# guoyihonggyh/MOBODY-Model-Based-Off-Dynamics-Offline-Reinforcement-Learning

Hardware: AMD Instinct MI355X
Metric: transitions/sec (minibatch rows through train(), refresh amortised at 1/5000) + grad-steps/sec (higher is better)
Workload: dtype f16x2

## Files before the change

### include/mobody_hip.h

```cpp
#ifndef MOBODY_HIP_H
#define MOBODY_HIP_H
#include <stddef.h>
#include <stdint.h>

#ifdef __cplusplus
extern "C" {
#endif

#define MOBODY_ABI_VERSION 6
#define MOBODY_E_ARG (-1)
#define MOBODY_E_LAUNCH (-2)
#define MOBODY_E_UNSUPPORTED (-3)

#define MOBODY_HIDDEN 256
#define MOBODY_ENSEMBLE 7
#define MOBODY_LATENT 16

enum { MOBODY_TERM_NEVER = 0, MOBODY_TERM_HALFCHEETAH = 1, MOBODY_TERM_HOPPER = 2, MOBODY_TERM_ANT = 3,
       MOBODY_TERM_WALKER2D = 4, MOBODY_TERM_HUMANOID = 5, MOBODY_TERM_PEN = 6 };

typedef struct MobodyLayer {
  int32_t in_dim, out_dim;
  int32_t Kp, Np;
  int64_t w_off, b_off;
// ... 31 lines not shown
#define MOBODY_HEALTH_F16_RANGE 1
#define MOBODY_HEALTH_NONFINITE 2
#define MOBODY_F16_W_LIMIT 255.875f
int mobody_health_bind(int32_t* words_dev);
int mobody_health_clear(void* stream);

int mobody_rng_normal(uint32_t seed, uint32_t stream_id, uint32_t call, int64_t n, float* out, void* stream);
int mobody_rng_index(uint32_t seed, uint32_t stream_id, uint32_t call, int64_t n, uint32_t bound, int32_t* out,
                     void* stream);

int mobody_dyn_forward(const float* dyn_blob, const float* dyn_planes, int precision, int S, int A, const float* obs,
                       const float* act, int64_t B, int use_trg, float* mean, void* stream);
int64_t mobody_dyn_planes_floats(void);
int mobody_dyn_planes(const float* dyn_blob, int S, int A, float* planes, int precision, void* stream);

int64_t mobody_dyn_step_workspace(int S, int A, int64_t B);

int mobody_dyn_step(const float* dyn_blob, const float* dyn_planes, int precision, int S, int A, int task,
                    const float* obs, const float* act, int64_t B,
                    const float* noise, const int32_t* elite_idx, const uint8_t* alive, const int32_t* elites,
                    int n_elites, uint32_t seed,
                    uint32_t call, const int64_t* call_dev, float penalty_coef, int use_penalty, int use_trg, float* next_obs,
                    float* reward,
                    uint8_t* terminal, float* penalty, float* raw_reward, float* mean_out, float* workspace,
                    void* stream);

int mobody_mopo_step(const float* dyn_blob, const float* dyn_planes, const float* mopo_blob, const float* mopo_blob_T,
                     int precision, int S, int A, int task, const float* obs, const float* act, int64_t B,
                     const float* noise, const int32_t* elite_idx, const uint8_t* alive, const int32_t* elites,
                     int n_elites, uint32_t seed, uint32_t call, float penalty_coef, int use_penalty, float* next_obs,
                     float* reward, uint8_t* terminal, float* penalty, float* raw_reward, float* mean_out,
                     float* workspace, void* stream);

enum { MOBODY_UNC_PAIRWISE = 0,
       MOBODY_UNC_ALEATORIC = 1,
       MOBODY_UNC_ENS_STD = 2 };

typedef struct MobodyEnsStep {
  int32_t struct_bytes, uncertainty_mode;
  const float *dyn_blob, *dyn_planes, *mopo_blob, *mopo_blob_T;
  int32_t precision, S, A, task;
  const float *obs, *act;
  int64_t B;
  const float* noise; const int32_t* elite_idx; const uint8_t* alive;
  const int32_t* elites;
  int32_t n_elites; uint32_t seed, call; int32_t use_penalty;
  const int64_t* call_dev;
  float penalty_coef; int32_t use_trg;
  float *next_obs, *reward; uint8_t* terminal; float *penalty, *raw_reward, *mean_out, *workspace;
} MobodyEnsStep;
int mobody_ens_step(const MobodyEnsStep* a, void* stream);

typedef struct MobodyBufferView {
  const float* state; const float* action; const float* next_state; const float* reward; const float* not_done;
  int64_t pitch;
} MobodyBufferView;
int64_t mobody_ring_pitch(int S, int A);

int64_t mobody_rollout_workspace(int S, int A, int64_t B);
int mobody_rollout(const float* dyn_blob, const float* dyn_planes, const float* actor_blob, const float* actor_blob_T,
                   int precision, int S, int A, int task, float max_action,
                   const float* init_obs, int64_t B, int H, const int32_t* elites, int n_elites, uint32_t seed, uint32_t call0,
                   float penalty_coef, int use_penalty, int use_trg, float env_filter, int filter_bad_rollout,
                   const MobodyBufferView* ring, int64_t cap, int64_t* ptr_size, float* workspace, void* stream);

typedef struct MobodyEnsRollout {
  int32_t struct_bytes, uncertainty_mode;
  const float *dyn_blob, *dyn_planes, *mopo_blob, *mopo_blob_T, *actor_blob, *actor_blob_T;
  int32_t precision, S, A, task;
  const float* init_obs;
  int64_t B;
  int32_t H, n_elites;
  const int32_t* elites;
  uint32_t seed, call0;
  const int64_t* call_dev;
  float max_action, penalty_coef, env_filter; int32_t use_penalty, use_trg, filter_bad_rollout;
  const MobodyBufferView* ring;
  int64_t cap;
  int64_t* ptr_size;
  float* workspace;
} MobodyEnsRollout;
int64_t mobody_ens_rollout_workspace(const MobodyEnsRollout* a);
int mobody_ens_rollout(const MobodyEnsRollout* a, void* stream);

int mobody_termination(int task, const float* next_obs, int64_t B, int S, uint8_t* done, void* stream);

int mobody_rollout_mask(const uint8_t* alive_in, const uint8_t* terminal, const float* penalty, float env_filter,
                        int use_filter, int64_t B, uint8_t* keep, uint8_t* alive_out, void* stream);

int mobody_sample_indices(uint32_t seed, uint32_t stream_id, const int64_t* counter, int64_t call_offset, int64_t n,
                          const int64_t* size, int32_t* out, void* stream);

int mobody_counter_add(int64_t* counter, int n, int64_t inc, void* stream);

int mobody_mlp3_forward(const float* blob, const float* blob_T, int precision, int in_dim, int out_dim, int members,
                        const float* src0, int n0, const float* src1, int n1, int64_t rows, int out_mode,
                        float max_action, float* out, float* save_x, float* save_h1, float* save_h2, void* stream);

int mobody_gather_batch(const MobodyBufferView* bufs, const int32_t* const* idx, const int64_t* counts, int nbuf,
                        int S, int A, float* state, float* action, float* next_state, float* reward, float* not_done,
                        void* stream);

int mobody_gather_batch_rng(const MobodyBufferView* bufs, const int64_t* counts, int nbuf, int S, int A,
                            const uint32_t* seeds, const int64_t* call_offsets, const int64_t* counter,
                            const int64_t* const* sizes, float* state, float* action, float* next_state,
                            float* reward, float* not_done, int64_t* const* bump, int nbump, void* stream);

int mobody_ring_append(const MobodyBufferView* ring, int64_t cap, int64_t* ptr_size, int S, int A, const float* obs,
                       const float* act, const float* next_obs, const float* reward, const uint8_t* terminal,
                       const uint8_t* keep, int64_t M, int32_t* scan_ws, void* stream);

typedef struct MobodyTrainDims {
  int32_t S, A;
  int64_t N;
  int64_t Nt;
  int64_t N_global;
  int64_t Nt_global;
} MobodyTrainDims;

typedef struct MobodyHyper {
  float gamma, tau, max_action, weight, bc_coef;
  int32_t q_weighted, scale_q;
  int32_t precision;
} MobodyHyper;

int64_t mobody_train_workspace(const MobodyTrainDims* d);

int mobody_critic_step(const MobodyTrainDims* d, const MobodyHyper* h, const float* actor_blob, const float* actor_blob_T,
                       const float* q_blob, const float* q_blob_T, const float* qtarg_blob, const float* qtarg_blob_T,
                       const float* state, const float* action, const float* next_state, const float* reward,
                       const float* not_done, const float* q_next, float* grad_q, float* loss_out, float* workspace,
                       int policy_forward, void* stream);

int mobody_critic_update(const MobodyTrainDims* d, const MobodyHyper* h, const float* actor_blob, const float* actor_blob_T,
                         float* q_blob, float* q_blob_T, float* qtarg_blob, float* qtarg_blob_T, const float* state,
                         const float* action, const float* next_state, const float* reward, const float* not_done,
                         const float* q_next, float* m, float* v, int64_t t, const int64_t* t_dev, float lr,
                         float* loss_out, float* workspace, int policy_forward, int64_t* bump, void* stream);

int mobody_actor_forward(const MobodyTrainDims* d, const MobodyHyper* h, const float* actor_blob, const float* actor_blob_T,
                         const float* q_blob, const float* q_blob_T, const float* state, const float* action, float* stats,
                         float* workspace, int policy_ready, void* stream);

int mobody_actor_backward(const MobodyTrainDims* d, const MobodyHyper* h, const float* actor_blob,
                          const float* actor_blob_T, const float* q_blob, const float* q_blob_T, const float* state,
                          const float* action, const float* stats, const float* v_true, float* grad_actor,
                          float* loss_out, float* workspace, void* stream);

int mobody_critic_update_phase(const MobodyTrainDims* d, const MobodyHyper* h, const float* actor_blob, const float* actor_blob_T,
                               float* q_blob, float* q_blob_T, float* qtarg_blob, float* qtarg_blob_T, const float* state,
                               const float* action, const float* next_state, const float* reward, const float* not_done,
                               const float* q_next, float* m, float* v, int64_t t, const int64_t* t_dev, float lr, float* loss_out,
                               float* workspace, int policy_forward, int64_t* bump, int phase, void* stream);

int mobody_actor_update(const MobodyTrainDims* d, const MobodyHyper* h, float* actor_blob, float* actor_blob_T,
                        const float* q_blob, const float* q_blob_T, const float* state, const float* action,
                        const float* stats, const float* v_true, float* m, float* v, int64_t t, const int64_t* t_dev,
                        float lr, float* loss_out, float* workspace, void* stream);

int mobody_value_loss_grad(const float* qt, const float* v, int64_t N, int64_t N_global, float* dz3, float* loss_out,
                           float* lossp_ws, void* stream);

int mobody_adam_polyak(int in_dim, int out_dim, int members, float* blob, float* blob_T, const float* grad, float* m,
                       float* v, float* target, float* target_T, int64_t t, float lr, float tau, float grad_scale,
                       int precision, void* stream);

int mobody_adam_polyak_dev(int in_dim, int out_dim, int members, float* blob, float* blob_T, const float* grad,
                           float* m, float* v, float* target, float* target_T, const int64_t* t_dev, float lr, float tau,
                           float grad_scale, int precision, void* stream);

int mobody_par_penalty(const float* next_state_true, const float* next_state_model, float* reward, float coef,
                       int64_t n, int S, void* stream);

int64_t mobody_mlp3_backward_workspace(int in_dim, int out_dim, int members, int64_t rows);
int mobody_mlp3_backward(const float* blob_T, int in_dim, int out_dim, int members, const float* dz3, const float* x,
                         const float* h1, const float* h2, int64_t rows, float* grad, float* workspace, void* stream);

int mobody_dara_inputs(const float* s, const float* a, const float* s2, int64_t N, int S, int A, float std,
                       const float* noise_sas, const float* noise_sa, uint32_t seed, uint32_t call, float* x_sas,
                       float* x_sa, void* stream);

int mobody_dara_loss_grad(const float* z_sas, const float* z_sa, const int32_t* labels, int64_t N, int64_t n_src,
                          float* dz_sas, float* dz_sa, float* loss_out, float* lossp_ws, void* stream);

int mobody_dara_penalty(const float* z_sas, const float* z_sa, int64_t n, float coef, float* reward, float* delta_out,
                        void* stream);

typedef struct MobodyPretrainLayout {
  int32_t S, A, za_in, _pad;
  MobodyMlpLayout enc, tr, rw;
  int64_t off_enc, off_tr, off_rw, off_za_src, off_za_trg;
  int64_t za_w1, za_b1, za_w2, za_b2, za_member_floats;
  int64_t total_floats;
  int64_t t_off_enc, t_off_tr, t_off_rw, t_total_floats;
} MobodyPretrainLayout;
int mobody_pretrain_layout(int S, int A, MobodyPretrainLayout* out);
int mobody_pretrain_transpose(int S, int A, const float* blob, float* blob_T, int precision, void* stream);
int64_t mobody_pretrain_workspace(int S, int A, int64_t b);

int mobody_pretrain_gather(const float* state, const float* action, const float* next_state, const float* reward,
                           const int32_t* idx, int64_t n_idx, int64_t start, const int64_t* start_dev, int64_t b, int S,
                           int A, float* xenc, float* act, float* rew, void* stream);

int mobody_pretrain_grads(int S, int A, int64_t b, int64_t b_global, int use_trg, float encoder_loss_coef,
                          const float* blob, const float* blob_T, const float* xenc, const float* act, const float* rew,
                          const float* noise6, const float* noise7, uint32_t seed, uint32_t call, float* grad,
                          float* loss_out, float* workspace, int precision, float transition_coef, float reward_coef,
                          void* stream);

int mobody_pretrain_update(int S, int A, int64_t b, int use_trg, float encoder_loss_coef, float* blob, float* blob_T,
                           const float* xenc, const float* act, const float* rew, const float* noise6, const float* noise7,
                           uint32_t seed, uint32_t call, const int64_t* call_dev, float* m, float* v, int64_t t_main,
                           int64_t t_za, const int64_t* t_dev, float lr, float* loss_out, float* loss_acc, float* workspace,
                           int precision, void* stream);

int mobody_pretrain_adam(int S, int A, int use_trg, float* blob, float* blob_T, const float* grad, float* m, float* v,
                         int64_t t_main, int64_t t_za, float lr, float grad_scale, int precision, int net_mask, int64_t t_rw,
                         void* stream);

int mobody_pretrain_za_adam(int S, int A, int use_trg, float* blob, const float* grad, float* m, float* v, int64_t t_za,
                            float lr, float grad_scale, void* stream);

int64_t mobody_dyn_validate_workspace(int S, int A, int64_t B);
int mobody_dyn_validate(const float* dyn_blob, int S, int A, const float* obs, const float* act, const float* next_obs,
                        const float* rew, int64_t B, int use_trg, float* out, float* workspace, void* stream);

typedef struct MobodyPretrainMopoLayout {
  int32_t S, A, _pad0, _pad1;
  MobodyMlpLayout dyn, rw;
  int64_t off_dyn, off_rw, total_floats;
  int64_t t_off_dyn, t_off_rw, t_total_floats;
} MobodyPretrainMopoLayout;
int mobody_pretrain_mopo_layout(int S, int A, MobodyPretrainMopoLayout* out);
int mobody_pretrain_mopo_transpose(int S, int A, const float* blob, float* blob_T, int precision, void* stream);
int64_t mobody_pretrain_mopo_workspace(int S, int A, int64_t b);
int mobody_pretrain_mopo_grads(int S, int A, int64_t b, int64_t b_global, int use_trg, float encoder_loss_coef,
                               const float* blob, const float* blob_T, const float* xenc, const float* act, const float* rew,
                               const float* noise, uint32_t seed, uint32_t call, float* grad, float* loss_out,
                               float* workspace, int precision, void* stream);
int mobody_pretrain_mopo_update(int S, int A, int64_t b, int use_trg, float encoder_loss_coef, float* blob, float* blob_T,
                                const float* xenc, const float* act, const float* rew, const float* noise, uint32_t seed,
                                uint32_t call, const int64_t* call_dev, float* m, float* v, int64_t t, const int64_t* t_dev,
                                float lr, float* loss_out, float* loss_acc, float* workspace, int precision, void* stream);
int mobody_pretrain_mopo_adam(int S, int A, float* blob, float* blob_T, const float* grad, float* m, float* v, int64_t t,
                              float lr, float grad_scale, int precision, void* stream);
int mobody_dyn_validate_mopo(const float* dyn_blob, const float* mopo_blob, int S, int A, const float* obs, const float* act,
                             const float* next_obs, const float* rew, int64_t B, float* out, float* workspace, void* stream);

int mobody_mlp_transpose(int in_dim, int out_dim, int members, const float* blob, float* blob_T, int precision,
                         void* stream);

#ifdef __cplusplus
}
#endif
#endif
```

### mobody-model-based-off-dynamics-offline-reinforcement-learning_amd/_lib.py

```python
import ctypes as C
import os

_HERE = os.path.dirname(os.path.abspath(__file__))
LIB_PATH = os.path.join(_HERE, "csrc", "libmobody_hip.so")

i32, i64, u32, f32 = C.c_int32, C.c_int64, C.c_uint32, C.c_float
vp = C.c_void_p


class MobodyLayer(C.Structure):
    _fields_ = [("in_dim", i32), ("out_dim", i32), ("Kp", i32), ("Np", i32), ("w_off", i64), ("b_off", i64)]


DL_NAMES = ["zs1", "zs2", "zs3", "za_src1", "za_src2", "za_trg1", "za_trg2", "transition1", "transition2",
            "transition3", "reward_model1", "reward_model2", "reward_model3"]


class MobodyDynLayout(C.Structure):
    _fields_ = [("S", i32), ("A", i32), ("E", i32), ("_pad", i32), ("layer", MobodyLayer * len(DL_NAMES)),
                ("total_floats", i64)]


class MobodyMlpLayout(C.Structure):
    _fields_ = [("in_dim", i32), ("out_dim", i32), ("members", i32), ("Kp1", i32), ("Np3", i32), ("Np1t", i32),
                ("w1", i64), ("b1", i64), ("w2", i64), ("b2", i64), ("w3", i64), ("b3", i64),
                ("member_floats", i64), ("total_floats", i64), ("w3t", i64), ("w2t", i64), ("w1t", i64),
                ("t_member_floats", i64), ("t_total_floats", i64), ("w2p", i64), ("w2tp", i64)]


class MobodyPretrainLayout(C.Structure):
    _fields_ = [("S", i32), ("A", i32), ("za_in", i32), ("_pad", i32), ("enc", MobodyMlpLayout), ("tr", MobodyMlpLayout),
                ("rw", MobodyMlpLayout), ("off_enc", i64), ("off_tr", i64), ("off_rw", i64), ("off_za_src", i64),
                ("off_za_trg", i64), ("za_w1", i64), ("za_b1", i64), ("za_w2", i64), ("za_b2", i64),
                ("za_member_floats", i64), ("total_floats", i64), ("t_off_enc", i64), ("t_off_tr", i64),
                ("t_off_rw", i64), ("t_total_floats", i64)]


class MobodyPretrainMopoLayout(C.Structure):
    _fields_ = [("S", i32), ("A", i32), ("_pad0", i32), ("_pad1", i32), ("dyn", MobodyMlpLayout), ("rw", MobodyMlpLayout),
                ("off_dyn", i64), ("off_rw", i64), ("total_floats", i64), ("t_off_dyn", i64), ("t_off_rw", i64),
                ("t_total_floats", i64)]


class MobodyBufferView(C.Structure):
    _fields_ = [("state", vp), ("action", vp), ("next_state", vp), ("reward", vp), ("not_done", vp), ("pitch", i64)]


class MobodyTrainDims(C.Structure):
    _fields_ = [("S", i32), ("A", i32), ("N", i64), ("Nt", i64), ("N_global", i64), ("Nt_global", i64)]


class MobodyHyper(C.Structure):
    _fields_ = [("gamma", f32), ("tau", f32), ("max_action", f32), ("weight", f32), ("bc_coef", f32),
                ("q_weighted", i32), ("scale_q", i32), ("precision", i32)]


class MobodyEnsStep(C.Structure):
    _fields_ = [("struct_bytes", i32), ("uncertainty_mode", i32), ("dyn_blob", vp), ("dyn_planes", vp), ("mopo_blob", vp),
                ("mopo_blob_T", vp), ("precision", i32), ("S", i32), ("A", i32), ("task", i32), ("obs", vp), ("act", vp),
                ("B", i64), ("noise", vp), ("elite_idx", vp), ("alive", vp), ("elites", C.POINTER(i32)), ("n_elites", i32),
                ("seed", u32), ("call", u32), ("use_penalty", i32), ("call_dev", vp), ("penalty_coef", f32), ("use_trg", i32),
                ("next_obs", vp), ("reward", vp), ("terminal", vp), ("penalty", vp), ("raw_reward", vp), ("mean_out", vp),
                ("workspace", vp)]


class MobodyEnsRollout(C.Structure):
    _fields_ = [("struct_bytes", i32), ("uncertainty_mode", i32), ("dyn_blob", vp), ("dyn_planes", vp), ("mopo_blob", vp),
                ("mopo_blob_T", vp), ("actor_blob", vp), ("actor_blob_T", vp), ("precision", i32), ("S", i32), ("A", i32),
                ("task", i32), ("init_obs", vp), ("B", i64), ("H", i32), ("n_elites", i32), ("elites", C.POINTER(i32)),
                ("seed", u32), ("call0", u32), ("call_dev", vp), ("max_action", f32), ("penalty_coef", f32),
                ("env_filter", f32), ("use_penalty", i32), ("use_trg", i32), ("filter_bad_rollout", i32),
                ("ring", C.POINTER(MobodyBufferView)), ("cap", i64), ("ptr_size", vp), ("workspace", vp)]


PRECISIONS = {"f32": 0, "bf16": 1, "bf16x2": 2, "bf16x3": 3, "f16x2": 4}


UNCERTAINTY_MODES = {"pairwise-diff": 0, "aleatoric": 1, "ensemble_std": 2}

TERM_IDS = {"never": 0, "halfcheetah": 1, "hopper": 2, "ant": 3, "walker2d": 4, "humanoid": 5, "pen": 6}

HEALTH_WORDS, HEALTH_F16_RANGE, HEALTH_NONFINITE = 8, 1, 2

PROTOTYPES = {
    "mobody_last_error": (C.c_char_p, []),
    "mobody_abi_version": (C.c_int, []),
    "mobody_dyn_layout": (C.c_int, [C.c_int, C.c_int, C.POINTER(MobodyDynLayout)]),
    "mobody_mlp_layout": (C.c_int, [C.c_int, C.c_int, C.c_int, C.POINTER(MobodyMlpLayout)]),
    "mobody_prof_begin": (C.c_int, [C.c_int]),
    "mobody_prof_end": (C.c_int, [C.POINTER(C.c_double), C.POINTER(i64), C.c_int]),
    "mobody_health_bind": (C.c_int, [vp]),
    "mobody_health_clear": (C.c_int, [vp]),
    "mobody_rng_normal": (C.c_int, [u32, u32, u32, i64, vp, vp]),
    "mobody_rng_index": (C.c_int, [u32, u32, u32, i64, u32, vp, vp]),
    "mobody_dyn_forward": (C.c_int, [vp, vp, C.c_int, C.c_int, C.c_int, vp, vp, i64, C.c_int, vp, vp]),
    "mobody_dyn_planes_floats": (i64, []),
    "mobody_dyn_planes": (C.c_int, [vp, C.c_int, C.c_int, vp, C.c_int, vp]),
    "mobody_dyn_step_workspace": (i64, [C.c_int, C.c_int, i64]),
    "mobody_dyn_step": (C.c_int, [vp, vp, C.c_int, C.c_int, C.c_int, C.c_int, vp, vp, i64, vp, vp, vp, C.POINTER(i32), C.c_int,
                                  u32, u32, vp, f32, C.c_int, C.c_int, vp, vp, vp, vp, vp, vp, vp, vp]),
    "mobody_mopo_step": (C.c_int, [vp, vp, vp, vp, C.c_int, C.c_int, C.c_int, C.c_int, vp, vp, i64, vp, vp, vp, C.POINTER(i32), C.c_int,
                                   u32, u32, f32, C.c_int, vp, vp, vp, vp, vp, vp, vp, vp]),
    "mobody_ens_step": (C.c_int, [C.POINTER(MobodyEnsStep), vp]),
    "mobody_ens_rollout_workspace": (i64, [C.POINTER(MobodyEnsRollout)]),
    "mobody_ens_rollout": (C.c_int, [C.POINTER(MobodyEnsRollout), vp]),
    "mobody_rollout_workspace": (i64, [C.c_int, C.c_int, i64]),
    "mobody_rollout": (C.c_int, [vp, vp, vp, vp, C.c_int, C.c_int, C.c_int, C.c_int, f32, vp, i64, C.c_int, C.POINTER(i32), C.c_int, u32, u32, f32,
                                 C.c_int, C.c_int, f32, C.c_int, C.POINTER(MobodyBufferView), i64, vp, vp, vp]),
    "mobody_termination": (C.c_int, [C.c_int, vp, i64, C.c_int, vp, vp]),
    "mobody_rollout_mask": (C.c_int, [vp, vp, vp, f32, C.c_int, i64, vp, vp, vp]),
    "mobody_sample_indices": (C.c_int, [u32, u32, vp, i64, i64, vp, vp, vp]),
    "mobody_counter_add": (C.c_int, [vp, C.c_int, i64, vp]),
    "mobody_mlp3_forward": (C.c_int, [vp, vp, C.c_int, C.c_int, C.c_int, C.c_int, vp, C.c_int, vp, C.c_int, i64, C.c_int, f32, vp,
                                      vp, vp, vp, vp]),
    "mobody_gather_batch": (C.c_int, [C.POINTER(MobodyBufferView), C.POINTER(vp), C.POINTER(i64), C.c_int, C.c_int,
                                      C.c_int, vp, vp, vp, vp, vp, vp]),
    "mobody_gather_batch_rng": (C.c_int, [C.POINTER(MobodyBufferView), C.POINTER(i64), C.c_int, C.c_int, C.c_int,
                                          C.POINTER(u32), C.POINTER(i64), vp, C.POINTER(vp), vp, vp, vp, vp, vp, C.POINTER(vp), C.c_int,
                                          vp]),
    "mobody_ring_append": (C.c_int, [C.POINTER(MobodyBufferView), i64, vp, C.c_int, C.c_int, vp, vp, vp, vp, vp, vp, i64, vp,
                                     vp]),
    "mobody_ring_pitch": (i64, [C.c_int, C.c_int]),
    "mobody_train_workspace": (i64, [C.POINTER(MobodyTrainDims)]),
    "mobody_critic_step": (C.c_int, [C.POINTER(MobodyTrainDims), C.POINTER(MobodyHyper), vp, vp, vp, vp, vp, vp, vp, vp, vp,
                                     vp, vp, vp, vp, vp, vp, C.c_int, vp]),
    "mobody_critic_update": (C.c_int, [C.POINTER(MobodyTrainDims), C.POINTER(MobodyHyper), vp, vp, vp, vp, vp, vp, vp, vp, vp,
                                       vp, vp, vp, vp, vp, i64, vp, f32, vp, vp, C.c_int, vp, vp]),
    "mobody_critic_update_phase": (C.c_int, [C.POINTER(MobodyTrainDims), C.POINTER(MobodyHyper), vp, vp, vp, vp, vp, vp, vp, vp, vp,
                                             vp, vp, vp, vp, vp, i64, vp, f32, vp, vp, C.c_int, vp, C.c_int, vp]),
    "mobody_actor_update": (C.c_int, [C.POINTER(MobodyTrainDims), C.POINTER(MobodyHyper), vp, vp, vp, vp, vp, vp, vp,
                                      vp, vp, vp, i64, vp, f32, vp, vp, vp]),
    "mobody_value_loss_grad": (C.c_int, [vp, vp, i64, i64, vp, vp, vp, vp]),
    "mobody_actor_forward": (C.c_int, [C.POINTER(MobodyTrainDims), C.POINTER(MobodyHyper), vp, vp, vp, vp, vp, vp, vp, vp,
                                       C.c_int, vp]),
    "mobody_actor_backward": (C.c_int, [C.POINTER(MobodyTrainDims), C.POINTER(MobodyHyper), vp, vp, vp, vp, vp, vp,
                                        vp, vp, vp, vp, vp, vp]),
    "mobody_adam_polyak": (C.c_int, [C.c_int, C.c_int, C.c_int, vp, vp, vp, vp, vp, vp, vp, i64, f32, f32, f32, C.c_int, vp]),
    "mobody_adam_polyak_dev": (C.c_int, [C.c_int, C.c_int, C.c_int, vp, vp, vp, vp, vp, vp, vp, vp, f32, f32, f32, C.c_int, vp]),
    "mobody_par_penalty": (C.c_int, [vp, vp, vp, f32, i64, C.c_int, vp]),
    "mobody_mlp3_backward_workspace": (i64, [C.c_int, C.c_int, C.c_int, i64]),
    "mobody_mlp3_backward": (C.c_int, [vp, C.c_int, C.c_int, C.c_int, vp, vp, vp, vp, i64, vp, vp, vp]),
    "mobody_dara_inputs": (C.c_int, [vp, vp, vp, i64, C.c_int, C.c_int, f32, vp, vp, u32, u32, vp, vp, vp]),
    "mobody_dara_loss_grad": (C.c_int, [vp, vp, vp, i64, i64, vp, vp, vp, vp, vp]),
    "mobody_dara_penalty": (C.c_int, [vp, vp, i64, f32, vp, vp, vp]),
    "mobody_mlp_transpose": (C.c_int, [C.c_int, C.c_int, C.c_int, vp, vp, C.c_int, vp]),
    "mobody_pretrain_layout": (C.c_int, [C.c_int, C.c_int, C.POINTER(MobodyPretrainLayout)]),
    "mobody_pretrain_transpose": (C.c_int, [C.c_int, C.c_int, vp, vp, C.c_int, vp]),
    "mobody_pretrain_workspace": (i64, [C.c_int, C.c_int, i64]),
    "mobody_pretrain_gather": (C.c_int, [vp, vp, vp, vp, vp, i64, i64, vp, i64, C.c_int, C.c_int, vp, vp, vp, vp]),
    "mobody_pretrain_update": (C.c_int, [C.c_int, C.c_int, i64, C.c_int, f32, vp, vp, vp, vp, vp, vp, vp, u32, u32, vp, vp,
                                         vp, i64, i64, vp, f32, vp, vp, vp, C.c_int, vp]),
    "mobody_pretrain_grads": (C.c_int, [C.c_int, C.c_int, i64, i64, C.c_int, f32, vp, vp, vp, vp, vp, vp, vp, u32, u32,
                                        vp, vp, vp, C.c_int, f32, f32, vp]),
    "mobody_pretrain_adam": (C.c_int, [C.c_int, C.c_int, C.c_int, vp, vp, vp, vp, vp, i64, i64, f32, f32, C.c_int, C.c_int, i64, vp]),
    "mobody_pretrain_za_adam": (C.c_int, [C.c_int, C.c_int, C.c_int, vp, vp, vp, vp, i64, f32, f32, vp]),
    "mobody_pretrain_mopo_layout": (C.c_int, [C.c_int, C.c_int, C.POINTER(MobodyPretrainMopoLayout)]),
    "mobody_pretrain_mopo_transpose": (C.c_int, [C.c_int, C.c_int, vp, vp, C.c_int, vp]),
    "mobody_pretrain_mopo_workspace": (i64, [C.c_int, C.c_int, i64]),
    "mobody_pretrain_mopo_grads": (C.c_int, [C.c_int, C.c_int, i64, i64, C.c_int, f32, vp, vp, vp, vp, vp, vp, u32, u32, vp, vp,
                                             vp, C.c_int, vp]),
    "mobody_pretrain_mopo_update": (C.c_int, [C.c_int, C.c_int, i64, C.c_int, f32, vp, vp, vp, vp, vp, vp, u32, u32, vp, vp, vp,
                                              i64, vp, f32, vp, vp, vp, C.c_int, vp]),
    "mobody_pretrain_mopo_adam": (C.c_int, [C.c_int, C.c_int, vp, vp, vp, vp, vp, i64, f32, f32, C.c_int, vp]),
    "mobody_dyn_validate_mopo": (C.c_int, [vp, vp, C.c_int, C.c_int, vp, vp, vp, vp, i64, vp, vp, vp]),
    "mobody_dyn_validate_workspace": (i64, [C.c_int, C.c_int, i64]),
    "mobody_dyn_validate": (C.c_int, [vp, C.c_int, C.c_int, vp, vp, vp, vp, i64, C.c_int, vp, vp, vp]),
}

_lib = None


def load():
    global _lib
    if _lib is not None:
        return _lib
    import torch
    if not os.path.exists(LIB_PATH):
        raise ImportError(
            f"{LIB_PATH} not found: build it with `python {os.path.join(_HERE, 'csrc', 'build.py')}` "
            "(or __graft_entry__.build()). There is no CPU fallback for the MOBODY hot path.")
    lib = C.CDLL(LIB_PATH)
    for name, (res, args) in PROTOTYPES.items():
        fn = getattr(lib, name)
        fn.restype, fn.argtypes = res, args
    if lib.mobody_abi_version() != 6:
        raise ImportError("libmobody_hip.so ABI version mismatch")
    _lib = lib
    return lib


class MobodyError(RuntimeError):
    pass


def check(rc, what=""):
    if rc != 0:
        msg = load().mobody_last_error().decode(errors="replace")
        raise MobodyError(f"{what} failed ({rc}): {msg}")


def ptr(t):
    if t is None:
        return None
    assert t.is_contiguous(), "C ABI needs contiguous tensors"
    return t.data_ptr()


_dev_index = None


def cur_stream():
    global _dev_index
    import torch
    if _dev_index is None:
        _dev_index = torch.cuda.current_device()
    return torch._C._cuda_getCurrentRawStream(_dev_index)


def dyn_layout(S, A):
    L = MobodyDynLayout()
    check(load().mobody_dyn_layout(S, A, C.byref(L)), "mobody_dyn_layout")
    return L


def mlp_layout(in_dim, out_dim, members):
    L = MobodyMlpLayout()
    check(load().mobody_mlp_layout(in_dim, out_dim, members, C.byref(L)), "mobody_mlp_layout")
    return L


def pretrain_layout(S, A):
    L = MobodyPretrainLayout()
    check(load().mobody_pretrain_layout(S, A, C.byref(L)), "mobody_pretrain_layout")
    return L


def pretrain_mopo_layout(S, A):
    L = MobodyPretrainMopoLayout()
    check(load().mobody_pretrain_mopo_layout(S, A, C.byref(L)), "mobody_pretrain_mopo_layout")
    return L
```

### mobody-model-based-off-dynamics-offline-reinforcement-learning_amd/algo/offline_offline/mobody.py

```python
import numpy as np
import torch

from ... import _lib, dp, ops, packing
from .. import utils

REFRESH_EVERY = 5000
REFRESH_SRC, REFRESH_TAR = 50000, 2000
REFRESH_FROM_SRC_TAR = 100
GRAPH_DYN_SEED = 0x51ED


class _PackedNet(object):

    def __init__(self, in_dim, out_dim, members, prefixes, device, out_mode=0, max_action=1.0, init=True, precision=0):
        self.in_dim, self.out_dim, self.members, self.prefixes = in_dim, out_dim, members, prefixes
        self.device, self.out_mode, self.max_action = device, out_mode, float(max_action)
        self.precision = int(precision)
        self.layout = _lib.mlp_layout(in_dim, out_dim, members)
        if init:
            sd = {}
            for p in prefixes:
                for li, (i, o) in zip((0, 2, 4), ((in_dim, 256), (256, 256), (256, out_dim))):
                    bound = 1.0 / np.sqrt(i)
                    sd[f"{p}network.{li}.weight"] = torch.empty(o, i).uniform_(-bound, bound)
# ... 288 lines not shown
        rew_mean = res["rewards"].mean()
        if self.config["filter_bad_rollout"]:
            keep = (res["penalty"] <= self.config["env_filter"]).squeeze(1)
            res = {k: v[keep] for k, v in res.items()}
        return res, {"num_transitions": n_tr, "reward_mean": rew_mean}

    def _rollout_into_fake(self, init_obss, rollout_length, use_trg=True):
        if rollout_length == 0:
            return 0
        dyn, m, fb = self.dynamics, self.dynamics.model, self.fake_replay_buffer
        obs = init_obss.contiguous()
        B = obs.shape[0]
        m.inference()
        self._roll_ws = ops.rollout(m.packed(), self.policy.blob, self.S, self.A, dyn._task_id, self.policy.max_action, obs,
                                    rollout_length, list(m.elites_host()),
                                    (dyn.seed + dp.rank_salt()) & 0xFFFFFFFF, dyn._calls + 1, float(dyn._penalty_coef or 0.0),
                                    use_trg, True, self.config["env_filter"], self.config["filter_bad_rollout"],
                                    fb._fields(), fb.max_size, fb.ptr_size, getattr(self, "_roll_ws", None),
                                    dyn_planes=m.planes() if dyn.precision else None, actor_blob_T=self.policy.blob_T,
                                    precision=dyn.precision, mopo=m.packed_mopo() if getattr(m, "mopo", False) else None,
                                    uncertainty_mode=dyn._unc_id)
        dyn._calls += rollout_length
        fb._pull()
        return B * rollout_length

    def _refresh(self, src_rb, tar_rb, batch_size):
        cfg = self.config
        world = self._world() if int(cfg.get("shard_refresh", 1)) else 1
        n_src, n_tar = -(-REFRESH_SRC // world), -(-REFRESH_TAR // world)
        s_idx = src_rb.draw_indices(n_src)
        t_idx = tar_rb.draw_indices(n_tar)
        src = ops.gather_batch([src_rb._fields()], [s_idx], self.S, self.A)
        tar = ops.gather_batch([tar_rb._fields()], [t_idx], self.S, self.A)
        if self.rng == "device":
            self._rollout_into_fake(src[0], cfg["src_rollout_length"])
            self._rollout_into_fake(tar[0], cfg["trg_rollout_length"])
        else:
            tr, _ = self.rollout(src[0], cfg["src_rollout_length"])
            self.fake_replay_buffer.add_batch(tr)
            tr, _ = self.rollout(tar[0], cfg["trg_rollout_length"])
            self.fake_replay_buffer.add_batch(tr)
        if cfg["use_src_sa_to_get_target_next_state"]:
            r = self.dynamics.step_device(src[0], src[1])
            keep = (r["penalty"] < cfg["env_filter"]).to(torch.uint8).squeeze(1)
            self.fake_replay_buffer.add_batch(dict(obss=src[0], next_obss=r["next_obs"], actions=src[1],
                                                   rewards=r["reward"], terminals=r["terminal"]), keep=keep)
        if cfg["rollout_from_src"]:
            if self.penalty_type != "dara":
                self.update_classifier(src_rb, tar_rb, batch_size)
            s_idx = src_rb.draw_indices(n_src)
            t_idx = tar_rb.draw_indices(-(-REFRESH_FROM_SRC_TAR // world))
            init = ops.gather_batch([src_rb._fields(), tar_rb._fields()], [s_idx, t_idx], self.S, self.A)[0]
            tr, _ = self.rollout(init, cfg["rollout_from_src_length"], use_trg=False)
            if tr is not None and tr["obss"].shape[0] > 0:
                self._dara_delta(tr["obss"].contiguous(), tr["actions"].contiguous(), tr["next_obss"].contiguous(),
                                 tr["rewards"], cfg["penalty_coef"])
                self.fake_replay_buffer.add_batch(tr)

    def _health_check(self):
        words = ops.health_bound(self.device)
        if words is None or self._fault is not None:
            return
        mask, step = ops.health_read(words)
        if mask == 0:
            return
        cls = self.classifier
        nets = (("q_funcs", self.q_funcs, self.q_optimizer), ("target_q_funcs", self.target_q_funcs, self.q_optimizer),
                ("policy", self.policy, self.policy_optimizer), ("v_func", self.v_func, self.v_optimizer),
                ("classifier.sa_classifier", cls.sa_classifier, cls.opt_sa), ("classifier.sas_classifier", cls.sas_classifier, cls.opt_sas))
        found = []
        for name, n, opt in nets:
            w2 = ops._mlp_w2(n.blob, n.layout, n.members)
            m = float(w2.abs().max())
            if (n.precision == 4 and not (m < ops.F16_W_LIMIT)) or not bool(torch.isfinite(n.blob).all()):
                found.append((name, m, opt))
        frozen = self._health_rewind(step, found[0][2] if found else None)
        self._graph = None
        bits = "|".join(ops.health_bits(mask))
        where = ", ".join(f"{name} (max |W2| = {m:g})" for name, m, _ in found) or "no policy network (another object on this device)"
        msg = (f"device health word {bits}" + (f" at Adam step {step}" if step else "") + f": {where}; "
               f"{frozen} optimizer step(s) were frozen, the parameters are those of the last healthy update (an optimizer launch "
               f"that ran next to the faulting one on another stream, if there was one, may hold that step in part). "
               f"f16x2 planes hold |w| < {ops.F16_W_LIMIT}: use mfma='bf16x3' (or f16_guard='fallback')")
        if self.f16_guard == "fallback" and mask == _lib.HEALTH_F16_RANGE and found:
            import warnings
            warnings.warn("falling back to mfma='bf16x3': " + msg)
            self.mfma, self.precision = "bf16x3", ops.prec_id("bf16x3")
            self.config["mfma"] = "bf16x3"
            for n in (self.q_funcs, self.target_q_funcs, self.policy):
                n.precision = self.precision
                ops.mlp_transpose(n.blob, n.in_dim, n.out_dim, n.members, out=n.blob_T, precision=self.precision)
                n.version += 1
            self._ws, self._ws_key = None, None
            ops.health_clear()
            return
        self._fault = msg
        raise FloatingPointError(msg)

    def _health_rewind(self, step, opt):
        order = [self.v_optimizer, self.q_optimizer, self.policy_optimizer]
        if opt not in order or step <= 0 or opt.t < step:
            return 0
        n = opt.t - step
        k = order.index(opt)
        for j, o in enumerate(order):
            if o.t > 0:
                o.t = max(0, o.t - n - (1 if j > k else 0))
        return n

    def _graph_ok(self, writer):
        want = self.use_graph == 1 or (self.use_graph == 2 and self._batch[0].shape[0] < 4096)
        dyn = self.dynamics
        par_ok = self.penalty_type != "par" or (dyn is not None and getattr(dyn, "noise_fn", None) is None
                                                and dyn.rng == "device")
        adv_ok = not self.config["advantage"] or (self._world() == 1 and self.fused_update and self._v_ws is not None)
        logs = writer is not None and (self.total_it % 5000 == 0 or (self.penalty_type == "par" and self.total_it % 100 == 0))
        return (want and self.rng == "device" and par_ok and adv_ok and (self.total_it - 1) % REFRESH_EVERY != 0 and not logs)

    @staticmethod
    def _world():
        d = torch.distributed
        return d.get_world_size() if d.is_available() and d.is_initialized() else 1

    def _graph_segments(self, src, tar, batch_size, world, segmented):
        cfg, S, A = self.config, self.S, self.A
        ns, nt = int(cfg["src_ratio"] * batch_size), int(cfg["trg_ratio"] * batch_size)
        nf = int(cfg["fake_batch_scale"] * batch_size) if cfg["fake_batch_scale"] != 0 else 0
        N, Nt = ns + nt + nf, ns + nt
        Ng, Ntg = N * world, Nt * world
        c, b = self._ctr, self._batch
        bufs, cnts, seeds = [src, tar], [ns, nt], [self._seed_for(101), self._seed_for(102)]
        if nf > 0:
            bufs.append(self.fake_replay_buffer); cnts.append(nf); seeds.append(self._seed_for(103))

        par = self.penalty_type == "par"

        def par_relabel(call):
            r = self.dynamics.step_device(b[0][:ns], b[1][:ns], call=call, call_dev=c[0:1], seed_offset=GRAPH_DYN_SEED)
            ops.par_penalty(b[2][:ns], r["next_obs"], b[3][:ns], cfg["penalty_coef"])

        def critic():
            ops.counter_add(c[0:3])
            ops.gather_batch_rng([rb._fields() for rb in bufs], cnts, seeds, [0] * len(bufs), c[0:1],
                                 [rb.ptr_size[1:2] for rb in bufs], S, A, b)
            if par:
                par_relabel(0)
            self.critic_grad(b, N, Nt, Ng, Ntg)

        def critic_apply_actor_stats():
            self.q_optimizer.step_dev(c[1:2], target=self.target_q_funcs, tau=self.tau)
            self.actor_stats(b, N, Nt, Ng, Ntg)

        def fused_step():
            ops.gather_batch_rng([rb._fields() for rb in bufs], cnts, seeds, [1] * len(bufs), c[0:1],
                                 [rb.ptr_size[1:2] for rb in bufs], S, A, b, bump=(c[1:2], c[2:3], c[3:4]))
            if par and not cfg["advantage"] and int(cfg.get("par_overlap", 1)):
                main = torch.cuda.current_stream()
                if getattr(self, "_side_stream", None) is None:
                    self._side_stream = torch.cuda.Stream(device=self.device)
                side = self._side_stream
                side.wait_stream(main)
                with torch.cuda.stream(side):
                    par_relabel(1)
                self.critic_update(b, N, Nt, t_dev=c[1:2], bump=c[0:1], phase=1)
                main.wait_stream(side)
                self.critic_update(b, N, Nt, t_dev=c[1:2], bump=c[0:1], phase=2)
                self.actor_stats(b, N, Nt, N, Nt)
                self.actor_update(b, N, Nt, t_dev=c[2:3])
                return
            if par:
                par_relabel(1)
            if cfg["advantage"]:
                self.value_grad(b, N, Nt, N, Nt)
                self.v_optimizer.step_dev(c[3:4])
            self.critic_update(b, N, Nt, t_dev=c[1:2], bump=c[0:1])
            self.actor_stats(b, N, Nt, N, Nt)
            self.actor_update(b, N, Nt, t_dev=c[2:3])

        def actor():
            self.actor_grad(b, N, Nt, Ng, Ntg)

        def actor_apply():
            self.policy_optimizer.step_dev(c[2:3])

        if not segmented:
            if self.fused_update:
                return [fused_step]
            return [lambda: (critic(), critic_apply_actor_stats(), actor(), actor_apply())]
        if self.dp_graph == "captured":
            d = torch.distributed

            def whole_step():
                critic(); d.all_reduce(self.q_optimizer.grad)
                critic_apply_actor_stats(); d.all_reduce(self._stats)
                actor(); d.all_reduce(self.policy_optimizer.grad)
                actor_apply()
            return [whole_step]
        return [critic, critic_apply_actor_stats, actor, actor_apply]

    def _graph_step(self, src, tar, batch_size):
        world = self._world()
        segmented = world > 1 or (self._force_segments and torch.distributed.is_initialized())
        if segmented and self.dp_graph == "captured" and torch.distributed.get_backend() != "nccl":
            self.dp_graph = "segments"
        fb = self.fake_replay_buffer
        nets = (self.q_funcs, self.target_q_funcs, self.policy, self.v_func)
        opts = (self.q_optimizer, self.policy_optimizer, self.v_optimizer)
        dyn_key = None
        if self.penalty_type == "par":
            m = self.dynamics.model
            dyn_key = (m.packed().data_ptr(), m.planes().data_ptr() if self.dynamics.precision else 0, self.dynamics.precision,
                       m.elites_host(), float(self.dynamics._penalty_coef or 0.0), self.dynamics._unc_id,
                       tuple(t.data_ptr() for t in m.packed_mopo()) if getattr(m, "mopo", False) else None)
        key = (batch_size, id(src), id(tar), src.state.data_ptr(), tar.state.data_ptr(), world, segmented,
               id(fb), fb.state.data_ptr(), fb.ptr_size.data_ptr(), tuple(t.data_ptr() for t in self._batch),
               tuple((n.blob.data_ptr(), n.blob_T.data_ptr()) for n in nets), self.precision,
               tuple((o.m.data_ptr(), o.v.data_ptr(), o.grad.data_ptr()) for o in opts),
               None if self._ws is None else self._ws.data_ptr(), self.dp_graph, dyn_key,
               None if self._v_ws is None else self._v_ws.data_ptr())
        if self._graph is None or self._graph_key != key:
            torch.cuda.synchronize()
            self._ctr[1] = self.q_optimizer.t
            self._ctr[2] = self.policy_optimizer.t
            self._ctr[3] = self.v_optimizer.t
            if self.penalty_type == "par":
                self.dynamics.step_device(self._batch[0][:int(self.config["src_ratio"] * batch_size)],
                                          self._batch[1][:int(self.config["src_ratio"] * batch_size)], call=0)
            graphs = []
            try:
                for seg in self._graph_segments(src, tar, batch_size, world, segmented):
                    g = torch.cuda.CUDAGraph()
                    with torch.cuda.graph(g, capture_error_mode="thread_local"):
                        seg()
                    graphs.append(g)
            except Exception as exc:
                import warnings
                torch.cuda.synchronize()
                if segmented and self.dp_graph == "captured":
                    warnings.warn(f"capturing the all-reduces failed ({exc!r}); falling back to segment graphs")
                    self.dp_graph, self._graph = "segments", None
                    return self._graph_step(src, tar, batch_size)
                warnings.warn(f"HIP-graph capture of the train() step failed ({exc!r}); continuing eagerly")
                self.use_graph, self._graph = 0, None
                return False
            self._graph, self._graph_key = graphs, key
        if len(self._graph) == 1:
            self._graph[0].replay()
        else:
            d = torch.distributed
            ga, gb, gc, gd = self._graph
            ga.replay()
            d.all_reduce(self.q_optimizer.grad)
            gb.replay()
            d.all_reduce(self._stats)
            gc.replay()
            d.all_reduce(self.policy_optimizer.grad)
            gd.replay()
        self.q_optimizer.t += 1
        self.policy_optimizer.t += 1
        if self.config["advantage"]:
            self.v_optimizer.t += 1
        return True

    def train(self, src_replay_buffer, tar_replay_buffer, batch_size=128, writer=None, wandbrun=None):
        cfg = self.config
        self.total_it += 1
        self.src_replay_buffer, self.tar_replay_buffer = src_replay_buffer, tar_replay_buffer
        if not self._synced:
            self.sync_replicas()
        S, A = self.S, self.A
        ns, nt = int(cfg["src_ratio"] * batch_size), int(cfg["trg_ratio"] * batch_size)
        nf = int(cfg["fake_batch_scale"] * batch_size) if cfg["fake_batch_scale"] != 0 else 0
        N, Nt = ns + nt + nf, ns + nt
        if (self.total_it - 1) % REFRESH_EVERY == 0 or (writer is not None and self.total_it % 5000 == 0):
            self._health_check()
        if (self._batch is not None and self._batch_key == (N,) and self._graph_ok(writer)
                and self._graph_step(src_replay_buffer, tar_replay_buffer, batch_size)):
            return
        if self._graph is not None:
            self._graph = None
        if self.penalty_type == "dara" and self.total_it == 1:
            self._dara_warmup(src_replay_buffer, tar_replay_buffer, batch_size, writer)
        if self._batch_key != (N,):
            dev = self.device
            self._batch = (torch.empty(N, S, device=dev), torch.empty(N, A, device=dev), torch.empty(N, S, device=dev),
                           torch.empty(N, 1, device=dev), torch.empty(N, 1, device=dev))
            self._batch_key = (N,)
        b = self._batch
        self._gather([src_replay_buffer, tar_replay_buffer], [ns, nt], tuple(t[:Nt] for t in b))
        if self.penalty_type == "par":
            r = self.dynamics.step_device(b[0][:ns], b[1][:ns])
            if writer is not None and self.total_it % 100 == 0:
                writer.add_scalar("train/reward_penalty_par", torch.mean((b[2][:ns] - r["next_obs"]) ** 2), global_step=self.total_it)
            ops.par_penalty(b[2][:ns], r["next_obs"], b[3][:ns], cfg["penalty_coef"])
        if (self.total_it - 1) % REFRESH_EVERY == 0:
            self._refresh(src_replay_buffer, tar_replay_buffer, batch_size)
        if nf > 0:
            self._gather([self.fake_replay_buffer], [nf], tuple(t[Nt:] for t in b))
        log5k = writer is not None and self.total_it % 5000 == 0
        if log5k and cfg["advantage"]:
            qt = ops.mlp3_forward(self.target_q_funcs.blob, S + A, 1, 2, b[0], b[1]).view(2, N)
            v0 = ops.mlp3_forward(self.v_func.blob, S, 1, 1, b[0]).view(N)
            writer.add_scalar("train/adv", (torch.minimum(qt[0], qt[1]) - v0).mean(), self.total_it)
            writer.add_scalar("train/value", v0.mean(), self.total_it)
        self._update(b, N, Nt)
        if log5k:
            if cfg["q_weighted"] and Nt > 0:
                qb = ops.mlp3_forward(self.q_funcs.blob, S + A, 1, 2, b[0][:Nt], b[1][:Nt], blob_T=self.q_funcs.blob_T,
                                      precision=self.precision).view(2, Nt)
                qb = torch.minimum(qb[0], qb[1])
                if cfg["advantage"]:
                    adv = qb - ops.mlp3_forward(self.v_func.blob, S, 1, 1, b[0][:Nt]).view(Nt)
                else:
                    adv = qb / qb.abs().mean()
                writer.add_scalar("train/exp_adv", torch.exp(3.0 * adv).clamp(max=100.0).mean(), self.total_it)
            q_loss, pi_loss, bc_loss = [float(x) for x in self._loss[:3].tolist()]
            writer.add_scalar("train/q_loss", q_loss, self.total_it)
            writer.add_scalar("train/policy_loss", pi_loss, self.total_it)
            writer.add_scalar("train/bc_loss", bc_loss, self.total_it)
            prec = self.precision
            q12 = ops.mlp3_forward(self.q_funcs.blob, self.S + self.A, 1, 2, b[0], b[1], blob_T=self.q_funcs.blob_T, precision=prec)
            pi = ops.mlp3_forward(self.policy.blob, self.S, self.A, 1, b[0], out_mode=1, max_action=cfg["max_action"],
                                  blob_T=self.policy.blob_T, precision=prec)[0]
            qpi = ops.mlp3_forward(self.q_funcs.blob, self.S + self.A, 1, 2, b[0], pi, blob_T=self.q_funcs.blob_T, precision=prec)
            writer.add_scalar("train/q1", q12[0].mean(), self.total_it)
            writer.add_scalar("train/q_behavior", torch.minimum(q12[0], q12[1]).mean(), self.total_it)
            writer.add_scalar("train/q_policy", torch.minimum(qpi[0], qpi[1]).mean(), self.total_it)
            if wandbrun is not None:
                wandbrun.log({"train/policy_loss": pi_loss, "train/q_loss": q_loss}, step=self.total_it)

    def _gather(self, bufs, counts, out):
        if self.rng == "device":
            for rb in bufs:
                if rb.size <= 0:
                    raise ValueError("low >= high")
                rb._draws += 1
            salt = dp.rank_salt()
            ops.gather_batch_rng([rb._fields() for rb in bufs], counts, [(rb.seed + salt) & 0xFFFFFFFF for rb in bufs],
                                 [rb._draws for rb in bufs], None, [rb.ptr_size[1:2] for rb in bufs], self.S, self.A, out)
        else:
            idx = [rb.draw_indices(n) for rb, n in zip(bufs, counts)]
            ops.gather_batch([rb._fields() for rb in bufs], idx, self.S, self.A, out=out)

    def _update(self, b, N, Nt):
        d = torch.distributed
        dist = d if d.is_available() and d.is_initialized() else None
        if self.fused_update and dp.world_size(dist) == 1:
            if self.config["advantage"]:
                self.value_grad(b, N, Nt, N, Nt)
                self.value_apply()
            self.critic_update(b, N, Nt)
            self.actor_stats(b, N, Nt, N, Nt)
            self.actor_update(b, N, Nt)
        else:
            dp.dp_update(self, b, N, Nt, dist)

    def comm_device(self):
        return self.device

    def _dims(self, N, Nt, Ng, Ntg):
        if self._ws_key != (N, Nt):
            self._ws = ops.train_workspace(ops.train_dims(self.S, self.A, N, Nt, N, Nt), self.device)
            self._ws_key = (N, Nt)
        return ops.train_dims(self.S, self.A, N, Nt, Ng, Ntg), ops.hyper(self.config)

    def has_value_phase(self):
        return bool(self.config["advantage"])

    def value_grad(self, b, N, Nt, Ng, Ntg):
        S, A = self.S, self.A
        qt = ops.mlp3_forward(self.target_q_funcs.blob, S + A, 1, 2, b[0], b[1])
        v, x, h1, h2 = ops.mlp3_forward(self.v_func.blob, S, 1, 1, b[0], save=True)
        dz3, loss = ops.value_loss_grad(qt.view(2, N), v.view(N), Ng)
        self._v_ws = ops.mlp3_backward(self.v_func.blob_T, S, 1, 1, dz3, x, h1, h2, self.v_optimizer.grad, self._v_ws)
        self._loss[3:4].copy_(loss)

    def value_grad_buffer(self):
        return self.v_optimizer.grad

    def value_apply(self):
        self.v_optimizer.step()

    def critic_grad(self, b, N, Nt, Ng, Ntg):
        dims, hyp = self._dims(N, Nt, Ng, Ntg)
        q_next = None
        if self.config["advantage"]:
            q_next = ops.mlp3_forward(self.v_func.blob, self.S, 1, 1, b[2]).view(N)
        ops.critic_step(dims, hyp, self.policy.blob, self.q_funcs.blob, self.q_funcs.blob_T, self.target_q_funcs.blob,
                        b, self.q_optimizer.grad, self._loss[0:1], self._ws, q_next=q_next,
                        policy_forward=self._policy_rides_along(), actor_blob_T=self.policy.blob_T,
                        qtarg_blob_T=self.target_q_funcs.blob_T)

    def _policy_rides_along(self):
        return not self.config["advantage"]

    def critic_update(self, b, N, Nt, t_dev=None, bump=None, phase=0):
        dims, hyp = self._dims(N, Nt, N, Nt)
        q_next = None
        if self.config["advantage"]:
            assert phase == 0, "the phased critic update is not used with the V-function target"
            q_next = ops.mlp3_forward(self.v_func.blob, self.S, 1, 1, b[2]).view(N)
        o = self.q_optimizer
        if t_dev is None and phase != 2:
            o.t += 1
        ops.critic_update(dims, hyp, self.policy.blob, self.q_funcs.blob, self.q_funcs.blob_T, self.target_q_funcs.blob, b,
                          o.m, o.v, o.t, o.lr, self._loss[0:1], self._ws, q_next=q_next, t_dev=t_dev,
                          policy_forward=self._policy_rides_along(), actor_blob_T=self.policy.blob_T,
                          qtarg_blob_T=self.target_q_funcs.blob_T, bump=bump, phase=phase)

    def actor_update(self, b, N, Nt, t_dev=None):
        dims, hyp = self._dims(N, Nt, N, Nt)
        v_true = None
        if self.config["advantage"] and Nt > 0:
            v_true = ops.mlp3_forward(self.v_func.blob, self.S, 1, 1, b[0][:Nt]).view(Nt)
        o = self.policy_optimizer
        if t_dev is None:
            o.t += 1
        ops.actor_update(dims, hyp, self.policy.blob, self.policy.blob_T, self.q_funcs.blob, self.q_funcs.blob_T, b[0], b[1],
                         self._stats, o.m, o.v, o.t, o.lr, self._loss[1:3], self._ws, v_true=v_true, t_dev=t_dev)

    def critic_grad_buffer(self):
        return self.q_optimizer.grad

    def critic_apply(self):
        self.q_optimizer.step(target=self.target_q_funcs, tau=self.tau)

    def actor_stats(self, b, N, Nt, Ng, Ntg):
        dims, hyp = self._dims(N, Nt, Ng, Ntg)
        ops.actor_forward(dims, hyp, self.policy.blob, self.q_funcs.blob, b[0], b[1], self._stats, self._ws,
                          policy_ready=self._policy_rides_along(), actor_blob_T=self.policy.blob_T, q_blob_T=self.q_funcs.blob_T)

    def stats_buffer(self):
        return self._stats

    def actor_grad(self, b, N, Nt, Ng, Ntg):
        dims, hyp = self._dims(N, Nt, Ng, Ntg)
        v_true = None
        if self.config["advantage"] and Nt > 0:
            v_true = ops.mlp3_forward(self.v_func.blob, self.S, 1, 1, b[0][:Nt]).view(Nt)
        ops.actor_backward(dims, hyp, self.policy.blob, self.policy.blob_T, self.q_funcs.blob, self.q_funcs.blob_T,
                           b[0], b[1], self._stats, self.policy_optimizer.grad, self._loss[1:3], self._ws, v_true=v_true)

    def actor_grad_buffer(self):
        return self.policy_optimizer.grad

    def actor_apply(self):
        self.policy_optimizer.step()

    def losses(self):
        return tuple(float(x) for x in self._loss[:3].tolist())

    def save(self, filename):
        self._health_check()
        torch.save(self.q_funcs.state_dict(), filename + "_critic")
        torch.save(self.q_optimizer.state_dict(), filename + "_critic_optimizer")
        torch.save(self.policy.state_dict(), filename + "_actor")
        torch.save(self.policy_optimizer.state_dict(), filename + "_actor_optimizer")

    def load(self, filename):
        self._graph = None
        self._synced = False
        ld = lambda s: torch.load(filename + s, map_location="cpu", weights_only=True)
        self.q_funcs.load_state_dict(ld("_critic"))
        self.q_optimizer.load_state_dict(ld("_critic_optimizer"))
        self.policy.load_state_dict(ld("_actor"))
        self.policy_optimizer.load_state_dict(ld("_actor_optimizer"))
```

### mobody-model-based-off-dynamics-offline-reinforcement-learning_amd/csrc/layers.h

```cpp
#pragma once
#include <stdint.h>
#include <stdlib.h>

#include <type_traits>

#include "../../include/mobody_hip.h"
#include "tile.h"

namespace mobody {

template <int ACT, int MT, class Extra, class Between>
__device__ __forceinline__ void wide_layer(float* Xs, const float* __restrict__ W, const float* __restrict__ b, int Kp,
                                           WideRing& ring, Extra&& extra, Between&& between, uint32_t* mask = nullptr,
                                           bool full = false, int mask_groups = 1 << 30) {
  const float bias0 = b[64 * wave_col() + (lane_id() & 31)], bias1 = b[64 * wave_col() + 32 + (lane_id() & 31)];
  f32x16 acc[MT][2];
  wide_zero<MT>(acc);
  wide_gemm<MT>(Xs, W, Kp, acc, ring);
  if (Kp == HID) TR(3);
  between();
  lds_barrier();
  if (full) {
    wide_foreach<MT>(acc, [&](int row, int col, float v) {
      const float y = activate<ACT>(v + ((col & 32) ? bias1 : bias0));
      Xs[row * LDX + col] = y;
      extra(std::false_type{}, row, col, y);
    });
  } else {
    wide_foreach<MT>(acc, [&](int row, int col, float v) {
      const float y = activate<ACT>(v + ((col & 32) ? bias1 : bias0));
      Xs[row * LDX + col] = y;
      extra(std::true_type{}, row, col, y);
    });
  }
  if (mask != nullptr) {
    const int i = lane_id() & 31, hh = lane_id() >> 5;
#pragma unroll
    for (int mt = 0; mt < MT; ++mt)
#pragma unroll
      for (int nt = 0; nt < 2; ++nt) {
        const float bias = nt ? bias1 : bias0;
        uint32_t word = 0;
#pragma unroll
        for (int r = 0; r < 16; ++r)
          word |= (uint32_t)(activate<ACT>(acc[mt][nt][r] + bias) > 0.f) << ((r & 3) + 8 * (r >> 2) + 4 * hh);
        word |= (uint32_t)__shfl_xor((int)word, 32);
        if (hh == 0 && mt < mask_groups) mask[mt * HID + 64 * wave_col() + 32 * nt + i] = word;
      }
  }
  lds_barrier();
}

template <int ACT, int MT, class Extra>
__device__ __forceinline__ void wide_layer(float* Xs, const float* __restrict__ W, const float* __restrict__ b, int Kp,
                                           Extra&& extra) {
  WideRing ring;
  wide_prefetch(W, Kp, ring);
  wide_layer<ACT, MT>(Xs, W, b, Kp, ring, extra, [] {});
}

template <int MT, class Extra, class Between>
__device__ __forceinline__ void wide_layer_swish_d(float* Xs, const float* __restrict__ W, const float* __restrict__ b,
                                                   int Kp, WideRing& ring, Extra&& extra, Between&& between, bool full) {
  const float bias0 = b[64 * wave_col() + (lane_id() & 31)], bias1 = b[64 * wave_col() + 32 + (lane_id() & 31)];
  f32x16 acc[MT][2];
  wide_zero<MT>(acc);
  wide_gemm<MT>(Xs, W, Kp, acc, ring);
  between();
  lds_barrier();
  auto body = [&](auto guarded) {
    wide_foreach<MT>(acc, [&](int row, int col, float v) {
      const float z = v + ((col & 32) ? bias1 : bias0);
      const float sig = fast_rcp(1.f + __expf(-z));
      const float y = z * sig;
      Xs[row * LDX + col] = y;
      extra(guarded, row, col, y, sig * (1.f + z * (1.f - sig)));
    });
  };
  if (full) body(std::false_type{});
  else body(std::true_type{});
  lds_barrier();
}

struct NoExtra {
  template <class Guard>
  __device__ __forceinline__ void operator()(Guard, int, int, float) const {}
};

struct Mlp3FwdArgs {
  const float* src[3];
  int ld[3], n[3];
  long long src_ms[3];
  long long x_ms;
  const float *w1, *b1, *w2, *b2, *w3, *b3;
  long long sw1, sb1, sw2, sb2, sw3, sb3;
  int Kp1, Np3, nout;
  long long rows;
  float* out;
  long long out_mstride;
  int out_ld;
  float* save_x;
  float* save_h1;
  float* save_h2;
  uint32_t* mask1;
  uint32_t* mask2;
  const unsigned short* w2_planes;
  long long planes_ms;
  float* save_d1;
  float* save_d2;
  unsigned short* save_h1p;
  long long h1p_ms;
  long long h1p_plane;
  int* save_e1;
  int out_mode;
  const float* resid;
  int resid_ld;
  float max_action;
};

constexpr long long DYN_PLANE_MEMBER = 3LL * HID * HID;
__host__ __device__ inline long long dyn_planes_off(int layer, int member) { return ((long long)layer * NENS + member) * DYN_PLANE_MEMBER; }

inline Mlp3FwdArgs fwd_net(const float* blob, const MobodyMlpLayout& L, long long rows) {
  Mlp3FwdArgs a{};
  a.w1 = blob + L.w1; a.b1 = blob + L.b1; a.w2 = blob + L.w2; a.b2 = blob + L.b2; a.w3 = blob + L.w3; a.b3 = blob + L.b3;
  a.sw1 = a.sb1 = a.sw2 = a.sb2 = a.sw3 = a.sb3 = L.member_floats;
  a.Kp1 = L.Kp1; a.Np3 = L.Np3; a.nout = L.out_dim; a.rows = rows;
  return a;
}
inline void fwd_set_planes(Mlp3FwdArgs& a, const float* blob_T, const MobodyMlpLayout& L) {
  a.w2_planes = reinterpret_cast<const unsigned short*>(blob_T + L.w2p);
  a.planes_ms = 2 * L.t_member_floats;
}
inline Mlp3FwdArgs fwd_reward_head(const float* dyn_blob, const MobodyDynLayout& L, const float* dyn_planes, long long rows) {
  Mlp3FwdArgs a{};
  const MobodyLayer &l1 = L.layer[MOBODY_DL_RW1], &l2 = L.layer[MOBODY_DL_RW2], &l3 = L.layer[MOBODY_DL_RW3];
  a.w1 = dyn_blob + l1.w_off; a.b1 = dyn_blob + l1.b_off; a.sw1 = (long long)l1.Kp * l1.Np; a.sb1 = l1.Np;
  a.w2 = dyn_blob + l2.w_off; a.b2 = dyn_blob + l2.b_off; a.sw2 = (long long)l2.Kp * l2.Np; a.sb2 = l2.Np;
  a.w3 = dyn_blob + l3.w_off; a.b3 = dyn_blob + l3.b_off; a.sw3 = (long long)l3.Kp * l3.Np; a.sb3 = l3.Np;
  a.Kp1 = l1.Kp; a.Np3 = l3.Np; a.nout = 1; a.rows = rows;
  if (dyn_planes != nullptr) {
    a.w2_planes = reinterpret_cast<const unsigned short*>(dyn_planes) + dyn_planes_off(2, 0);
    a.planes_ms = DYN_PLANE_MEMBER;
  }
  return a;
}
inline void fwd_set_src(Mlp3FwdArgs& a, int k, const float* src, int ld, int n, long long ms = 0) {
  a.src[k] = src; a.ld[k] = ld; a.n[k] = n; a.src_ms[k] = ms;
}
inline void fwd_set_out(Mlp3FwdArgs& a, float* out, int out_mode, float max_action, const float* resid = nullptr, int resid_ld = 0) {
  a.out = out; a.out_mstride = a.rows * a.nout; a.out_ld = a.nout;
  a.out_mode = out_mode; a.max_action = max_action; a.resid = resid; a.resid_ld = resid_ld;
}
inline void fwd_set_saves(Mlp3FwdArgs& a, float* x, long long x_ms, float* h1, int* e1, float* h2, uint32_t* m1 = nullptr,
                          uint32_t* m2 = nullptr, float* d1 = nullptr, float* d2 = nullptr) {
  if (e1 != nullptr && h1 != nullptr) {
    const long long r32 = (a.rows + 31) & ~31LL;
    a.save_h1p = reinterpret_cast<unsigned short*>(h1); a.h1p_plane = r32 * HID; a.h1p_ms = 2 * r32 * HID; a.save_e1 = e1;
    h1 = nullptr;
  }
  a.save_x = x; a.x_ms = x_ms; a.save_h1 = h1; a.save_h2 = h2; a.mask1 = m1; a.mask2 = m2; a.save_d1 = d1; a.save_d2 = d2;
}

template <class F>
inline int dispatch_out_width(int Np3, F&& f) {
  return Np3 == 16 ? f(std::integral_constant<int, 1>{}) : Np3 == 32 ? f(std::integral_constant<int, 2>{})
                                                                     : f(std::integral_constant<int, 0>{});
}

int launch_mlp3_forward(const Mlp3FwdArgs& a, int members_a, const Mlp3FwdArgs& b, int members_b, int act, int prec, hipStream_t st);
inline int launch_mlp3_forward(const Mlp3FwdArgs& a, int members, int act, int prec, hipStream_t st) {
  return launch_mlp3_forward(a, members, Mlp3FwdArgs{}, 0, act, prec, st);
}

constexpr int MLP_TILE_ROWS = 32;
constexpr int MLP_MT = MLP_TILE_ROWS / 32;

__device__ __forceinline__ int fwd_load_sources(const Mlp3FwdArgs& a, int m, float* Xs, long long row0, int rows_here) {
  int c0 = 0;
#pragma unroll
  for (int k = 0; k < 3; ++k) {
    if (a.n[k] > 0) {
      tile_load(Xs, c0, a.src[k] + m * a.src_ms[k] + row0 * a.ld[k], a.ld[k], a.n[k], 0, rows_here, MLP_TILE_ROWS);
      c0 += a.n[k];
    }
  }
  return c0;
}

__device__ __forceinline__ void fwd_save_x(const Mlp3FwdArgs& a, int m, const float* Xs, long long row0, int rows_here) {
  if (a.save_x != nullptr && (m == 0 || a.x_ms != 0)) {
    const int c = threadIdx.x & 31, r0 = threadIdx.x >> 5;
    float* sx = a.save_x + m * a.x_ms;
    for (int col = c; col < a.Kp1; col += 32)
      for (int r = r0; r < rows_here; r += NTHREADS >> 5) sx[(row0 + r) * a.Kp1 + col] = Xs[r * LDX + col];
  }
}

struct FwdTileOut { float *h1, *h2; uint32_t *mask1, *mask2; float* out; };
__device__ __forceinline__ FwdTileOut fwd_tile_out(const Mlp3FwdArgs& a, int m, long long row0) {
  FwdTileOut t;
  t.h1 = a.save_h1 ? a.save_h1 + ((long long)m * a.rows + row0) * HID : nullptr;
  t.h2 = a.save_h2 ? a.save_h2 + ((long long)m * a.rows + row0) * HID : nullptr;
  const long long mtile = ((long long)m * ((a.rows + 31) / 32) + row0 / 32) * HID;
  t.mask1 = a.mask1 ? a.mask1 + mtile : nullptr;
  t.mask2 = a.mask2 ? a.mask2 + mtile : nullptr;
  t.out = a.out + m * a.out_mstride + row0 * a.out_ld;
  return t;
}

__device__ __forceinline__ void fwd_emit(const Mlp3FwdArgs& a, float* out, long long row0, int rows_here, int row, int col,
                                         float v, float bias) {
  if (row < rows_here && col < a.nout) {
    float y = v + bias;
    if (a.out_mode == 1) y = a.max_action * tanhf(y);
    if (a.resid != nullptr) y += a.resid[(row0 + row) * a.resid_ld + col];
    out[row * a.out_ld + col] = y;
  }
}

}
```

### mobody-model-based-off-dynamics-offline-reinforcement-learning_amd/csrc/mlp_fwd.hip

```cpp
#include <stdlib.h>

#include "common.h"
#include "layers.h"

namespace mobody {

constexpr int TB = MLP_TILE_ROWS;

template <int ACT, int NT>
__device__ __forceinline__ void mlp3_fwd_tail(const Mlp3FwdArgs& a, int m, float* Xs, WideRing& ring, float* h2,
                                              uint32_t* mask2, float* out, long long row0, int rows_here) {
  const float* w3 = a.w3 + m * a.sw3;
  const float* b3 = a.b3 + m * a.sb3;
  const bool full = rows_here == TB;
  auto save_h2 = [=](auto guarded, int row, int col, float y) {
    if (h2 != nullptr && (!decltype(guarded)::value || row < rows_here)) h2[row * HID + col] = y;
  };
  auto emit = [&](int row, int col, float v, float bias) { fwd_emit(a, out, row0, rows_here, row, col, v, bias); };
  if constexpr (NT > 0) {
    NarrowRegs<NT> br;
    const int mycol = threadIdx.x % (16 * NT);
    float bias;
    wide_layer<ACT, MLP_MT>(Xs, a.w2 + m * a.sw2, a.b2 + m * a.sb2, HID, ring, save_h2, [&] {
      narrow_prefetch<NT>(w3, 16 * NT, br);
      bias = b3[mycol < a.nout ? mycol : 0];
    }, mask2, full, (rows_here + 31) / 32);
    TR(4);
    narrow_run<TB / 16, NT>(Xs, br, [&](int row, int col, float v) { emit(row, col, v, bias); });
  } else {
    wide_layer<ACT, MLP_MT>(Xs, a.w2 + m * a.sw2, a.b2 + m * a.sb2, HID, ring, save_h2, [] {}, mask2, full, (rows_here + 31) / 32);
    TR(4);
    narrow_layer(Xs, w3, HID, a.Np3, [&](int row, int col, float v) { emit(row, col, v, b3[col < a.nout ? col : 0]); }, TB);
  }
}

template <int ACT, int NT>
__device__ __forceinline__ void mlp3_fwd_tile(const Mlp3FwdArgs& a, int m, float* Xs) {
  const long long row0 = (long long)blockIdx.x * TB;
  const int rows_here = (int)min((long long)TB, a.rows - row0);
  const float* w1 = a.w1 + m * a.sw1;
  const float* w2 = a.w2 + m * a.sw2;
  TR(0);
  WideRing ring;
  wide_prefetch(w1, a.Kp1, ring);
  tile_zero_cols(Xs, fwd_load_sources(a, m, Xs, row0, rows_here), a.Kp1, TB);
  lds_barrier();
  TR(1);
  fwd_save_x(a, m, Xs, row0, rows_here);
  const FwdTileOut t = fwd_tile_out(a, m, row0);
  float* h1 = t.h1;
  wide_layer<ACT, MLP_MT>(Xs, w1, a.b1 + m * a.sb1, a.Kp1, ring,
                      [=](auto guarded, int row, int col, float y) {
                        if (h1 != nullptr && (!decltype(guarded)::value || row < rows_here)) h1[row * HID + col] = y;
                      },
                      [&] { wide_prefetch(w2, HID, ring); }, t.mask1, rows_here == TB, (rows_here + 31) / 32);
  TR(2);
  mlp3_fwd_tail<ACT, NT>(a, m, Xs, ring, t.h2, t.mask2, t.out, row0, rows_here);
  TR(5);
}

template <int ACT, int NT>
__global__ __launch_bounds__(NTHREADS, 2) void k_mlp3_fwd(Mlp3FwdArgs a) {
  extern __shared__ __attribute__((aligned(16))) float Xs[];
  mlp3_fwd_tile<ACT, NT>(a, blockIdx.y, Xs);
}

template <int ACT, int NT>
__global__ __launch_bounds__(NTHREADS, 2) void k_mlp3_fwd2(Mlp3FwdArgs a, Mlp3FwdArgs b, int members_a) {
  extern __shared__ __attribute__((aligned(16))) float Xs[];
  const bool second = (int)blockIdx.y >= members_a;
  const Mlp3FwdArgs s = second ? b : a;
  if ((long long)blockIdx.x * TB >= s.rows) return;
  mlp3_fwd_tile<ACT, NT>(s, second ? (int)blockIdx.y - members_a : (int)blockIdx.y, Xs);
}

template <int ACT, int NT>
static int launch_fwd_t(const Mlp3FwdArgs& a, int members, hipStream_t stream) {
  size_t lds = (size_t)TB * LDX * sizeof(float);
  static bool once = false;
  if (!once) {
    int rc = allow_big_lds(k_mlp3_fwd<ACT, NT>, 160 * 1024);
    if (rc) return rc;
    once = true;
  }
  dim3 grid((unsigned)cdiv(a.rows, TB), (unsigned)members);
  ProfScope prof(PROF_MLP_FWD, stream);
  hipLaunchKernelGGL((k_mlp3_fwd<ACT, NT>), grid, dim3(NTHREADS), lds, stream, a);
  MB_LAUNCH_OK("k_mlp3_fwd");
  return 0;
}

template <int NT>
static int launch_fwd2_t(const Mlp3FwdArgs& a, int members_a, const Mlp3FwdArgs& b, int members_b, hipStream_t stream) {
  size_t lds = (size_t)TB * LDX * sizeof(float);
  static bool once = false;
  if (!once) {
    int rc = allow_big_lds(k_mlp3_fwd2<ACT_RELU, NT>, 160 * 1024);
    if (rc) return rc;
    once = true;
  }
  const long long rows = a.rows > b.rows ? a.rows : b.rows;
  dim3 grid((unsigned)cdiv(rows, TB), (unsigned)(members_a + members_b));
  ProfScope prof(PROF_MLP_FWD, stream);
  hipLaunchKernelGGL((k_mlp3_fwd2<ACT_RELU, NT>), grid, dim3(NTHREADS), lds, stream, a, b, members_a);
  MB_LAUNCH_OK("k_mlp3_fwd2");
  return 0;
}

static int launch_fwd_pair(const Mlp3FwdArgs& a, int members_a, const Mlp3FwdArgs& b, int members_b, hipStream_t stream) {
  return dispatch_out_width(a.Np3, [&](auto nt) { return launch_fwd2_t<decltype(nt)::value>(a, members_a, b, members_b, stream); });
}

template <int ACT>
static int launch_fwd_act(const Mlp3FwdArgs& a, int members, hipStream_t stream) {
  return dispatch_out_width(a.Np3, [&](auto nt) { return launch_fwd_t<ACT, decltype(nt)::value>(a, members, stream); });
}

static int launch_mlp3_fwd(const Mlp3FwdArgs& a, int members, int act, hipStream_t stream) {
  return act == ACT_SWISH ? launch_fwd_act<ACT_SWISH>(a, members, stream) : launch_fwd_act<ACT_RELU>(a, members, stream);
}

int launch_mlp3_fwd_bf(const Mlp3FwdArgs& a, int members_a, const Mlp3FwdArgs& b, int members_b, int act, int prec, hipStream_t st);
int launch_fwd_train(const Mlp3FwdArgs& a, int members, hipStream_t st);

static bool nets_share_launch(const Mlp3FwdArgs& a, const Mlp3FwdArgs& b, int act, int prec) {
  if (act != ACT_RELU) return false;
  return a.Np3 == b.Np3 || (prec == PREC_F16X2 && ((a.Np3 == 16 && b.Np3 == 32) || (a.Np3 == 32 && b.Np3 == 16)));
}

int launch_mlp3_forward(const Mlp3FwdArgs& a, int members_a, const Mlp3FwdArgs& b, int members_b, int act, int prec, hipStream_t st) {
  auto one = [&](const Mlp3FwdArgs& x, int members) {
    if (prec != PREC_F32) return launch_mlp3_fwd_bf(x, members, Mlp3FwdArgs{}, 0, act, prec, st);
    return x.save_d1 != nullptr ? launch_fwd_train(x, members, st) : launch_mlp3_fwd(x, members, act, st);
  };
  const bool has_a = members_a > 0 && a.rows > 0, has_b = members_b > 0 && b.rows > 0;
  if (!has_a || !has_b) return has_a ? one(a, members_a) : has_b ? one(b, members_b) : 0;
  if (!nets_share_launch(a, b, act, prec)) {
    int rc = one(a, members_a);
    return rc ? rc : one(b, members_b);
  }
  return prec == PREC_F32 ? launch_fwd_pair(a, members_a, b, members_b, st) : launch_mlp3_fwd_bf(a, members_a, b, members_b, act, prec, st);
}

}

using namespace mobody;

extern "C" int mobody_mlp3_forward(const float* blob, const float* blob_T, int precision, int in_dim, int out_dim,
                                   int members, const float* src0, int n0, const float* src1, int n1, int64_t rows,
                                   int out_mode, float max_action, float* out, float* save_x, float* save_h1,
                                   float* save_h2, void* stream) {
  MobodyMlpLayout L;
  int rc = mobody_mlp_layout(in_dim, out_dim, members, &L);
  if (rc) return rc;
  MB_REQUIRE(rows >= 0, "mobody_mlp3_forward: rows < 0");
  if (rows == 0) return 0;
  MB_REQUIRE(blob && src0 && out, "mobody_mlp3_forward: null pointer");
  MB_REQUIRE(n0 + n1 == in_dim && n0 > 0 && n1 >= 0 && (n1 == 0 || src1), "mobody_mlp3_forward: n0+n1=%d != in_dim=%d", n0 + n1, in_dim);
  rc = check_precision("mobody_mlp3_forward", precision, blob_T != nullptr);
  if (rc) return rc;
  Mlp3FwdArgs a = fwd_net(blob, L, rows);
  fwd_set_src(a, 0, src0, n0, n0);
  fwd_set_src(a, 1, src1, n1, n1);
  fwd_set_out(a, out, out_mode, max_action);
  fwd_set_saves(a, save_x, 0, save_h1, nullptr, save_h2);
  if (precision != PREC_F32) fwd_set_planes(a, blob_T, L);
  return launch_mlp3_forward(a, members, ACT_RELU, precision, as_stream(stream));
}
```

### mobody-model-based-off-dynamics-offline-reinforcement-learning_amd/csrc/mlp_fwd_bf.hip

```cpp
#include <stdlib.h>

#include "common.h"
#include "layers_bf.h"

namespace mobody {

constexpr int TB = MLP_TILE_ROWS, MT = MLP_MT;
constexpr int FWD_L1_RING = 3;
constexpr int FWD_F16_WAVES = 4;

template <int ACT, int PM, int NT, bool DS = false>
__device__ __forceinline__ void mlp3_fwd_bf_tile(const Mlp3FwdArgs& a, int m, float* Xs) {
  char* Ps = reinterpret_cast<char*>(Xs);
  float* scr = reinterpret_cast<float*>(Ps + split_scr_offset<PM, TB>());
  const long long row0 = (long long)blockIdx.x * TB;
  const int rows_here = (int)min((long long)TB, a.rows - row0);
  const bool full = rows_here == TB;
  const float* w1 = a.w1 + m * a.sw1;
  const s16x8* w2b = reinterpret_cast<const s16x8*>(a.w2_planes + m * a.planes_ms);
  const float* w3 = a.w3 + m * a.sw3;
  const float* b3 = a.b3 + m * a.sb3;
  TR(0);
  WideRingT<FWD_L1_RING> ring;
  wide_prefetch(w1, a.Kp1, ring);
  int c0;
  if (a.n[0] <= 32 && a.n[1] <= 32 && a.n[2] == 0) {
    tile_load2<TB>(Xs, a.src[0] + m * a.src_ms[0] + row0 * a.ld[0], a.ld[0], a.n[0],
                   a.n[1] > 0 ? a.src[1] + m * a.src_ms[1] + row0 * a.ld[1] : nullptr, a.ld[1], a.n[1], rows_here);
    c0 = a.n[0] + a.n[1];
  } else {
    c0 = fwd_load_sources(a, m, Xs, row0, rows_here);
  }
  tile_zero_cols(Xs, c0, a.Kp1, TB);
  lds_barrier();
  TR(1);
  fwd_save_x(a, m, Xs, row0, rows_here);
  const FwdTileOut t = fwd_tile_out(a, m, row0);
  float* d1 = DS ? a.save_d1 + ((long long)m * a.rows + row0) * HID : nullptr;
  float* d2 = DS ? a.save_d2 + ((long long)m * a.rows + row0) * HID : nullptr;
  const int mg = (rows_here + 31) / 32;
  BfRing<PM> bring;
  PlaneSave gs{nullptr, 0, nullptr};
  if (a.save_h1p != nullptr) {
    gs.base = reinterpret_cast<short*>(a.save_h1p) + m * a.h1p_ms + (row0 / 8) * (HID * 8);
    gs.plane_stride = a.h1p_plane;
    gs.e_out = a.save_e1 + (long long)m * cdiv(a.rows, 32) + row0 / 32;
  }
  const int e1 = wide_layer_to_planes<ACT, MT, PM, TB, DS>(Xs, Ps, scr, w1, a.b1 + m * a.sb1, a.Kp1, ring,
                                                           [&] { bf_prefetch<PM>(w2b, bring); }, t.mask1, full, mg, rows_here, t.h1, gs, d1);
  TR(2);
  auto emit = [&](int row, int col, float v, float bias) { fwd_emit(a, t.out, row0, rows_here, row, col, v, bias); };
  if constexpr (NT > 0) {
    NarrowRegs<NT> br;
    const int mycol = threadIdx.x % (16 * NT);
    float bias;
    bf_layer<ACT, MT, PM, TB, DS>(Xs, Ps, e1, w2b, a.b2 + m * a.sb2, bring, [&] {
      narrow_prefetch<NT>(w3, 16 * NT, br);
      bias = b3[mycol < a.nout ? mycol : 0];
    }, t.mask2, mg, rows_here, t.h2, d2);
    TR(4);
    narrow_run<TB / 16, NT>(Xs, br, [&](int row, int col, float v) { emit(row, col, v, bias); });
  } else {
    bf_layer<ACT, MT, PM, TB, DS>(Xs, Ps, e1, w2b, a.b2 + m * a.sb2, bring, [] {}, t.mask2, mg, rows_here, t.h2, d2);
    narrow_layer(Xs, w3, HID, a.Np3, [&](int row, int col, float v) { emit(row, col, v, b3[col < a.nout ? col : 0]); }, TB);
  }
  TR(5);
}

template <int ACT, int PM, int NT, bool DS = false, int NT2 = NT>
__global__ __launch_bounds__(NTHREADS, (PM == 4 && !DS) ? FWD_F16_WAVES : 2) void k_mlp3_fwd_bf(Mlp3FwdArgs a, Mlp3FwdArgs b, int members_a) {
  extern __shared__ __attribute__((aligned(16))) float Xs[];
  const bool second = (int)blockIdx.y >= members_a;
  const Mlp3FwdArgs s = second ? b : a;
  if ((long long)blockIdx.x * TB >= s.rows) return;
  if constexpr (NT2 == NT) {
    mlp3_fwd_bf_tile<ACT, PM, NT, DS>(s, second ? (int)blockIdx.y - members_a : (int)blockIdx.y, Xs);
  } else {
    if (second) mlp3_fwd_bf_tile<ACT, PM, NT2, DS>(s, (int)blockIdx.y - members_a, Xs);
    else mlp3_fwd_bf_tile<ACT, PM, NT, DS>(s, (int)blockIdx.y, Xs);
  }
}

template <int ACT, int PM, int NT, bool DS = false, int NT2 = NT>
static int launch_bf_t(const Mlp3FwdArgs& a, int members_a, const Mlp3FwdArgs& b, int members_b, hipStream_t st) {
  constexpr size_t lds = split_lds_bytes<PM, TB>();
  static bool once = false;
  if (!once) {
    int rc = allow_big_lds(k_mlp3_fwd_bf<ACT, PM, NT, DS, NT2>, 160 * 1024);
    if (rc) return rc;
    once = true;
  }
  const long long rows = a.rows > b.rows ? a.rows : b.rows;
  ProfScope prof(PROF_MLP_FWD, st);
  hipLaunchKernelGGL((k_mlp3_fwd_bf<ACT, PM, NT, DS, NT2>), dim3((unsigned)cdiv(rows, TB), (unsigned)(members_a + members_b)),
                     dim3(NTHREADS), lds, st, a, b, members_a);
  MB_LAUNCH_OK("k_mlp3_fwd_bf");
  return 0;
}

template <int ACT, int PM>
static int launch_bf_nt(const Mlp3FwdArgs& a, int ma, const Mlp3FwdArgs& b, int mb, hipStream_t st) {
  if constexpr (PM == 4 && ACT == ACT_RELU) {
    if (mb > 0 && a.Np3 != b.Np3)
      return a.Np3 == 16 ? launch_bf_t<ACT, PM, 1, false, 2>(a, ma, b, mb, st) : launch_bf_t<ACT, PM, 2, false, 1>(a, ma, b, mb, st);
  }
  return dispatch_out_width(a.Np3, [&](auto nt) { return launch_bf_t<ACT, PM, decltype(nt)::value>(a, ma, b, mb, st); });
}

int launch_mlp3_fwd_bf(const Mlp3FwdArgs& a, int members_a, const Mlp3FwdArgs& b, int members_b, int act, int prec, hipStream_t st) {
  if (a.save_d1 != nullptr || a.save_d2 != nullptr) {
    if (act != ACT_SWISH || prec != PREC_F16X2 || members_b != 0 || !a.save_d1 || !a.save_d2)
      return fail(MOBODY_E_ARG, "launch_mlp3_fwd_bf: derivative saves need one Swish net in the f16x2 mode");
    return dispatch_out_width(a.Np3, [&](auto nt) { return launch_bf_t<ACT_SWISH, 4, decltype(nt)::value, true>(a, members_a, b, 0, st); });
  }
#define BF_CASE(ACT, PM) launch_bf_nt<ACT, PM>(a, members_a, b, members_b, st)
  if (act == ACT_SWISH) return prec == PREC_BF16 ? BF_CASE(ACT_SWISH, 1) : prec == PREC_BF16X2 ? BF_CASE(ACT_SWISH, 2) : prec == PREC_BF16X3 ? BF_CASE(ACT_SWISH, 3) : BF_CASE(ACT_SWISH, 4);
  return prec == PREC_BF16 ? BF_CASE(ACT_RELU, 1) : prec == PREC_BF16X2 ? BF_CASE(ACT_RELU, 2) : prec == PREC_BF16X3 ? BF_CASE(ACT_RELU, 3) : BF_CASE(ACT_RELU, 4);
#undef BF_CASE
}

}
```

### mobody-model-based-off-dynamics-offline-reinforcement-learning_amd/csrc/replay.hip

```cpp
#include <stdlib.h>

#include "common.h"
#include "rng.h"

namespace mobody {

constexpr int ROWS_WG = 16;

__host__ __device__ inline bool view_packed(const MobodyBufferView& b, int S, int A) {
  return b.pitch > 0 && b.pitch % 16 == 0 && b.pitch >= 2LL * S + A + 2 && (reinterpret_cast<uintptr_t>(b.state) & 15) == 0 &&
         b.action == b.state + S && b.next_state == b.action + A && b.reward == b.next_state + S && b.not_done == b.reward + 1;
}

struct GatherArgs {
  MobodyBufferView bufs[3];
  int packed[3];
  const int32_t* idx[3];
  long long start[4];
  int nbuf, S, A, WS;
  float *state, *action, *next_state, *reward, *not_done;
  uint32_t seed[3];
  long long call_offset[3];
  const long long* counter;
  const long long* size[3];
  long long* bump[4];
  int nbump;
};

__host__ __device__ inline uint32_t div_magic(int n) { return (uint32_t)((0x100000000ULL + (uint32_t)n - 1) / (uint32_t)n); }
__device__ __forceinline__ int fast_div(int e, uint32_t magic, int n) { return n == 1 ? e : (int)__umulhi((uint32_t)e, magic); }

__device__ __forceinline__ void stage_to_batch(const float* stage, int WS, int off, int n, int rows, float* out) {
  const uint32_t magic = div_magic(n);
  for (int e = threadIdx.x; e < rows * n; e += 256) {
    const int r = fast_div(e, magic, n), c = e - r * n;
    out[e] = stage[r * WS + off + c];
  }
}

__device__ __forceinline__ long long gather_src(const GatherArgs& a, long long r, int& k) {
  k = 0;
  if (a.nbuf > 1 && r >= a.start[1]) k = 1;
  if (a.nbuf > 2 && r >= a.start[2]) k = 2;
  if (a.idx[k] != nullptr) return a.idx[k][r - a.start[k]];
  const uint32_t call = (uint32_t)((a.counter ? a.counter[0] : 0) + a.call_offset[k]);
  const long long sz = a.size[k][0];
  return rng_index_at(a.seed[k], STREAM_SAMPLE, call, (uint64_t)(r - a.start[k]), (uint32_t)(sz > 0 ? sz : 1));
}

template <int P, int NQ>
__global__ __launch_bounds__(256) void k_gather_rows(GatherArgs a) {
  extern __shared__ __attribute__((aligned(16))) float stage[];
  constexpr int ROWS = ROWS_WG * P;
  const int lane = threadIdx.x & 15, g = threadIdx.x >> 4;
  if (blockIdx.x == 0 && threadIdx.x == 0)
    for (int k = 0; k < a.nbump; ++k) a.bump[k][0] += 1;
  const long long row0 = (long long)blockIdx.x * ROWS;
  const long long N = a.start[a.nbuf];
  const int S = a.S, A = a.A, WS = a.WS, nq = WS >> 2;
  const float* mine = nullptr;
  if (lane < P) {
    const long long r = min(row0 + ROWS_WG * lane + g, N - 1);
    int k;
    const long long src = gather_src(a, r, k);
    mine = a.bufs[k].state + src * a.bufs[k].pitch;
  }
  typedef float v4f __attribute__((ext_vector_type(4)));
  typedef const __attribute__((address_space(1))) v4f* gptr_t;
  v4f v[P][NQ];
#pragma unroll
  for (int p = 0; p < P; ++p) {
    const unsigned long long up = (unsigned long long)mine;
    const unsigned lo = (unsigned)__shfl((int)(unsigned)up, (threadIdx.x & 48) + p, 64), hi = (unsigned)__shfl((int)(unsigned)(up >> 32), (threadIdx.x & 48) + p, 64);
    gptr_t rp = (gptr_t)(((unsigned long long)hi << 32) | lo);
#pragma unroll
    for (int j = 0; j < NQ; ++j) v[p][j] = rp[min(lane + 16 * j, nq - 1)];
  }
#pragma unroll
  for (int p = 0; p < P; ++p)
#pragma unroll
    for (int j = 0; j < NQ; ++j)
      if (lane + 16 * j < nq) reinterpret_cast<v4f*>(stage + (ROWS_WG * p + g) * WS)[lane + 16 * j] = v[p][j];
  __syncthreads();
  const int rows = (int)min((long long)ROWS, N - row0);
  stage_to_batch(stage, WS, 0, S, rows, a.state + row0 * S);
  stage_to_batch(stage, WS, S, A, rows, a.action + row0 * A);
  stage_to_batch(stage, WS, S + A, S, rows, a.next_state + row0 * S);
  stage_to_batch(stage, WS, 2 * S + A, 1, rows, a.reward + row0);
  stage_to_batch(stage, WS, 2 * S + A + 1, 1, rows, a.not_done + row0);
}

__global__ __launch_bounds__(256) void k_gather(GatherArgs a) {
  extern __shared__ __attribute__((aligned(16))) float stage[];
  const int lane = threadIdx.x & 15, g = threadIdx.x >> 4;
  if (blockIdx.x == 0 && threadIdx.x == 0)
    for (int k = 0; k < a.nbump; ++k) a.bump[k][0] += 1;
  const long long row0 = (long long)blockIdx.x * ROWS_WG;
  const long long row = row0 + g;
  const long long N = a.start[a.nbuf];
  const bool ok = row < N;
  const long long r = ok ? row : 0;
  int k = 0;
  long long src = 0;
  if (lane == 0) src = gather_src(a, r, k);
  src = __shfl(src, threadIdx.x & 48, 64);
  k = __shfl(k, threadIdx.x & 48, 64);
  const int S = a.S, A = a.A, WS = a.WS;
  float* mine = stage + g * WS;
  if (ok) {
    const MobodyBufferView& b = a.bufs[k];
    if (a.packed[k]) {
      const float4* rp = reinterpret_cast<const float4*>(b.state + src * b.pitch);
      for (int q = lane; 4 * q < WS; q += 16) reinterpret_cast<float4*>(mine)[q] = rp[q];
    } else {
      const long long ps = b.pitch ? b.pitch : S, pa = b.pitch ? b.pitch : A, p1 = b.pitch ? b.pitch : 1;
      for (int c = lane; c < S; c += 16) {
        mine[c] = b.state[src * ps + c];
        mine[S + A + c] = b.next_state[src * ps + c];
      }
      for (int c = lane; c < A; c += 16) mine[S + c] = b.action[src * pa + c];
      if (lane == 0) mine[2 * S + A] = b.reward[src * p1];
      if (lane == 1) mine[2 * S + A + 1] = b.not_done[src * p1];
    }
  }
  __syncthreads();
  const int rows = (int)min((long long)ROWS_WG, N - row0);
  stage_to_batch(stage, WS, 0, S, rows, a.state + row0 * S);
  stage_to_batch(stage, WS, S, A, rows, a.action + row0 * A);
  stage_to_batch(stage, WS, S + A, S, rows, a.next_state + row0 * S);
  stage_to_batch(stage, WS, 2 * S + A, 1, rows, a.reward + row0);
  stage_to_batch(stage, WS, 2 * S + A + 1, 1, rows, a.not_done + row0);
}

template <int P, int NQ>
static void launch_gather_rows(const GatherArgs& a, long long N, hipStream_t st) {
  const size_t lds = (size_t)ROWS_WG * P * a.WS * sizeof(float);
  hipLaunchKernelGGL((k_gather_rows<P, NQ>), dim3((unsigned)cdiv(N, ROWS_WG * P)), dim3(256), lds, st, a);
}

static int launch_gather(const GatherArgs& a, long long N, hipStream_t st) {
  const size_t lds = (size_t)ROWS_WG * a.WS * sizeof(float);
  if (lds > 64 * 1024) return fail(MOBODY_E_ARG, "gather: rows of %d floats do not fit the LDS stage", a.WS);
  bool all_packed = true;
  for (int k = 0; k < a.nbuf; ++k) all_packed = all_packed && (a.packed[k] || a.start[k + 1] == a.start[k]);
  const int nq = (a.WS / 4 + 15) / 16;
  if (all_packed && nq <= 4) {
    if (nq == 1) launch_gather_rows<4, 1>(a, N, st);
    else if (nq == 2) launch_gather_rows<2, 2>(a, N, st);
    else if (nq == 3) launch_gather_rows<1, 3>(a, N, st);
    else launch_gather_rows<1, 4>(a, N, st);
    MB_LAUNCH_OK("k_gather_rows");
    return 0;
  }
  hipLaunchKernelGGL(k_gather, dim3((unsigned)cdiv(N, ROWS_WG)), dim3(256), lds, st, a);
  MB_LAUNCH_OK("k_gather");
  return 0;
}

constexpr int SCAN_PER_THREAD = 16;
constexpr int SCAN_BLOCK = 1024 * SCAN_PER_THREAD;

struct ScanArgs {
  const uint8_t* keep;
  long long M, cap;
  int32_t *pos, *tops, *meta;
  long long* ptr_size;
  int nblocks;
};

__device__ __forceinline__ int32_t block_scan_1024(int32_t v, int32_t* wtot) {
  const int lane = threadIdx.x & 63, w = threadIdx.x >> 6;
#pragma unroll
  for (int o = 1; o < 64; o <<= 1) {
    const int32_t u = __shfl_up(v, o, 64);
    if (lane >= o) v += u;
  }
  __syncthreads();
  if (lane == 63) wtot[w] = v;
  __syncthreads();
  int32_t before = 0;
#pragma unroll
  for (int k = 0; k < 15; ++k) before += (k < w) ? wtot[k] : 0;
  return v + before;
}

__global__ __launch_bounds__(1024) void k_scan_blocks(ScanArgs a) {
  __shared__ int32_t wtot[16];
  __shared__ int last;
  constexpr int T = SCAN_PER_THREAD;
  const long long i0 = (long long)blockIdx.x * SCAN_BLOCK + T * threadIdx.x;
  int32_t f[T];
  if (a.keep != nullptr && i0 + T <= a.M && ((reinterpret_cast<uintptr_t>(a.keep) & 15) == 0)) {
    const uint4 w = *reinterpret_cast<const uint4*>(a.keep + i0);
    const uint32_t ws[4] = {w.x, w.y, w.z, w.w};
#pragma unroll
    for (int j = 0; j < T; ++j) f[j] = ((ws[j >> 2] >> (8 * (j & 3))) & 0xffu) != 0;
  } else {
#pragma unroll
    for (int j = 0; j < T; ++j) f[j] = (i0 + j < a.M) ? (a.keep ? (a.keep[i0 + j] != 0) : 1) : 0;
  }
  int32_t mine4 = 0;
#pragma unroll
  for (int j = 0; j < T; ++j) mine4 += f[j];
  const int32_t inc = block_scan_1024(mine4, wtot);
  int32_t run = inc - mine4;
  if (i0 + T <= a.M) {
#pragma unroll
    for (int q = 0; q < T / 4; ++q) {
      int4 o;
      o.x = run; run += f[4 * q]; o.y = run; run += f[4 * q + 1]; o.z = run; run += f[4 * q + 2]; o.w = run; run += f[4 * q + 3];
      reinterpret_cast<int4*>(a.pos + i0)[q] = o;
    }
  } else {
#pragma unroll
    for (int j = 0; j < T; ++j) {
      if (i0 + j < a.M) a.pos[i0 + j] = run;
      run += f[j];
    }
  }
  if (threadIdx.x == 1023) {
    a.tops[blockIdx.x] = inc;
    __threadfence();
    last = atomicAdd(&a.meta[0], 1) == a.nblocks - 1;
  }
  __syncthreads();
  if (!last) return;
  __threadfence();
  const int32_t mine = (int)threadIdx.x < a.nblocks ? a.tops[threadIdx.x] : 0;
  const int32_t pre = block_scan_1024(mine, wtot);
  if ((int)threadIdx.x < a.nblocks) a.tops[threadIdx.x] = pre - mine;
  if (threadIdx.x == 1023) {
    const long long K = pre;
    const long long ptr = a.ptr_size[0], size = a.ptr_size[1];
    a.meta[1] = (int32_t)K;
    a.meta[2] = (int32_t)(ptr & 0xFFFFFFFFLL); a.meta[3] = (int32_t)(ptr >> 32);
    const long long end = (ptr + K < a.cap) ? ptr + K : a.cap;
    const long long used = end - ptr;
    long long nptr = end % a.cap;
    const long long nsize = size + used < a.cap ? size + used : a.cap;
    if (nptr == 0) nptr = K - used;
    a.ptr_size[0] = nptr;
    a.ptr_size[1] = nsize;
    a.meta[0] = 0;
  }
}

struct RingArgs {
  MobodyBufferView ring;
  int packed;
  long long cap;
  int S, A, WS;
  const float *obs, *act, *next_obs, *reward;
  const uint8_t *terminal, *keep;
  long long M;
  const int32_t *pos, *tops, *meta;
};

__device__ __forceinline__ long long ring_dst(long long j, long long ptr, long long K, long long cap) {
  const long long end = (ptr + K < cap) ? ptr + K : cap;
  const long long used = end - ptr;
  return j < used ? ptr + j : j - used;
}

__device__ __forceinline__ void batch_to_stage(float* stage, int WS, int off, int n, int rows, const float* in) {
  const uint32_t magic = div_magic(n);
  for (int e = threadIdx.x; e < rows * n; e += 256) {
    const int r = fast_div(e, magic, n), c = e - r * n;
    stage[r * WS + off + c] = in[e];
  }
}

constexpr int STAGE_U = 5;
struct StageRegs { float v[STAGE_U]; };
__device__ __forceinline__ void stage_ld(StageRegs& r, int n, int rows, const float* in) {
  const int total = rows * n;
#pragma unroll
  for (int u = 0; u < STAGE_U; ++u) r.v[u] = in[min((int)threadIdx.x + 256 * u, total - 1)];
}
__device__ __forceinline__ void stage_st(const StageRegs& r, float* stage, int WS, int off, int n, int rows, const float* in) {
  const uint32_t magic = div_magic(n);
  const int total = rows * n;
#pragma unroll
  for (int u = 0; u < STAGE_U; ++u) {
    const int e = threadIdx.x + 256 * u;
    if (e < total) { const int rr = fast_div(e, magic, n); stage[rr * WS + off + (e - rr * n)] = r.v[u]; }
  }
  for (int e = threadIdx.x + 256 * STAGE_U; e < total; e += 256) {
    const int rr = fast_div(e, magic, n);
    stage[rr * WS + off + (e - rr * n)] = in[e];
  }
}

template <int P>
__global__ __launch_bounds__(256) void k_ring_scatter(RingArgs a) {
  extern __shared__ __attribute__((aligned(16))) float stage[];
  const int lane = threadIdx.x & 15, g = threadIdx.x >> 4;
  const long long row0 = (long long)blockIdx.x * (ROWS_WG * P);
  const int S = a.S, A = a.A, WS = a.WS, W = 2 * S + A + 2;
  const int rows = (int)min((long long)ROWS_WG * P, a.M - row0);
  const long long base = a.tops[row0 / SCAN_BLOCK];
  const long long K = a.meta[1];
  const long long ptr = ((long long)(uint32_t)a.meta[2]) | ((long long)a.meta[3] << 32);
  int32_t pos[P];
  bool kept[P];
#pragma unroll
  for (int p = 0; p < P; ++p) {
    const long long i = row0 + ROWS_WG * p + g, ic = min(i, a.M - 1);
    pos[p] = a.pos[ic];
    kept[p] = i < a.M && (a.keep == nullptr || a.keep[ic] != 0);
  }
  StageRegs rs, ra, rn;
  stage_ld(rs, S, rows, a.obs + row0 * S);
  stage_ld(ra, A, rows, a.act + row0 * A);
  stage_ld(rn, S, rows, a.next_obs + row0 * S);
  const int tr = min((int)threadIdx.x, rows - 1);
  const float rew = a.reward[row0 + tr];
  const float ndone = 1.f - (float)(a.terminal[row0 + tr] != 0);
  stage_st(rs, stage, WS, 0, S, rows, a.obs + row0 * S);
  stage_st(ra, stage, WS, S, A, rows, a.act + row0 * A);
  stage_st(rn, stage, WS, S + A, S, rows, a.next_obs + row0 * S);
  if ((int)threadIdx.x < rows) { stage[threadIdx.x * WS + 2 * S + A] = rew; stage[threadIdx.x * WS + 2 * S + A + 1] = ndone; }
  for (int e = threadIdx.x; e < rows * (WS - W); e += 256) {
    const int r = e / (WS - W), c = e - r * (WS - W);
    stage[r * WS + W + c] = 0.f;
  }
  __syncthreads();
  const MobodyBufferView& b = a.ring;
#pragma unroll
  for (int p = 0; p < P; ++p) {
    if (!kept[p]) continue;
    const long long d = ring_dst(base + pos[p], ptr, K, a.cap);
    const float* mine = stage + (ROWS_WG * p + g) * WS;
    if (a.packed) {
      float4* rp = reinterpret_cast<float4*>(const_cast<float*>(b.state) + d * b.pitch);
      for (int q = lane; 4 * q < WS; q += 16) rp[q] = reinterpret_cast<const float4*>(mine)[q];
    } else {
      const long long ps = b.pitch ? b.pitch : S, pa = b.pitch ? b.pitch : A, p1 = b.pitch ? b.pitch : 1;
      float* bs = const_cast<float*>(b.state); float* bn = const_cast<float*>(b.next_state); float* ba = const_cast<float*>(b.action);
      for (int c = lane; c < S; c += 16) {
        bs[d * ps + c] = mine[c];
        bn[d * ps + c] = mine[S + A + c];
      }
      for (int c = lane; c < A; c += 16) ba[d * pa + c] = mine[S + c];
      if (lane == 0) const_cast<float*>(b.reward)[d * p1] = mine[2 * S + A];
      if (lane == 1) const_cast<float*>(b.not_done)[d * p1] = mine[2 * S + A + 1];
    }
  }
}

int launch_ring_append(const MobodyBufferView& ring, long long cap, long long* ptr_size, int S, int A, const float* obs,
                       const float* act, const float* next_obs, const float* reward, const uint8_t* terminal,
                       const uint8_t* keep, long long M, int32_t* scan_ws, hipStream_t st) {
  const int nblocks = (int)cdiv(M, SCAN_BLOCK);
  int32_t* meta = scan_ws;
  int32_t* tops = scan_ws + 8;
  int32_t* pos = scan_ws + 1040;
  ScanArgs sa{keep, M, cap, pos, tops, meta, ptr_size, nblocks};
  hipLaunchKernelGGL(k_scan_blocks, dim3(nblocks), dim3(1024), 0, st, sa);
  MB_LAUNCH_OK("k_scan_blocks");
  const int packed = view_packed(ring, S, A);
  const int WS = packed ? (int)ring.pitch : (2 * S + A + 2 + 3) & ~3;
  const int P = M >= 32768 && WS <= 64 ? 4 : 1;
  const size_t lds = (size_t)ROWS_WG * P * WS * sizeof(float);
  if (lds > 64 * 1024) return fail(MOBODY_E_ARG, "ring append: rows of %d floats do not fit the LDS stage", WS);
  RingArgs a{ring, packed, cap, S, A, WS, obs, act, next_obs, reward, terminal, keep, M, pos, tops, meta};
  if (P == 4) hipLaunchKernelGGL(k_ring_scatter<4>, dim3((unsigned)cdiv(M, ROWS_WG * 4)), dim3(256), lds, st, a);
  else hipLaunchKernelGGL(k_ring_scatter<1>, dim3((unsigned)cdiv(M, ROWS_WG)), dim3(256), lds, st, a);
  MB_LAUNCH_OK("k_ring_scatter");
  return 0;
}

static int check_view(const char* who, const MobodyBufferView& b, int S, int A) {
  MB_REQUIRE(b.state && b.action && b.next_state && b.reward && b.not_done, "%s: null pointer in a buffer view", who);
  MB_REQUIRE(b.pitch == 0 || b.pitch >= S, "%s: pitch %lld smaller than a state row", who, (long long)b.pitch);
  return 0;
}

}
using namespace mobody;

extern "C" int64_t mobody_ring_pitch(int S, int A) { return S >= 1 && A >= 1 ? ((2LL * S + A + 2 + 15) / 16) * 16 : -1; }

static int gather_common(const char* who, GatherArgs& a, const MobodyBufferView* bufs, const int64_t* counts, int nbuf, int S, int A,
                         float* state, float* action, float* next_state, float* reward, float* not_done, long long& N) {
  MB_REQUIRE(S >= 1 && A >= 1, "%s: bad dims", who);
  N = 0;
  for (int k = 0; k < nbuf; ++k) {
    MB_REQUIRE(counts[k] >= 0, "%s: negative count", who);
    if (counts[k] > 0) { int rc = check_view(who, bufs[k], S, A); if (rc) return rc; }
    a.bufs[k] = bufs[k]; a.packed[k] = view_packed(bufs[k], S, A); a.start[k] = N; N += counts[k];
  }
  a.start[nbuf] = N; a.nbuf = nbuf; a.S = S; a.A = A; a.WS = (2 * S + A + 2 + 3) & ~3;
  if (N == 0) return 0;
  MB_REQUIRE(state && action && next_state && reward && not_done, "%s: null output", who);
  a.state = state; a.action = action; a.next_state = next_state; a.reward = reward; a.not_done = not_done;
  return 0;
}

extern "C" int mobody_gather_batch(const MobodyBufferView* bufs, const int32_t* const* idx, const int64_t* counts,
                                   int nbuf, int S, int A, float* state, float* action, float* next_state,
                                   float* reward, float* not_done, void* stream) {
  MB_REQUIRE(bufs && idx && counts && nbuf >= 1 && nbuf <= 3, "mobody_gather_batch: need 1..3 source buffers");
  GatherArgs a{};
  long long N;
  int rc = gather_common("mobody_gather_batch", a, bufs, counts, nbuf, S, A, state, action, next_state, reward, not_done, N);
  if (rc || N == 0) return rc;
  for (int k = 0; k < nbuf; ++k) {
    MB_REQUIRE(counts[k] == 0 || idx[k], "mobody_gather_batch: null index array of source %d", k);
    a.idx[k] = idx[k];
  }
  return launch_gather(a, N, as_stream(stream));
}

extern "C" int mobody_ring_append(const MobodyBufferView* ring, int64_t cap, int64_t* ptr_size, int S, int A, const float* obs,
                                  const float* act, const float* next_obs, const float* reward,
                                  const uint8_t* terminal, const uint8_t* keep, int64_t M, int32_t* scan_ws,
                                  void* stream) {
  MB_REQUIRE(M >= 0 && cap >= 1, "mobody_ring_append: bad sizes");
  if (M == 0) return 0;
  MB_REQUIRE(M <= cap, "mobody_ring_append: batch of %lld rows overflows the ring of %lld twice (add_batch would raise)", (long long)M, (long long)cap);
  MB_REQUIRE(M <= (int64_t)SCAN_BLOCK * 1024, "mobody_ring_append: at most %d rows per call", SCAN_BLOCK * 1024);
  MB_REQUIRE(ring && ptr_size && obs && act && next_obs && reward && terminal && scan_ws, "mobody_ring_append: null pointer");
  MB_REQUIRE(S >= 1 && A >= 1, "mobody_ring_append: bad dims");
  int rc = check_view("mobody_ring_append", *ring, S, A);
  if (rc) return rc;
  return launch_ring_append(*ring, cap, (long long*)ptr_size, S, A, obs, act, next_obs, reward, terminal, keep, M, scan_ws,
                            as_stream(stream));
}

extern "C" int mobody_gather_batch_rng(const MobodyBufferView* bufs, const int64_t* counts, int nbuf, int S, int A,
                                       const uint32_t* seeds, const int64_t* call_offsets, const int64_t* counter,
                                       const int64_t* const* sizes, float* state, float* action, float* next_state,
                                       float* reward, float* not_done, int64_t* const* bump, int nbump, void* stream) {
  MB_REQUIRE(bufs && counts && seeds && call_offsets && sizes && nbuf >= 1 && nbuf <= 3, "mobody_gather_batch_rng: need 1..3 source buffers");
  MB_REQUIRE(nbump >= 0 && nbump <= 4 && (nbump == 0 || bump), "mobody_gather_batch_rng: at most 4 words to advance");
  GatherArgs a{};
  long long N;
  int rc = gather_common("mobody_gather_batch_rng", a, bufs, counts, nbuf, S, A, state, action, next_state, reward, not_done, N);
  if (rc || N == 0) return rc;
  for (int k = 0; k < nbuf; ++k) {
    MB_REQUIRE(counts[k] == 0 || sizes[k], "mobody_gather_batch_rng: null size word of source %d", k);
    a.idx[k] = nullptr; a.seed[k] = seeds[k]; a.call_offset[k] = call_offsets[k]; a.size[k] = (const long long*)sizes[k];
  }
  a.counter = (const long long*)counter;
  for (int k = 0; k < nbump; ++k) {
    MB_REQUIRE(bump[k] && bump[k] != counter, "mobody_gather_batch_rng: bump word %d is null or the call counter itself", k);
    a.bump[k] = (long long*)bump[k];
  }
  a.nbump = nbump;
  return launch_gather(a, N, as_stream(stream));
}
```

### mobody-model-based-off-dynamics-offline-reinforcement-learning_amd/csrc/train.hip

```cpp
#include <math.h>

#include "common.h"
#include "layers.h"
#include "train.h"

namespace mobody {

struct TrainWs {
  uint32_t *mq1, *mq2, *ma1, *ma2;
  int *eh1q, *eh1a, *edz2;
  float *pin;
  float *pi, *qt, *q, *qb, *xq, *h1q, *h2q, *xa, *h1a, *h2a, *dz3q, *dz2, *dz1, *dz3a, *dxa, *bcw, *dbp, *slabs, *lossp;
  long long total;
  int nsplit_q, nsplit_a, ntiles;
  MobodyMlpLayout Lq, La;
};

static int carve(const MobodyTrainDims& d, float* base, TrainWs& w) {
  int rc = mobody_mlp_layout(d.S + d.A, 1, 2, &w.Lq);
  if (rc) return rc;
  rc = mobody_mlp_layout(d.S, d.A, 1, &w.La);
  if (rc) return rc;
  const long long N = d.N, Nt = d.Nt;
  const long long N32 = (N + 31) & ~31LL;
// ... 48 lines not shown
  const int w = threadIdx.x >> 6, nw = blockDim.x >> 6;
  __syncthreads();
  if ((threadIdx.x & 63) == 0) sm[w] = v;
  __syncthreads();
  float s = 0.f;
  for (int k = 0; k < nw; ++k) s += sm[k];
  return s;
}

__global__ __launch_bounds__(1024) void k_actor_stats(const float* qp, const float* qb, long long N, long long Nt,
                                                      float* stats) {
  __shared__ float sm[16];
  constexpr int U = 4;
  float s0 = 0.f, s1 = 0.f;
  for (long long base = threadIdx.x; base < N; base += U * 1024) {
    float a[U], b[U];
#pragma unroll
    for (int u = 0; u < U; ++u) { const long long r = base + u * 1024; const long long rc = r < N ? r : 0; a[u] = qp[rc]; b[u] = qp[N + rc]; }
#pragma unroll
    for (int u = 0; u < U; ++u) if (base + u * 1024 < N) s0 += fabsf(fminf(a[u], b[u]));
  }
  for (long long base = threadIdx.x; base < Nt; base += U * 1024) {
    float a[U], b[U];
#pragma unroll
    for (int u = 0; u < U; ++u) { const long long r = base + u * 1024; const long long rc = r < Nt ? r : 0; a[u] = qb[rc]; b[u] = qb[Nt + rc]; }
#pragma unroll
    for (int u = 0; u < U; ++u) if (base + u * 1024 < Nt) s1 += fabsf(fminf(a[u], b[u]));
  }
  s0 = block_sum(s0, sm);
  s1 = block_sum(s1, sm);
  if (threadIdx.x == 0) { stats[0] = s0; stats[1] = s1; }
}

__global__ __launch_bounds__(256) void k_v_loss(const float* qt, const float* v, long long N, float invNg, int Np3,
                                                float* dz3, float* lossp) {
  __shared__ float sm[4];
  const long long row = (long long)blockIdx.x * blockDim.x + threadIdx.x;
  float l = 0.f;
  if (row < N) {
    const float adv = fminf(qt[row], qt[N + row]) - v[row];
    const float w = fabsf(0.7f - (adv < 0.f ? 1.f : 0.f));
    l = w * adv * adv;
    float* o = dz3 + row * Np3;
    o[0] = -2.f * w * adv * invNg;
    for (int c = 1; c < Np3; ++c) o[c] = 0.f;
  }
  l = block_sum(l, sm);
  if (threadIdx.x == 0) lossp[blockIdx.x] = l;
}
__global__ __launch_bounds__(256) void k_sum_scale(const float* parts, int n, float scale, float* out) {
  __shared__ float sm[4];
  float s = 0.f;
  for (int k = threadIdx.x; k < n; k += blockDim.x) s += parts[k];
  s = block_sum(s, sm);
  if (threadIdx.x == 0) out[0] = s * scale;
}

__global__ __launch_bounds__(256) void k_adam(AdamTarget a, const float* g, long long n, MobodyMlpLayout L) {
  __shared__ float adam_sm[2];
  adam_block_consts(a, adam_sm);
  const long long j = (long long)blockIdx.x * blockDim.x + threadIdx.x;
  if (j >= n || (health_mask(a) != 0 && health_foreign(a))) return;
  adam_element(a, L, j, g[j], adam_sm);
}

int launch_adam(const AdamTarget& a, const float* g, const MobodyMlpLayout& L, hipStream_t st) {
  hipLaunchKernelGGL(k_adam, dim3((unsigned)cdiv(L.total_floats, 256)), dim3(256), 0, st, a, g, (long long)L.total_floats, L);
  MB_LAUNCH_OK("k_adam");
  return 0;
}

__global__ __launch_bounds__(256) void k_mlp_transpose(MobodyMlpLayout L, const float* blob, float* bt, int precision, int* health) {
  const long long j = (long long)blockIdx.x * blockDim.x + threadIdx.x;
  if (j >= L.t_total_floats) return;
  const int m = (int)(j / L.t_member_floats);
  const long long o = j - (long long)m * L.t_member_floats;
  const float* src = blob + (long long)m * L.member_floats;
  if (o >= L.w2p) {
    if (o >= L.w2p + HID * HID) return;
    const int e = (int)(o - L.w2p), k = e / HID, n = e % HID;
    const float w = src[L.w2 + wide_idx(k, n)];
    write_w2_planes(bt + (long long)m * L.t_member_floats, L, k, n, w, precision);
    if (precision == 4) {
      short* tm = reinterpret_cast<short*>(bt + (long long)m * L.t_member_floats);
      tm[2 * L.w2p + bf_plane_idx(2, k, n)] = 0; tm[2 * L.w2tp + bf_plane_idx(2, n, k)] = 0;
      health_check_f16(health, w);
    }
    return;
  }
  float val;
  if (o < L.w1t) {
    const bool is3 = o < L.w2t;
    const long long oo = is3 ? o : o - L.w2t;
    const long long g = oo >> 2;
    const int kk = (int)(g / HID) * 4 + (int)(oo & 3), c = (int)(g % HID);
    val = is3 ? src[L.w3 + (long long)c * L.Np3 + kk] : src[L.w2 + wide_idx(c, kk)];
  } else {
    const long long oo = o - L.w1t;
    const int n = (int)(oo / L.Np1t), k = (int)(oo % L.Np1t);
    val = k < L.Kp1 ? src[L.w1 + wide_idx(k, n)] : 0.f;
  }
  bt[j] = val;
}

static Mlp3FwdArgs fwd_args(const float* blob, const MobodyMlpLayout& L, const float* s0, int n0, const float* s1, int n1,
                            long long rows, float* out, int out_mode, float max_action, float* sx, float* sh1,
                            float* sh2, uint32_t* m1 = nullptr, uint32_t* m2 = nullptr, const float* blob_T = nullptr,
                            int* e1 = nullptr) {
  Mlp3FwdArgs a = fwd_net(blob, L, rows);
  if (blob_T != nullptr) fwd_set_planes(a, blob_T, L);
  fwd_set_src(a, 0, s0, n0, n0);
  fwd_set_src(a, 1, s1, n1, s1 ? n1 : 0);
  fwd_set_out(a, out, out_mode, max_action);
  fwd_set_saves(a, sx, 0, sh1, e1, sh2, m1, m2);
  return a;
}

static int weight_grads(const MobodyMlpLayout& L, const float* x, const float* h1, const float* h2, const float* dz3,
                        const float* dz2, const float* dz1, long long rows, const TrainWs& w, float* grad,
                        const LossFinal& loss, const AdamTarget& adam, hipStream_t st, int prec = 0, const int* e_h1 = nullptr) {
  return mlp3_weight_grads(L, x, 0, h1, h2, dz3, dz2, dz1, rows, L.members == 1 ? w.nsplit_a : w.nsplit_q, w.slabs, w.dbp,
                           w.ntiles, grad, loss, adam, st, prec, prec == PREC_F16X2 ? e_h1 : nullptr, prec == PREC_F16X2 ? w.edz2 : nullptr);
}

static Mlp3BwdArgs bwd_args(const MobodyMlpLayout& L, const float* blob_T, const float* dz3, const float* h1,
                            const float* h2, long long rows, float* dz2, float* dz1, float* dbp,
                            const uint32_t* m1 = nullptr, const uint32_t* m2 = nullptr, int prec = PREC_F32, int* e2 = nullptr) {
  Mlp3BwdArgs b = bwd_net(L, blob_T, rows);
  bwd_set_planes(b, L, prec);
  bwd_set_acts(b, h1, h2, m1, m2, 0);
  bwd_set_grads(b, dz3, dz2, dz1, dbp, prec == PREC_F16X2 ? e2 : nullptr);
  return b;
}

}

using namespace mobody;

extern "C" int64_t mobody_train_workspace(const MobodyTrainDims* d) {
  if (check_dims(d, "mobody_train_workspace")) return -1;
  TrainWs w;
  if (carve(*d, nullptr, w)) return -1;
  return w.total;
}

static AdamTarget adam_target(float* blob, float* blob_T, float* m, float* v, float* target, int64_t t, const int64_t* t_dev,
                              float lr, float tau, float grad_scale, int precision);

static int critic_impl(const MobodyTrainDims* d, const MobodyHyper* h, const float* actor_blob, const float* actor_blob_T,
                       const float* q_blob, const float* q_blob_T, const float* qtarg_blob, const float* qtarg_blob_T,
                       const float* state, const float* action,
                       const float* next_state, const float* reward, const float* not_done, const float* q_next,
                       float* grad_q, const AdamTarget& adam, float* loss_out, float* workspace, int policy_forward,
                       void* stream, int phase = 0) {
  int rc = check_dims(d, "mobody_critic_step");
  if (rc) return rc;
  MB_REQUIRE(h && q_blob && q_blob_T && state && action && reward && not_done && (grad_q || adam.on) && loss_out && workspace,
             "mobody_critic_step: null pointer");
  MB_REQUIRE(q_next || (actor_blob && qtarg_blob && next_state), "mobody_critic_step: need q_next or actor/target/next_state");
  rc = check_precision("mobody_critic_step", h->precision, q_next != nullptr || (actor_blob_T && qtarg_blob_T));
  if (rc) return rc;
  const int prec = h->precision;
  const float *aT = prec != PREC_F32 ? actor_blob_T : nullptr, *qT = prec != PREC_F32 ? q_blob_T : nullptr, *tT = prec != PREC_F32 ? qtarg_blob_T : nullptr;
  TrainWs w;
  rc = carve(*d, workspace, w);
  if (rc) return rc;
  hipStream_t st = as_stream(stream);
  const long long N = d->N;
  const int S = d->S, A = d->A;
  const Mlp3FwdArgs fq = fwd_args(q_blob, w.Lq, state, S, action, A, N, w.q, 0, 1.f, w.xq, w.h1q, w.h2q, w.mq1, w.mq2, qT,
                                  prec == PREC_F16X2 ? w.eh1q : nullptr);
  if (phase == 2) {
  } else if (q_next == nullptr) {
    rc = launch_mlp3_forward(fq, 2, fwd_args(actor_blob, w.La, next_state, S, nullptr, 0, N, w.pin, 1, h->max_action, nullptr, nullptr, nullptr, nullptr, nullptr, aT), 1, ACT_RELU, prec, st);
    const Mlp3FwdArgs ft = fwd_args(qtarg_blob, w.Lq, next_state, S, w.pin, A, N, w.qt, 0, 1.f, nullptr, nullptr, nullptr, nullptr, nullptr, tT);
    if (!rc && policy_forward)
      rc = launch_mlp3_forward(ft, 2, fwd_args(actor_blob, w.La, state, S, nullptr, 0, N, w.pi, 1, h->max_action, w.xa, w.h1a, w.h2a, w.ma1, w.ma2, aT,
                                               prec == PREC_F16X2 ? w.eh1a : nullptr), 1, ACT_RELU, prec, st);
    else if (!rc)
      rc = launch_mlp3_forward(ft, 2, ACT_RELU, prec, st);
  } else {
    rc = launch_mlp3_forward(fq, 2, ACT_RELU, prec, st);
  }
  if (rc || phase == 1) return rc;
  const float invNg = 1.f / (float)d->N_global;
  Mlp3BwdArgs bq = bwd_args(w.Lq, q_blob_T, w.dz3q, w.h1q, w.h2q, N, w.dz2, w.dz1, w.dbp, w.mq1, w.mq2, prec, w.edz2);
  bq.seed.mode = 1; bq.seed.q = w.q; bq.seed.qt = w.qt; bq.seed.qnext = q_next; bq.seed.r = reward; bq.seed.nd = not_done;
  bq.seed.gamma = h->gamma; bq.seed.inv_ng = invNg; bq.seed.dz3_out = w.dz3q; bq.seed.lossp = w.lossp;
  rc = launch_mlp3_bwd(bq, 2, false, st);
  if (rc) return rc;
  LossFinal lf{};
  lf.kind = 1; lf.nparts = 2 * w.ntiles; lf.scale = invNg; lf.parts = w.lossp; lf.out = loss_out;
  return weight_grads(w.Lq, w.xq, w.h1q, w.h2q, w.dz3q, w.dz2, w.dz1, N, w, grad_q, lf, adam, st, prec, w.eh1q);
}

extern "C" int mobody_critic_step(const MobodyTrainDims* d, const MobodyHyper* h, const float* actor_blob,
                                  const float* actor_blob_T, const float* q_blob, const float* q_blob_T,
                                  const float* qtarg_blob, const float* qtarg_blob_T, const float* state,
                                  const float* action, const float* next_state, const float* reward, const float* not_done,
                                  const float* q_next, float* grad_q, float* loss_out, float* workspace, int policy_forward,
                                  void* stream) {
  MB_REQUIRE(grad_q, "mobody_critic_step: grad_q is null");
  return critic_impl(d, h, actor_blob, actor_blob_T, q_blob, q_blob_T, qtarg_blob, qtarg_blob_T, state, action, next_state, reward,
                     not_done, q_next, grad_q, AdamTarget{}, loss_out, workspace, policy_forward, stream);
}

extern "C" int mobody_critic_update(const MobodyTrainDims* d, const MobodyHyper* h, const float* actor_blob,
                                    const float* actor_blob_T, float* q_blob, float* q_blob_T, float* qtarg_blob,
                                    float* qtarg_blob_T, const float* state, const float* action, const float* next_state,
                                    const float* reward, const float* not_done, const float* q_next, float* m, float* v,
                                    int64_t t, const int64_t* t_dev, float lr, float* loss_out, float* workspace,
                                    int policy_forward, int64_t* bump, void* stream) {
  MB_REQUIRE(h && q_blob && q_blob_T && qtarg_blob && m && v, "mobody_critic_update: null pointer");
  MB_REQUIRE(t_dev != nullptr || t >= 1, "mobody_critic_update: step t must be >= 1");
  MB_REQUIRE(bump == nullptr || bump != t_dev, "mobody_critic_update: bump must not be the step word the launch reads");
  AdamTarget at = adam_target(q_blob, q_blob_T, m, v, qtarg_blob, t, t_dev, lr, h->tau, 1.f, h->precision);
  at.target_T = qtarg_blob_T;
  at.bump = (long long*)bump;
  return critic_impl(d, h, actor_blob, actor_blob_T, q_blob, q_blob_T, qtarg_blob, qtarg_blob_T, state, action, next_state, reward,
                     not_done, q_next, nullptr, at, loss_out, workspace, policy_forward, stream);
}

extern "C" int mobody_critic_update_phase(const MobodyTrainDims* d, const MobodyHyper* h, const float* actor_blob,
                                          const float* actor_blob_T, float* q_blob, float* q_blob_T, float* qtarg_blob,
                                          float* qtarg_blob_T, const float* state, const float* action, const float* next_state,
                                          const float* reward, const float* not_done, const float* q_next, float* m, float* v,
                                          int64_t t, const int64_t* t_dev, float lr, float* loss_out, float* workspace,
                                          int policy_forward, int64_t* bump, int phase, void* stream) {
  MB_REQUIRE(h && q_blob && q_blob_T && qtarg_blob && m && v, "mobody_critic_update_phase: null pointer");
  MB_REQUIRE(phase == 1 || phase == 2, "mobody_critic_update_phase: phase is 1 (forwards) or 2 (backward + update)");
  MB_REQUIRE(t_dev != nullptr || t >= 1, "mobody_critic_update_phase: step t must be >= 1");
  MB_REQUIRE(bump == nullptr || bump != t_dev, "mobody_critic_update_phase: bump must not be the step word the launch reads");
  AdamTarget at = adam_target(q_blob, q_blob_T, m, v, qtarg_blob, t, t_dev, lr, h->tau, 1.f, h->precision);
  at.target_T = qtarg_blob_T;
  at.bump = (long long*)bump;
  return critic_impl(d, h, actor_blob, actor_blob_T, q_blob, q_blob_T, qtarg_blob, qtarg_blob_T, state, action, next_state, reward,
                     not_done, q_next, nullptr, at, loss_out, workspace, policy_forward, stream, phase);
}

extern "C" int mobody_actor_forward(const MobodyTrainDims* d, const MobodyHyper* h, const float* actor_blob,
                                    const float* actor_blob_T, const float* q_blob, const float* q_blob_T,
                                    const float* state, const float* action, float* stats, float* workspace, int policy_ready,
                                    void* stream) {
  int rc = check_dims(d, "mobody_actor_forward");
  if (rc) return rc;
  MB_REQUIRE(h && actor_blob && q_blob && state && action && stats && workspace, "mobody_actor_forward: null pointer");
  rc = check_precision("mobody_actor_forward", h->precision, actor_blob_T && q_blob_T);
  if (rc) return rc;
  const int prec = h->precision;
  const float *aT = prec != PREC_F32 ? actor_blob_T : nullptr, *qT = prec != PREC_F32 ? q_blob_T : nullptr;
  TrainWs w;
  rc = carve(*d, workspace, w);
  if (rc) return rc;
  hipStream_t st = as_stream(stream);
  const long long N = d->N, Nt = d->Nt;
  const int S = d->S, A = d->A;
  const Mlp3FwdArgs fb = fwd_args(q_blob, w.Lq, state, S, action, A, Nt, w.qb, 0, 1.f, nullptr, nullptr, nullptr, nullptr, nullptr, qT);
  const Mlp3FwdArgs fp = fwd_args(q_blob, w.Lq, state, S, w.pi, A, N, w.q, 0, 1.f, nullptr, nullptr, nullptr, w.mq1, w.mq2, qT);
  if (policy_ready) {
    rc = launch_mlp3_forward(fb, 2, fp, 2, ACT_RELU, prec, st);
  } else {
    rc = launch_mlp3_forward(fb, 2, fwd_args(actor_blob, w.La, state, S, nullptr, 0, N, w.pi, 1, h->max_action, w.xa, w.h1a, w.h2a, w.ma1, w.ma2, aT,
                                             prec == PREC_F16X2 ? w.eh1a : nullptr), 1, ACT_RELU, prec, st);
    if (!rc) rc = launch_mlp3_forward(fp, 2, ACT_RELU, prec, st);
  }
  if (rc) return rc;
  hipLaunchKernelGGL(k_actor_stats, dim3(1), dim3(1024), 0, st, w.q, w.qb, N, Nt, stats);
  MB_LAUNCH_OK("k_actor_stats");
  return 0;
}

static int actor_backward_impl(const MobodyTrainDims* d, const MobodyHyper* h, const float* actor_blob,
                               const float* actor_blob_T, const float* q_blob, const float* q_blob_T, const float* state,
                               const float* action, const float* stats, const float* v_true, float* grad_actor,
                               const AdamTarget& adam, float* loss_out, float* workspace, void* stream) {
  int rc = check_dims(d, "mobody_actor_backward");
  if (rc) return rc;
  MB_REQUIRE(h && actor_blob && actor_blob_T && q_blob && q_blob_T && state && action && stats && (grad_actor || adam.on) &&
                 loss_out && workspace, "mobody_actor_backward: null pointer");
  rc = check_precision("mobody_actor_backward", h->precision, true);
  if (rc) return rc;
  TrainWs w;
  rc = carve(*d, workspace, w);
  if (rc) return rc;
  hipStream_t st = as_stream(stream);
  const long long N = d->N;
  ActorRowArgs ra{};
  ra.qp = w.q; ra.qb = w.qb; ra.stats = stats; ra.pi = w.pi; ra.act = action; ra.dxa = w.dxa; ra.v_true = v_true;
  ra.bcw = w.bcw; ra.N = N; ra.Nt = d->Nt; ra.Ng = d->N_global; ra.Ntg = d->Nt_global > 0 ? d->Nt_global : 1;
  ra.A = d->A; ra.h = *h;
  Mlp3BwdArgs bq = bwd_args(w.Lq, q_blob_T, nullptr, nullptr, nullptr, N, nullptr, nullptr, w.dbp, w.mq1, w.mq2, h->precision);
  bq.seed.mode = 2; bq.seed.ar = ra;
  bq.dx = w.dxa; bq.dx_c0 = d->S; bq.dx_n = d->A;
  rc = launch_mlp3_bwd(bq, 2, true, st);
  if (rc) return rc;
  Mlp3BwdArgs ba = bwd_args(w.La, actor_blob_T, w.dz3a, w.h1a, w.h2a, N, w.dz2, w.dz1, w.dbp, w.ma1, w.ma2, h->precision, w.edz2);
  ba.seed.mode = 3; ba.seed.ar = ra; ba.seed.dz3_out = w.dz3a; ba.seed.lossp = w.lossp;
  rc = launch_mlp3_bwd(ba, 1, false, st);
  if (rc) return rc;
  LossFinal lf{};
  lf.kind = 2; lf.nparts = w.ntiles; lf.scale_q = h->scale_q; lf.weight = h->weight; lf.bc_coef = h->bc_coef;
  lf.ng = (float)ra.Ng; lf.ntg_a = (float)ra.Ntg * (float)ra.A; lf.parts = w.lossp; lf.stats = stats; lf.out = loss_out;
  return weight_grads(w.La, w.xa, w.h1a, w.h2a, w.dz3a, w.dz2, w.dz1, N, w, grad_actor, lf, adam, st, h->precision, w.eh1a);
}

extern "C" int mobody_actor_backward(const MobodyTrainDims* d, const MobodyHyper* h, const float* actor_blob,
                                     const float* actor_blob_T, const float* q_blob, const float* q_blob_T,
                                     const float* state, const float* action, const float* stats, const float* v_true,
                                     float* grad_actor, float* loss_out, float* workspace, void* stream) {
  MB_REQUIRE(grad_actor, "mobody_actor_backward: grad_actor is null");
  return actor_backward_impl(d, h, actor_blob, actor_blob_T, q_blob, q_blob_T, state, action, stats, v_true, grad_actor,
                             AdamTarget{}, loss_out, workspace, stream);
}

extern "C" int mobody_actor_update(const MobodyTrainDims* d, const MobodyHyper* h, float* actor_blob, float* actor_blob_T,
                                   const float* q_blob, const float* q_blob_T, const float* state, const float* action,
                                   const float* stats, const float* v_true, float* m, float* v, int64_t t,
                                   const int64_t* t_dev, float lr, float* loss_out, float* workspace, void* stream) {
  MB_REQUIRE(actor_blob && actor_blob_T && m && v, "mobody_actor_update: null pointer");
  MB_REQUIRE(t_dev != nullptr || t >= 1, "mobody_actor_update: step t must be >= 1");
  return actor_backward_impl(d, h, actor_blob, actor_blob_T, q_blob, q_blob_T, state, action, stats, v_true, nullptr,
                             adam_target(actor_blob, actor_blob_T, m, v, nullptr, t, t_dev, lr, -1.f, 1.f, h ? h->precision : 0), loss_out,
                             workspace, stream);
}

extern "C" int mobody_mlp_transpose(int in_dim, int out_dim, int members, const float* blob, float* blob_T, int precision,
                                    void* stream) {
  MobodyMlpLayout L;
  int rc = mobody_mlp_layout(in_dim, out_dim, members, &L);
  if (rc) return rc;
  MB_REQUIRE(blob && blob_T, "mobody_mlp_transpose: null pointer");
  rc = check_precision("mobody_mlp_transpose", precision, true);
  if (rc) return rc;
  hipLaunchKernelGGL(k_mlp_transpose, dim3((unsigned)cdiv(L.t_total_floats, 256)), dim3(256), 0, as_stream(stream), L, blob, blob_T,
                     precision, health_words());
  MB_LAUNCH_OK("k_mlp_transpose");
  return 0;
}

static AdamTarget adam_target(float* blob, float* blob_T, float* m, float* v, float* target, int64_t t, const int64_t* t_dev,
                              float lr, float tau, float grad_scale, int precision) {
  const double tt = t_dev ? 1.0 : (double)t;
  const double bc1 = 1.0 - pow(0.9, tt), bc2 = 1.0 - pow(0.999, tt);
  AdamTarget a{};
  a.p = blob; a.m = m; a.v = v; a.blob_T = blob_T;
  a.target = (target != nullptr && tau >= 0.f) ? target : nullptr;
  a.c.step_size = (float)((double)lr / bc1); a.c.bc2_sqrt = (float)sqrt(bc2);
  a.c.tau = tau; a.c.one_minus_tau = (float)(1.0 - (double)tau); a.c.gscale = grad_scale;
  a.t_dev = (const long long*)t_dev; a.lr = lr; a.on = 1; a.precision = precision;
  a.health = health_words(); a.health_tag = a.health ? health_next_tag() : 0; a.t_host = (int)t;
  return a;
}

static int adam_impl(int in_dim, int out_dim, int members, float* blob, float* blob_T, const float* grad, float* m,
                     float* v, float* target, float* target_T, int64_t t, const int64_t* t_dev, float lr, float tau,
                     float grad_scale, int precision, void* stream) {
  MobodyMlpLayout L;
  int rc = mobody_mlp_layout(in_dim, out_dim, members, &L);
  if (rc) return rc;
  MB_REQUIRE(blob && grad && m && v, "mobody_adam_polyak: null pointer");
  MB_REQUIRE(t_dev != nullptr || t >= 1, "mobody_adam_polyak: step t must be >= 1");
  rc = check_precision("mobody_adam_polyak", precision, true);
  if (rc) return rc;
  AdamTarget a = adam_target(blob, blob_T, m, v, target, t, t_dev, lr, tau, grad_scale, precision);
  a.target_T = a.target ? target_T : nullptr;
  hipStream_t st = as_stream(stream);
  hipLaunchKernelGGL(k_adam, dim3((unsigned)cdiv(L.total_floats, 256)), dim3(256), 0, st, a, grad, (long long)L.total_floats, L);
  MB_LAUNCH_OK("k_adam");
  return 0;
}

extern "C" int mobody_adam_polyak(int in_dim, int out_dim, int members, float* blob, float* blob_T, const float* grad,
                                  float* m, float* v, float* target, float* target_T, int64_t t, float lr, float tau,
// ... 48 lines not shown
```

### mobody-model-based-off-dynamics-offline-reinforcement-learning_amd/engine.py

```python
import torch

from . import ops, packing


def default_config(S, A, **over):
    cfg = dict(gamma=0.99, tau=0.005, update_interval=2, state_dim=S, action_dim=A, penalty_type="none",
               hidden_sizes=256, max_action=1.0, critic_lr=3e-4, actor_lr=3e-4, gaussian_noise_std=1.0,
               penalize_fake=0, src_ratio=1, trg_ratio=1, src_rollout_length=1, trg_rollout_length=1,
               use_src_sa_to_get_target_next_state=1, env_filter=10.0, rollout_from_src=0, fake_batch_scale=0.5,
               advantage=0, scale_Q=1, weight=2.5, bc_coef=1.0, q_weighted=1, filter_bad_rollout=1,
               penalty_coef=0.1, mopo=0, latent_reward=0, encoder_loss_coef=1, domain_loss_coef=0.0,
               cycle_loss_coef=0.3)
    cfg.update(over)
    return cfg


class Engine:

    def __init__(self, S, A, pa, pq, dev):
        self.ops, self.packing, self.S, self.A, self.dev = ops, packing, S, A, dev
        self.actor = packing.pack_mlp([{k[len("network."):]: v for k, v in pa.items()}], S, A, dev)
        self.q = packing.pack_mlp(pq, S + A, 1, dev, prefixes=["network1.", "network2."])
        self.qt = self.q.clone()
        self.prec = ops.prec_id(ops.default_mfma())
        self.actor_T = ops.mlp_transpose(self.actor, S, A, 1, precision=self.prec)
        self.q_T = ops.mlp_transpose(self.q, S + A, 1, 2, precision=self.prec)
        self.qt_T = self.q_T.clone()
        z = torch.zeros_like
        self.ma, self.va, self.mq, self.vq = z(self.actor), z(self.actor), z(self.q), z(self.q)
        self.ga, self.gq = z(self.actor), z(self.q)
        self.t = 0
        self.loss = torch.zeros(4, device=dev)
        self.stats = torch.zeros(2, device=dev)

    def step(self, batch, n_true, cfg, apply=True, dims=None):
        ops = self.ops
        S, A = self.S, self.A
        b = [torch.as_tensor(x, dtype=torch.float32).to(self.dev).contiguous() for x in batch]
        N = b[0].shape[0]
        dims = dims or ops.train_dims(S, A, N, n_true)
        hyp = ops.hyper(cfg)
        if (hyp.precision == 4) != (self.prec == 4):
            ops.mlp_transpose(self.actor, S, A, 1, out=self.actor_T, precision=hyp.precision)
            ops.mlp_transpose(self.q, S + A, 1, 2, out=self.q_T, precision=hyp.precision)
            ops.mlp_transpose(self.qt, S + A, 1, 2, out=self.qt_T, precision=hyp.precision)
        self.prec = hyp.precision
        ws = ops.train_workspace(dims, self.dev)
        ops.critic_step(dims, hyp, self.actor, self.q, self.q_T, self.qt, b, self.gq, self.loss[0:1], ws,
                        actor_blob_T=self.actor_T, qtarg_blob_T=self.qt_T)
        if apply:
            self.t += 1
            ops.adam_polyak(S + A, 1, 2, self.q, self.q_T, self.gq, self.mq, self.vq, self.qt, self.t, cfg["critic_lr"], cfg["tau"],
                            target_T=self.qt_T, precision=self.prec)
        ops.actor_forward(dims, hyp, self.actor, self.q, b[0], b[1], self.stats, ws, actor_blob_T=self.actor_T, q_blob_T=self.q_T)
        ops.actor_backward(dims, hyp, self.actor, self.actor_T, self.q, self.q_T, b[0], b[1], self.stats, self.ga,
                           self.loss[1:3], ws)
        if apply:
            ops.adam_polyak(S, A, 1, self.actor, self.actor_T, self.ga, self.ma, self.va, None, self.t, cfg["actor_lr"],
                            precision=self.prec)
        torch.cuda.synchronize()
        return dict(q_loss=float(self.loss[0]), pi_loss=float(self.loss[1]), bc_loss=float(self.loss[2]))

    def unpack(self, blob, which):
        if which == "actor":
            return {"network." + k: v for k, v in self.packing.unpack_mlp(blob, self.S, self.A, 1)[0].items()}
        ms = self.packing.unpack_mlp(blob, self.S + self.A, 1, 2)
        return {f"network{j + 1}." + k: v for j in range(2) for k, v in ms[j].items()}
```

### mobody-model-based-off-dynamics-offline-reinforcement-learning_amd/ops.py

```python
import ctypes as C

import torch

from . import _lib
from ._lib import check, cur_stream, load, ptr


def _f32(t, device=None):
    t = torch.as_tensor(t, dtype=torch.float32)
    if device is not None:
        t = t.to(device)
    return t.contiguous()


def rng_normal(seed, stream_id, call, n, device):
    out = torch.empty(n, dtype=torch.float32, device=device)
    check(load().mobody_rng_normal(seed, stream_id, call, n, ptr(out), cur_stream()), "mobody_rng_normal")
    return out


def rng_index(seed, stream_id, call, n, bound, device):
    out = torch.empty(n, dtype=torch.int32, device=device)
    check(load().mobody_rng_index(seed, stream_id, call, n, bound, ptr(out), cur_stream()), "mobody_rng_index")
    return out
# ... 60 lines not shown


def health_bound(device=None):
    idx = torch.cuda.current_device() if device is None or torch.device(device).index is None else torch.device(device).index
    return _health_blocks.get(idx)


def health_clear():
    check(load().mobody_health_clear(cur_stream()), "mobody_health_clear")


def health_read(words=None):
    w = words if words is not None else _health_blocks.get(torch.cuda.current_device())
    if w is None:
        return 0, 0
    h = w[:2].tolist()
    return int(h[0]), int(h[1])


def health_bits(mask):
    return [n for n, b in (("F16_RANGE", _lib.HEALTH_F16_RANGE), ("NONFINITE", _lib.HEALTH_NONFINITE)) if mask & b]


def _mlp_w2(blob, L, members):
    return blob[:members * L.member_floats].view(members, L.member_floats)[:, L.w2:L.w2 + 65536]


def dyn_planes(blob, S, A, out=None, precision=3):
    if prec_id(precision) == 4:
        L = _lib.dyn_layout(S, A)
        lays = [L.layer[_lib.DL_NAMES.index(n)] for n in ("zs2", "transition2", "reward_model2")]
        _check_f16_weights([blob[y.w_off:y.w_off + L.E * y.Kp * y.Np] for y in lays], "dyn_planes")
    pl = out if out is not None else torch.empty(load().mobody_dyn_planes_floats(), dtype=torch.float32, device=blob.device)
    check(load().mobody_dyn_planes(ptr(blob), S, A, ptr(pl), prec_id(precision), cur_stream()), "mobody_dyn_planes")
    return pl


def dyn_forward(blob, S, A, obs, act, use_trg=True, planes=None, precision=0):
    obs, act = _f32(obs), _f32(act)
    B = obs.shape[0]
    mean = torch.empty(7, B, S, dtype=torch.float32, device=obs.device)
    check(load().mobody_dyn_forward(ptr(blob), ptr(planes), prec_id(precision), S, A, ptr(obs), ptr(act), B, int(use_trg),
                                    ptr(mean), cur_stream()), "mobody_dyn_forward")
    return mean


def dyn_step(blob, S, A, task_id, obs, act, noise=None, elite_idx=None, alive=None, elites=(0, 1, 2, 3, 4), seed=0,
             call=0, penalty_coef=0.0, use_penalty=True, use_trg=True, want_mean=False, workspace=None, out=None,
             planes=None, precision=0, mopo=None, call_dev=None, uncertainty_mode=0):
    obs, act = _f32(obs), _f32(act)
    dev, B = obs.device, obs.shape[0]
    if noise is not None:
        noise = _f32(noise, dev)
        assert noise.shape == (7, B, S)
    if elite_idx is not None:
        elite_idx = torch.as_tensor(elite_idx).to(device=dev, dtype=torch.int32).contiguous()
    need = load().mobody_dyn_step_workspace(S, A, B)
    if workspace is None or workspace.numel() < need:
        workspace = torch.empty(max(need, 1), dtype=torch.float32, device=dev)
    o = out or {}
    nxt = o.get("next_obs", None)
    if nxt is None:
        nxt = torch.empty(B, S, dtype=torch.float32, device=dev)
    rew = o["reward"] if "reward" in o else torch.empty(B, 1, dtype=torch.float32, device=dev)
    term = o["terminal"] if "terminal" in o else torch.empty(B, 1, dtype=torch.uint8, device=dev)
    pen = o["penalty"] if "penalty" in o else torch.empty(B, 1, dtype=torch.float32, device=dev)
    raw = o["raw_reward"] if "raw_reward" in o else torch.empty(B, 1, dtype=torch.float32, device=dev)
    mean = torch.empty(7, B, S, dtype=torch.float32, device=dev) if want_mean else None
    el = (C.c_int32 * len(elites))(*[int(e) for e in elites])
    mb, mbt = mopo if mopo is not None else (None, None)
    a = _lib.MobodyEnsStep(C.sizeof(_lib.MobodyEnsStep), unc_id(uncertainty_mode), ptr(blob), ptr(planes), ptr(mb), ptr(mbt),
                           prec_id(precision), S, A, task_id, ptr(obs), ptr(act), B, ptr(noise), ptr(elite_idx), ptr(alive),
                           el, len(elites), seed, call, int(bool(use_penalty)), ptr(call_dev), float(penalty_coef),
                           int(bool(use_trg)), ptr(nxt), ptr(rew), ptr(term), ptr(pen), ptr(raw), ptr(mean), ptr(workspace))
    check(load().mobody_ens_step(C.byref(a), cur_stream()), "mobody_ens_step")
    res = dict(next_obs=nxt, reward=rew, terminal=term, penalty=pen, raw_reward=raw)
    if want_mean:
        res["mean"] = mean
    return res


def mlp3_forward(blob, in_dim, out_dim, members, src0, src1=None, out_mode=0, max_action=1.0, save=False, blob_T=None,
                 precision=0):
    src0 = _f32(src0)
    rows, n0 = src0.shape
    n1 = 0
    if src1 is not None:
        src1 = _f32(src1)
        n1 = src1.shape[1]
    dev = src0.device
    out = torch.empty(members, rows, out_dim, dtype=torch.float32, device=dev)
    sx = sh1 = sh2 = None
    if save:
        L = _lib.mlp_layout(in_dim, out_dim, members)
        sx = torch.empty(rows, L.Kp1, dtype=torch.float32, device=dev)
        sh1 = torch.empty(members, rows, 256, dtype=torch.float32, device=dev)
        sh2 = torch.empty(members, rows, 256, dtype=torch.float32, device=dev)
    check(load().mobody_mlp3_forward(ptr(blob), ptr(blob_T), prec_id(precision), in_dim, out_dim, members, ptr(src0), n0, ptr(src1), n1, rows, out_mode,
                                     float(max_action), ptr(out), ptr(sx), ptr(sh1), ptr(sh2), cur_stream()),
          "mobody_mlp3_forward")
    return (out, sx, sh1, sh2) if save else out


def train_dims(S, A, N, Nt, N_global=None, Nt_global=None):
    return _lib.MobodyTrainDims(S, A, N, Nt, N if N_global is None else N_global, Nt if Nt_global is None else Nt_global)


def hyper(cfg):
    return _lib.MobodyHyper(float(cfg["gamma"]), float(cfg["tau"]), float(cfg["max_action"]), float(cfg["weight"]),
                            float(cfg["bc_coef"]), int(bool(cfg["q_weighted"])), int(bool(cfg["scale_Q"])),
                            prec_id(cfg.get("mfma", default_mfma())))


def train_workspace(dims, device):
    n = load().mobody_train_workspace(C.byref(dims))
    if n < 0:
        raise _lib.MobodyError("mobody_train_workspace: " + load().mobody_last_error().decode())
    return torch.empty(n, dtype=torch.float32, device=device)


def mlp_transpose(blob, in_dim, out_dim, members, out=None, precision=0):
    L = _lib.mlp_layout(in_dim, out_dim, members)
    if prec_id(precision) == 4:
        _check_f16_weights([_mlp_w2(blob, L, members)], "mlp_transpose")
    bt = out if out is not None else torch.empty(L.t_total_floats, dtype=torch.float32, device=blob.device)
    assert bt.numel() == L.t_total_floats
    check(load().mobody_mlp_transpose(in_dim, out_dim, members, ptr(blob), ptr(bt), prec_id(precision), cur_stream()),
          "mobody_mlp_transpose")
    return bt


def critic_step(dims, hyp, actor_blob, q_blob, q_blob_T, qtarg_blob, batch, grad_q, loss_out, ws, q_next=None,
                policy_forward=False, actor_blob_T=None, qtarg_blob_T=None):
    s, a, s2, r, nd = batch
    check(load().mobody_critic_step(C.byref(dims), C.byref(hyp), ptr(actor_blob), ptr(actor_blob_T), ptr(q_blob), ptr(q_blob_T),
                                    ptr(qtarg_blob), ptr(qtarg_blob_T), ptr(s), ptr(a), ptr(s2), ptr(r), ptr(nd), ptr(q_next), ptr(grad_q),
                                    ptr(loss_out), ptr(ws), int(bool(policy_forward)), cur_stream()), "mobody_critic_step")


def actor_forward(dims, hyp, actor_blob, q_blob, state, action, stats, ws, policy_ready=False, actor_blob_T=None, q_blob_T=None):
    check(load().mobody_actor_forward(C.byref(dims), C.byref(hyp), ptr(actor_blob), ptr(actor_blob_T), ptr(q_blob), ptr(q_blob_T), ptr(state),
                                      ptr(action), ptr(stats), ptr(ws), int(bool(policy_ready)), cur_stream()),
          "mobody_actor_forward")


def actor_backward(dims, hyp, actor_blob, actor_blob_T, q_blob, q_blob_T, state, action, stats, grad_actor, loss_out,
                   ws, v_true=None):
    check(load().mobody_actor_backward(C.byref(dims), C.byref(hyp), ptr(actor_blob), ptr(actor_blob_T), ptr(q_blob),
                                       ptr(q_blob_T), ptr(state), ptr(action), ptr(stats), ptr(v_true), ptr(grad_actor),
                                       ptr(loss_out), ptr(ws), cur_stream()), "mobody_actor_backward")


def critic_update(dims, hyp, actor_blob, q_blob, q_blob_T, qtarg_blob, batch, m, v, t, lr, loss_out, ws, q_next=None,
                  t_dev=None, policy_forward=False, actor_blob_T=None, qtarg_blob_T=None, bump=None, phase=0):
    s, a, s2, r, nd = batch
    args = (C.byref(dims), C.byref(hyp), ptr(actor_blob), ptr(actor_blob_T), ptr(q_blob), ptr(q_blob_T),
            ptr(qtarg_blob), ptr(qtarg_blob_T), ptr(s), ptr(a), ptr(s2), ptr(r), ptr(nd), ptr(q_next), ptr(m),
            ptr(v), int(t), ptr(t_dev), float(lr), ptr(loss_out), ptr(ws), int(bool(policy_forward)), ptr(bump))
    if phase:
        check(load().mobody_critic_update_phase(*args, int(phase), cur_stream()), "mobody_critic_update_phase")
    else:
        check(load().mobody_critic_update(*args, cur_stream()), "mobody_critic_update")


def actor_update(dims, hyp, actor_blob, actor_blob_T, q_blob, q_blob_T, state, action, stats, m, v, t, lr, loss_out, ws,
                 v_true=None, t_dev=None):
    check(load().mobody_actor_update(C.byref(dims), C.byref(hyp), ptr(actor_blob), ptr(actor_blob_T), ptr(q_blob),
                                     ptr(q_blob_T), ptr(state), ptr(action), ptr(stats), ptr(v_true), ptr(m), ptr(v),
                                     int(t), ptr(t_dev), float(lr), ptr(loss_out), ptr(ws), cur_stream()),
          "mobody_actor_update")


def value_loss_grad(qt, v, n_global):
    N = v.numel()
    dz3 = torch.empty(N, 16, dtype=torch.float32, device=v.device)
    loss = torch.empty(1, dtype=torch.float32, device=v.device)
    lossp = torch.empty((N + 255) // 256, dtype=torch.float32, device=v.device)
    check(load().mobody_value_loss_grad(ptr(qt), ptr(v), N, int(n_global), ptr(dz3), ptr(loss), ptr(lossp), cur_stream()),
          "mobody_value_loss_grad")
    return dz3, loss


def adam_polyak(in_dim, out_dim, members, blob, blob_T, grad, m, v, target, t, lr, tau=-1.0, grad_scale=1.0, target_T=None,
                precision=0):
    check(load().mobody_adam_polyak(in_dim, out_dim, members, ptr(blob), ptr(blob_T), ptr(grad), ptr(m), ptr(v),
                                    ptr(target), ptr(target_T), int(t), float(lr), float(tau), float(grad_scale),
                                    prec_id(precision), cur_stream()),
          "mobody_adam_polyak")


class RingView:

    def __init__(self, store, S, A):
        assert store.is_contiguous() and store.dtype == torch.float32 and store.shape[1] >= 2 * S + A + 2
        self.store, self.S, self.A = store, int(S), int(A)
        self.device = store.device

    def fields(self):
        S, A, st = self.S, self.A, self.store
        return st[:, :S], st[:, S:S + A], st[:, S + A:2 * S + A], st[:, 2 * S + A:2 * S + A + 1], st[:, 2 * S + A + 1:2 * S + A + 2]

    def __iter__(self):
        return iter(self.fields())

    def __getitem__(self, k):
        return self.fields()[k]


def ring_pitch(S, A):
    return int(load().mobody_ring_pitch(int(S), int(A)))


def buffer_view(b):
    if isinstance(b, RingView):
        base, S, A = b.store.data_ptr(), b.S, b.A
        return _lib.MobodyBufferView(base, base + 4 * S, base + 4 * (S + A), base + 4 * (2 * S + A), base + 4 * (2 * S + A + 1), b.store.shape[1])
    return _lib.MobodyBufferView(*[ptr(t) for t in b], 0)


def _view_device(b):
    return b.device if isinstance(b, RingView) else b[0].device


def gather_batch(buffers, indices, S, A, out=None):
    n = len(buffers)
    dev = _view_device(buffers[0])
    views = (_lib.MobodyBufferView * n)(*[buffer_view(b) for b in buffers])
    idx = [i.to(device=dev, dtype=torch.int32).contiguous() for i in indices]
    iptr = (C.c_void_p * n)(*[ptr(i) if i.numel() else None for i in idx])
    cnt = (C.c_int64 * n)(*[i.numel() for i in idx])
    N = sum(i.numel() for i in idx)
    if out is None:
        out = (torch.empty(N, S, device=dev), torch.empty(N, A, device=dev), torch.empty(N, S, device=dev),
               torch.empty(N, 1, device=dev), torch.empty(N, 1, device=dev))
    check(load().mobody_gather_batch(views, iptr, cnt, n, S, A, *[ptr(t) for t in out], cur_stream()),
          "mobody_gather_batch")
    return out


_scan_ws = {}


def ring_append(buf, cap, ptr_size, S, A, obs, act, next_obs, reward, terminal, keep=None):
    M = obs.shape[0]
    if M == 0:
        return
    dev = obs.device
    scan = _scan_ws.get(dev)
    if scan is None or scan.numel() < M + 1040:
        scan = _scan_ws[dev] = torch.zeros(max(M + 1040, 2 * (scan.numel() if scan is not None else 0)), dtype=torch.int32, device=dev)
    check(load().mobody_ring_append(C.byref(buffer_view(buf)), cap, ptr(ptr_size), S, A, ptr(obs), ptr(act), ptr(next_obs),
                                    ptr(reward), ptr(terminal), ptr(keep), M, ptr(scan), cur_stream()),
          "mobody_ring_append")


def termination(task_id, next_obs):
    B, S = next_obs.shape
    done = torch.empty(B, 1, dtype=torch.uint8, device=next_obs.device)
    check(load().mobody_termination(task_id, ptr(next_obs), B, S, ptr(done), cur_stream()), "mobody_termination")
    return done


def rollout_mask(alive_in, terminal, penalty, env_filter, use_filter, keep, alive_out):
    B = terminal.shape[0]
    check(load().mobody_rollout_mask(ptr(alive_in), ptr(terminal), ptr(penalty), float(env_filter), int(bool(use_filter)),
                                     B, ptr(keep), ptr(alive_out), cur_stream()), "mobody_rollout_mask")


def sample_indices(seed, stream_id, counter, call_offset, n, size_dev, out=None):
    if out is None:
        out = torch.empty(n, dtype=torch.int32, device=size_dev.device)
    check(load().mobody_sample_indices(seed, stream_id, ptr(counter), call_offset, n, ptr(size_dev), ptr(out),
                                       cur_stream()), "mobody_sample_indices")
    return out


def counter_add(counter, inc=1):
    check(load().mobody_counter_add(ptr(counter), counter.numel(), inc, cur_stream()), "mobody_counter_add")


def par_penalty(next_state_true, next_state_model, reward, coef):
    n, S = next_state_true.shape
    check(load().mobody_par_penalty(ptr(next_state_true), ptr(next_state_model), ptr(reward), float(coef), n, S,
                                    cur_stream()), "mobody_par_penalty")


def adam_polyak_dev(in_dim, out_dim, members, blob, blob_T, grad, m, v, target, t_dev, lr, tau=-1.0, grad_scale=1.0,
                    target_T=None, precision=0):
    check(load().mobody_adam_polyak_dev(in_dim, out_dim, members, ptr(blob), ptr(blob_T), ptr(grad), ptr(m), ptr(v),
                                        ptr(target), ptr(target_T), ptr(t_dev), float(lr), float(tau), float(grad_scale),
                                        prec_id(precision), cur_stream()), "mobody_adam_polyak_dev")


def gather_batch_rng(buffers, counts, seeds, call_offsets, counter, sizes, S, A, out, bump=()):
    n = len(buffers)
    views = (_lib.MobodyBufferView * n)(*[buffer_view(b) for b in buffers])
    cnt = (C.c_int64 * n)(*[int(c) for c in counts])
    sd = (C.c_uint32 * n)(*[int(s) & 0xFFFFFFFF for s in seeds])
    off = (C.c_int64 * n)(*[int(o) for o in call_offsets])
    sz = (C.c_void_p * n)(*[ptr(s) for s in sizes])
    bp = (C.c_void_p * max(1, len(bump)))(*[ptr(t) for t in bump])
    check(load().mobody_gather_batch_rng(views, cnt, n, S, A, sd, off, ptr(counter), sz, *[ptr(t) for t in out], bp, len(bump),
                                         cur_stream()), "mobody_gather_batch_rng")
    return out


def mlp3_backward(blob_T, in_dim, out_dim, members, dz3, x, h1, h2, grad, ws=None):
    rows = x.shape[0]
    need = load().mobody_mlp3_backward_workspace(in_dim, out_dim, members, rows)
    if ws is None or ws.numel() < need:
        ws = torch.empty(need, dtype=torch.float32, device=x.device)
    check(load().mobody_mlp3_backward(ptr(blob_T), in_dim, out_dim, members, ptr(dz3), ptr(x), ptr(h1), ptr(h2), rows,
                                      ptr(grad), ptr(ws), cur_stream()), "mobody_mlp3_backward")
    return ws


def dara_inputs(s, a, s2, std, noise_sas=None, noise_sa=None, seed=0, call=0):
    N, S = s.shape
    A = a.shape[1]
    x_sas = torch.empty(N, 2 * S + A, dtype=torch.float32, device=s.device)
    x_sa = torch.empty(N, S + A, dtype=torch.float32, device=s.device)
    check(load().mobody_dara_inputs(ptr(s), ptr(a), ptr(s2), N, S, A, float(std), ptr(noise_sas), ptr(noise_sa), seed,
                                    call, ptr(x_sas), ptr(x_sa), cur_stream()), "mobody_dara_inputs")
    return x_sas, x_sa


def dara_loss_grad(z_sas, z_sa, n_src, labels=None):
    N = z_sas.shape[0]
    dev = z_sas.device
    dz_sas = torch.empty(N, 16, dtype=torch.float32, device=dev)
    dz_sa = torch.empty(N, 16, dtype=torch.float32, device=dev)
    loss = torch.empty(2, dtype=torch.float32, device=dev)
    lossp = torch.empty(2 * ((N + 255) // 256), dtype=torch.float32, device=dev)
    if labels is not None:
        labels = torch.as_tensor(labels).to(device=dev, dtype=torch.int32).contiguous()
    check(load().mobody_dara_loss_grad(ptr(z_sas), ptr(z_sa), ptr(labels), N, int(n_src), ptr(dz_sas), ptr(dz_sa),
                                       ptr(loss), ptr(lossp), cur_stream()), "mobody_dara_loss_grad")
    return dz_sas, dz_sa, loss


def dara_penalty(z_sas, z_sa, coef, reward=None, want_delta=False):
    n = z_sas.shape[0]
    delta = torch.empty(n, 1, dtype=torch.float32, device=z_sas.device) if want_delta or reward is None else None
    check(load().mobody_dara_penalty(ptr(z_sas), ptr(z_sa), n, float(coef), ptr(reward), ptr(delta), cur_stream()),
          "mobody_dara_penalty")
    return delta


def pretrain_transpose(blob, S, A, out=None, precision=0):
    L = _lib.pretrain_layout(S, A)
    if prec_id(precision) == 4:
        _check_f16_weights([_mlp_w2(blob[L.off_enc:], L.enc, 7), _mlp_w2(blob[L.off_tr:], L.tr, 7),
                            _mlp_w2(blob[L.off_rw:], L.rw, 7)], "pretrain_transpose")
    bt = out if out is not None else torch.zeros(L.t_total_floats, dtype=torch.float32, device=blob.device)
    check(load().mobody_pretrain_transpose(S, A, ptr(blob), ptr(bt), prec_id(precision), cur_stream()), "mobody_pretrain_transpose")
    return bt


def pretrain_workspace(S, A, b, device):
    n = load().mobody_pretrain_workspace(S, A, b)
    if n < 0:
        raise _lib.MobodyError("mobody_pretrain_workspace: " + load().mobody_last_error().decode())
    return torch.empty(n, dtype=torch.float32, device=device)


def pretrain_gather(state, action, next_state, reward, idx, start, b, out=None, start_dev=None):
    S, A = state.shape[1], action.shape[1]
    dev = state.device
    assert idx.dtype == torch.int32 and idx.dim() == 2 and idx.shape[0] == 7 and idx.is_contiguous()
    xenc, act, rew = out or (torch.empty(7, 2 * b, S, dtype=torch.float32, device=dev),
                             torch.empty(7, b, A, dtype=torch.float32, device=dev),
                             torch.empty(7, b, dtype=torch.float32, device=dev))
    check(load().mobody_pretrain_gather(ptr(state), ptr(action), ptr(next_state), ptr(reward), ptr(idx), idx.shape[1], start,
                                        ptr(start_dev), b, S, A, ptr(xenc), ptr(act), ptr(rew), cur_stream()),
          "mobody_pretrain_gather")
    return xenc, act, rew


def pretrain_grads(S, A, b, use_trg, encoder_loss_coef, blob, blob_T, xenc, act, rew, grad, loss_out, ws, noise6=None,
                   noise7=None, seed=0, call=0, b_global=None, precision=0, transition_coef=1.0, reward_coef=1.0):
    check(load().mobody_pretrain_grads(S, A, b, b if b_global is None else b_global, int(bool(use_trg)),
                                       float(encoder_loss_coef), ptr(blob), ptr(blob_T), ptr(xenc), ptr(act), ptr(rew),
                                       ptr(noise6), ptr(noise7), seed, call, ptr(grad), ptr(loss_out), ptr(ws),
                                       prec_id(precision), float(transition_coef), float(reward_coef), cur_stream()), "mobody_pretrain_grads")


def pretrain_update(S, A, b, use_trg, encoder_loss_coef, blob, blob_T, xenc, act, rew, m, v, t_main, t_za, lr, loss_out, ws,
                    noise6=None, noise7=None, seed=0, call=0, call_dev=None, t_dev=None, precision=0, loss_acc=None):
    check(load().mobody_pretrain_update(S, A, b, int(bool(use_trg)), float(encoder_loss_coef), ptr(blob), ptr(blob_T), ptr(xenc),
                                        ptr(act), ptr(rew), ptr(noise6), ptr(noise7), seed, call, ptr(call_dev), ptr(m), ptr(v),
                                        t_main, t_za, ptr(t_dev), float(lr), ptr(loss_out), ptr(loss_acc), ptr(ws), prec_id(precision), cur_stream()),
          "mobody_pretrain_update")


def pretrain_adam(S, A, use_trg, blob, blob_T, grad, m, v, t_main, t_za, lr, grad_scale=1.0, precision=0, net_mask=7, t_rw=None):
    check(load().mobody_pretrain_adam(S, A, int(bool(use_trg)), ptr(blob), ptr(blob_T), ptr(grad), ptr(m), ptr(v), t_main,
                                      t_za, float(lr), float(grad_scale), prec_id(precision), int(net_mask),
                                      t_main if t_rw is None else t_rw, cur_stream()), "mobody_pretrain_adam")


def pretrain_za_adam(S, A, use_trg, blob, grad, m, v, t_za, lr, grad_scale=1.0):
    check(load().mobody_pretrain_za_adam(S, A, int(bool(use_trg)), ptr(blob), ptr(grad), ptr(m), ptr(v), t_za, float(lr),
                                         float(grad_scale), cur_stream()), "mobody_pretrain_za_adam")


def pretrain_mopo_transpose(blob, S, A, out=None, precision=0):
    L = _lib.pretrain_mopo_layout(S, A)
    if prec_id(precision) == 4:
        _check_f16_weights([_mlp_w2(blob[L.off_dyn:], L.dyn, 7), _mlp_w2(blob[L.off_rw:], L.rw, 7)], "pretrain_mopo_transpose")
    bt = out if out is not None else torch.zeros(L.t_total_floats, dtype=torch.float32, device=blob.device)
    check(load().mobody_pretrain_mopo_transpose(S, A, ptr(blob), ptr(bt), prec_id(precision), cur_stream()),
          "mobody_pretrain_mopo_transpose")
    return bt


def pretrain_mopo_workspace(S, A, b, device):
    n = load().mobody_pretrain_mopo_workspace(S, A, b)
    if n < 0:
        raise _lib.MobodyError("mobody_pretrain_mopo_workspace: " + load().mobody_last_error().decode())
    return torch.empty(n, dtype=torch.float32, device=device)


def pretrain_mopo_grads(S, A, b, use_trg, encoder_loss_coef, blob, blob_T, xenc, act, rew, grad, loss_out, ws, noise=None,
                        seed=0, call=0, b_global=None, precision=0):
    check(load().mobody_pretrain_mopo_grads(S, A, b, b if b_global is None else b_global, int(bool(use_trg)),
                                            float(encoder_loss_coef), ptr(blob), ptr(blob_T), ptr(xenc), ptr(act), ptr(rew),
                                            ptr(noise), seed, call, ptr(grad), ptr(loss_out), ptr(ws), prec_id(precision),
                                            cur_stream()), "mobody_pretrain_mopo_grads")


def pretrain_mopo_update(S, A, b, use_trg, encoder_loss_coef, blob, blob_T, xenc, act, rew, m, v, t, lr, loss_out, ws,
                         noise=None, seed=0, call=0, call_dev=None, t_dev=None, precision=0, loss_acc=None):
    check(load().mobody_pretrain_mopo_update(S, A, b, int(bool(use_trg)), float(encoder_loss_coef), ptr(blob), ptr(blob_T),
                                             ptr(xenc), ptr(act), ptr(rew), ptr(noise), seed, call, ptr(call_dev), ptr(m),
                                             ptr(v), t, ptr(t_dev), float(lr), ptr(loss_out), ptr(loss_acc), ptr(ws),
                                             prec_id(precision), cur_stream()), "mobody_pretrain_mopo_update")


def pretrain_mopo_adam(S, A, blob, blob_T, grad, m, v, t, lr, grad_scale=1.0, precision=0):
    check(load().mobody_pretrain_mopo_adam(S, A, ptr(blob), ptr(blob_T), ptr(grad), ptr(m), ptr(v), t, float(lr),
                                           float(grad_scale), prec_id(precision), cur_stream()), "mobody_pretrain_mopo_adam")


def dyn_validate_mopo(blob, mopo_blob, S, A, obs, act, next_obs, rew, ws=None):
# ... 45 lines not shown
```

Before: 47.28 million.

## Fuse minibatch gather into the critic's first forward MLP launch

Adds a critic update entry point whose first forward kernel (Q on (s,a) plus policy on s') samples ring-buffer rows directly with the device RNG. It loads them into LDS and writes the gathered minibatch out for later kernels, instead of running a separate gather kernel first. This removes one launch and one round trip of the minibatch through global memory per step. In exchange it adds per-tile index generation and shuffle-based row loads inside the forward kernel, and it is limited to packed ring views without PAR/DARA penalty or advantage mode.

```diff
diff --git a/include/mobody_hip.h b/include/mobody_hip.h
--- a/include/mobody_hip.h
+++ b/include/mobody_hip.h
@@ -207,6 +207,24 @@
                                const float* action, const float* next_state, const float* reward, const float* not_done,
                                const float* q_next, float* m, float* v, int64_t t, const int64_t* t_dev, float lr, float* loss_out,
                                float* workspace, int policy_forward, int64_t* bump, int phase, void* stream);
+
+typedef struct MobodyGatherRng {
+  const MobodyBufferView* bufs;
+  const int64_t* counts;
+  int nbuf;
+  const uint32_t* seeds;
+  const int64_t* call_offsets;
+  const int64_t* counter;
+  const int64_t* const* sizes;
+  int64_t* const* bump;
+  int nbump;
+} MobodyGatherRng;
+int mobody_critic_update_gather(const MobodyTrainDims* d, const MobodyHyper* h, const float* actor_blob, const float* actor_blob_T,
+                                float* q_blob, float* q_blob_T, float* qtarg_blob, float* qtarg_blob_T, float* state,
+                                float* action, float* next_state, float* reward, float* not_done, const float* q_next,
+                                float* m, float* v, int64_t t, const int64_t* t_dev, float lr, float* loss_out,
+                                float* workspace, int policy_forward, int64_t* bump, int phase, const MobodyGatherRng* gr,
+                                void* stream);
 
 int mobody_actor_update(const MobodyTrainDims* d, const MobodyHyper* h, float* actor_blob, float* actor_blob_T,
                         const float* q_blob, const float* q_blob_T, const float* state, const float* action,
diff --git a/mobody-model-based-off-dynamics-offline-reinforcement-learning_amd/_lib.py b/mobody-model-based-off-dynamics-offline-reinforcement-learning_amd/_lib.py
--- a/mobody-model-based-off-dynamics-offline-reinforcement-learning_amd/_lib.py
+++ b/mobody-model-based-off-dynamics-offline-reinforcement-learning_amd/_lib.py
@@ -53,6 +53,12 @@
 class MobodyHyper(C.Structure):
     _fields_ = [("gamma", f32), ("tau", f32), ("max_action", f32), ("weight", f32), ("bc_coef", f32),
                 ("q_weighted", i32), ("scale_q", i32), ("precision", i32)]
+
+
+class MobodyGatherRng(C.Structure):
+    _fields_ = [("bufs", C.POINTER(MobodyBufferView)), ("counts", C.POINTER(i64)), ("nbuf", C.c_int), ("seeds", C.POINTER(u32)),
+                ("call_offsets", C.POINTER(i64)), ("counter", vp), ("sizes", C.POINTER(vp)), ("bump", C.POINTER(vp)),
+                ("nbump", C.c_int)]
 
 
 class MobodyEnsStep(C.Structure):
@@ -126,6 +132,9 @@
                                      vp, vp, vp, vp, vp, vp, C.c_int, vp]),
     "mobody_critic_update": (C.c_int, [C.POINTER(MobodyTrainDims), C.POINTER(MobodyHyper), vp, vp, vp, vp, vp, vp, vp, vp, vp,
                                        vp, vp, vp, vp, vp, i64, vp, f32, vp, vp, C.c_int, vp, vp]),
+    "mobody_critic_update_gather": (C.c_int, [C.POINTER(MobodyTrainDims), C.POINTER(MobodyHyper), vp, vp, vp, vp, vp, vp, vp, vp, vp,
+                                              vp, vp, vp, vp, vp, i64, vp, f32, vp, vp, C.c_int, vp, C.c_int,
+                                              C.POINTER(MobodyGatherRng), vp]),
     "mobody_critic_update_phase": (C.c_int, [C.POINTER(MobodyTrainDims), C.POINTER(MobodyHyper), vp, vp, vp, vp, vp, vp, vp, vp, vp,
                                              vp, vp, vp, vp, vp, i64, vp, f32, vp, vp, C.c_int, vp, C.c_int, vp]),
     "mobody_actor_update": (C.c_int, [C.POINTER(MobodyTrainDims), C.POINTER(MobodyHyper), vp, vp, vp, vp, vp, vp, vp,
diff --git a/mobody-model-based-off-dynamics-offline-reinforcement-learning_amd/algo/offline_offline/mobody.py b/mobody-model-based-off-dynamics-offline-reinforcement-learning_amd/algo/offline_offline/mobody.py
--- a/mobody-model-based-off-dynamics-offline-reinforcement-learning_amd/algo/offline_offline/mobody.py
+++ b/mobody-model-based-off-dynamics-offline-reinforcement-learning_amd/algo/offline_offline/mobody.py
@@ -464,8 +464,14 @@
             self.actor_stats(b, N, Nt, Ng, Ntg)
 
         def fused_step():
-            ops.gather_batch_rng([rb._fields() for rb in bufs], cnts, seeds, [1] * len(bufs), c[0:1],
-                                 [rb.ptr_size[1:2] for rb in bufs], S, A, b, bump=(c[1:2], c[2:3], c[3:4]))
+            gather = dict(buffers=[rb._fields() for rb in bufs], counts=cnts, seeds=seeds, call_offsets=[1] * len(bufs),
+                          counter=c[0:1], sizes=[rb.ptr_size[1:2] for rb in bufs], bump=(c[1:2], c[2:3], c[3:4]))
+            if self._gather_in_forward(gather["buffers"]):
+                self.critic_update(b, N, Nt, t_dev=c[1:2], bump=c[0:1], gather=gather)
+                self.actor_stats(b, N, Nt, N, Nt)
+                self.actor_update(b, N, Nt, t_dev=c[2:3])
+                return
+            ops.gather_batch_rng(S=S, A=A, out=b, **gather)
             if par and not cfg["advantage"] and int(cfg.get("par_overlap", 1)):
                 main = torch.cuda.current_stream()
                 if getattr(self, "_side_stream", None) is None:
@@ -509,6 +515,11 @@
                 actor_apply()
             return [whole_step]
         return [critic, critic_apply_actor_stats, actor, actor_apply]
+
+    def _gather_in_forward(self, views):
+        return bool(int(self.config.get("fused_gather", 1)) and self.penalty_type not in ("par", "dara")
+                    and not self.config["advantage"] and self.rng == "device"
+                    and all(isinstance(v, ops.RingView) for v in views))
 
     def _graph_step(self, src, tar, batch_size):
         world = self._world()
@@ -706,7 +717,7 @@
     def _policy_rides_along(self):
         return not self.config["advantage"]
 
-    def critic_update(self, b, N, Nt, t_dev=None, bump=None, phase=0):
+    def critic_update(self, b, N, Nt, t_dev=None, bump=None, phase=0, gather=None):
         dims, hyp = self._dims(N, Nt, N, Nt)
         q_next = None
         if self.config["advantage"]:
@@ -718,7 +729,7 @@
         ops.critic_update(dims, hyp, self.policy.blob, self.q_funcs.blob, self.q_funcs.blob_T, self.target_q_funcs.blob, b,
                           o.m, o.v, o.t, o.lr, self._loss[0:1], self._ws, q_next=q_next, t_dev=t_dev,
                           policy_forward=self._policy_rides_along(), actor_blob_T=self.policy.blob_T,
-                          qtarg_blob_T=self.target_q_funcs.blob_T, bump=bump, phase=phase)
+                          qtarg_blob_T=self.target_q_funcs.blob_T, bump=bump, phase=phase, gather=gather)
 
     def actor_update(self, b, N, Nt, t_dev=None):
         dims, hyp = self._dims(N, Nt, N, Nt)
diff --git a/mobody-model-based-off-dynamics-offline-reinforcement-learning_amd/csrc/gather.h b/mobody-model-based-off-dynamics-offline-reinforcement-learning_amd/csrc/gather.h
--- /dev/null
+++ b/mobody-model-based-off-dynamics-offline-reinforcement-learning_amd/csrc/gather.h
@@ -0,0 +1,55 @@
+#pragma once
+#include "common.h"
+#include "rng.h"
+
+namespace mobody {
+
+__host__ __device__ inline bool view_packed(const MobodyBufferView& b, int S, int A) {
+  return b.pitch > 0 && b.pitch % 16 == 0 && b.pitch >= 2LL * S + A + 2 && (reinterpret_cast<uintptr_t>(b.state) & 15) == 0 &&
+         b.action == b.state + S && b.next_state == b.action + A && b.reward == b.next_state + S && b.not_done == b.reward + 1;
+}
+
+struct GatherArgs {
+  MobodyBufferView bufs[3];
+  int packed[3];
+  const int32_t* idx[3];
+  long long start[4];
+  int nbuf, S, A, WS;
+  float *state, *action, *next_state, *reward, *not_done;
+  uint32_t seed[3];
+  long long call_offset[3];
+  const long long* counter;
+  const long long* size[3];
+  long long* bump[4];
+  int nbump;
+};
+
+__host__ __device__ inline uint32_t div_magic(int n) { return (uint32_t)((0x100000000ULL + (uint32_t)n - 1) / (uint32_t)n); }
+__device__ __forceinline__ int fast_div(int e, uint32_t magic, int n) { return n == 1 ? e : (int)__umulhi((uint32_t)e, magic); }
+
+__device__ __forceinline__ long long gather_src(const GatherArgs& a, long long r, int& k) {
+  k = 0;
+  if (a.nbuf > 1 && r >= a.start[1]) k = 1;
+  if (a.nbuf > 2 && r >= a.start[2]) k = 2;
+  if (a.idx[k] != nullptr) return a.idx[k][r - a.start[k]];
+  const uint32_t call = (uint32_t)((a.counter ? a.counter[0] : 0) + a.call_offset[k]);
+  const long long sz = a.size[k][0];
+  return rng_index_at(a.seed[k], STREAM_SAMPLE, call, (uint64_t)(r - a.start[k]), (uint32_t)(sz > 0 ? sz : 1));
+}
+
+typedef float v4f __attribute__((ext_vector_type(4)));
+typedef const __attribute__((address_space(1))) v4f* gather_ptr_t;
+
+__device__ __forceinline__ gather_ptr_t gather_group_row(const float* mine, int p) {
+  const unsigned long long up = (unsigned long long)mine;
+  const unsigned lo = (unsigned)__shfl((int)(unsigned)up, (threadIdx.x & 48) + p, 64), hi = (unsigned)__shfl((int)(unsigned)(up >> 32), (threadIdx.x & 48) + p, 64);
+  return (gather_ptr_t)(((unsigned long long)hi << 32) | lo);
+}
+
+int gather_args_rng(const char* who, GatherArgs& a, const MobodyBufferView* bufs, const int64_t* counts, int nbuf, int S, int A,
+                    const uint32_t* seeds, const int64_t* call_offsets, const int64_t* counter, const int64_t* const* sizes,
+                    float* state, float* action, float* next_state, float* reward, float* not_done, int64_t* const* bump,
+                    int nbump, long long& N);
+int launch_gather(const GatherArgs& a, long long N, hipStream_t st);
+
+}
diff --git a/mobody-model-based-off-dynamics-offline-reinforcement-learning_amd/csrc/layers.h b/mobody-model-based-off-dynamics-offline-reinforcement-learning_amd/csrc/layers.h
--- a/mobody-model-based-off-dynamics-offline-reinforcement-learning_amd/csrc/layers.h
+++ b/mobody-model-based-off-dynamics-offline-reinforcement-learning_amd/csrc/layers.h
@@ -5,6 +5,7 @@
 #include <type_traits>
 
 #include "../../include/mobody_hip.h"
+#include "gather.h"
 #include "tile.h"
 
 namespace mobody {
@@ -162,6 +163,15 @@
   a.save_x = x; a.x_ms = x_ms; a.save_h1 = h1; a.save_h2 = h2; a.mask1 = m1; a.mask2 = m2; a.save_d1 = d1; a.save_d2 = d2;
 }
 
+struct FwdGather {
+  GatherArgs g;
+  int off[2], n[2];
+};
+inline void fwd_set_gather(FwdGather& fg, int k, const Mlp3FwdArgs& a, int off) {
+  fg.off[k] = off; fg.n[k] = a.n[0] + a.n[1] + a.n[2];
+}
+constexpr int FWD_GATHER_NQ = 2;
+
 template <class F>
 inline int dispatch_out_width(int Np3, F&& f) {
   return Np3 == 16 ? f(std::integral_constant<int, 1>{}) : Np3 == 32 ? f(std::integral_constant<int, 2>{})
@@ -172,6 +182,11 @@
 inline int launch_mlp3_forward(const Mlp3FwdArgs& a, int members, int act, int prec, hipStream_t st) {
   return launch_mlp3_forward(a, members, Mlp3FwdArgs{}, 0, act, prec, st);
 }
+
+int launch_mlp3_forward_gather(const Mlp3FwdArgs& a, int members_a, const Mlp3FwdArgs& b, int members_b, const FwdGather& fg,
+                               int prec, hipStream_t st);
+int launch_mlp3_fwd_bf_gather(const Mlp3FwdArgs& a, int members_a, const Mlp3FwdArgs& b, int members_b, const FwdGather& fg,
+                              int prec, hipStream_t st);
 
 constexpr int MLP_TILE_ROWS = 32;
 constexpr int MLP_MT = MLP_TILE_ROWS / 32;
@@ -186,6 +201,72 @@
     }
   }
   return c0;
+}
+
+template <int NQ>
+__device__ __forceinline__ void fwd_gather_rows(const FwdGather& fg, bool second, float* Xs, long long row0, int rows_here) {
+  const GatherArgs& g = fg.g;
+  const int lane = threadIdx.x & 15, grp = threadIdx.x >> 4;
+  const long long N = g.start[g.nbuf];
+  const float* mine = nullptr;
+  if (lane < 2) {
+    const long long r = min(row0 + 16 * lane + grp, N - 1);
+    int k;
+    const long long src = gather_src(g, r, k);
+    mine = g.bufs[k].state + src * g.bufs[k].pitch;
+  }
+  const int off = second ? fg.off[1] : fg.off[0], n = second ? fg.n[1] : fg.n[0];
+  const int q0 = off >> 2, q1 = (off + n + (second ? 2 : 0) + 3) >> 2;
+  v4f v[2][NQ];
+#pragma unroll
+  for (int p = 0; p < 2; ++p) {
+    const gather_ptr_t rp = gather_group_row(mine, p);
+#pragma unroll
+    for (int j = 0; j < NQ; ++j) v[p][j] = rp[min(q0 + lane + 16 * j, q1 - 1)];
+  }
+#pragma unroll
+  for (int p = 0; p < 2; ++p) {
+    const int r = 16 * p + grp;
+    const bool ok = r < rows_here;
+#pragma unroll
+    for (int j = 0; j < NQ; ++j) {
+      const int q = q0 + lane + 16 * j;
+      if (q >= q1) continue;
+#pragma unroll
+      for (int e = 0; e < 4; ++e) {
+        const int c = 4 * q + e - off;
+        if (c >= 0 && c < n) Xs[r * LDX + c] = ok ? v[p][j][e] : 0.f;
+        if (second && ok && c == n) g.reward[row0 + r] = v[p][j][e];
+        if (second && ok && c == n + 1) g.not_done[row0 + r] = v[p][j][e];
+      }
+    }
+  }
+}
+
+__device__ __forceinline__ int fwd_gather_tile(const FwdGather& fg, bool second, float* Xs, long long row0, int rows_here) {
+  if (blockIdx.x == 0 && blockIdx.y == 0 && threadIdx.x == 0)
+    for (int k = 0; k < fg.g.nbump; ++k) fg.g.bump[k][0] += 1;
+  const int off = second ? fg.off[1] : fg.off[0], n = second ? fg.n[1] : fg.n[0];
+  if (((off + n + (second ? 2 : 0) + 3) >> 2) - (off >> 2) <= 16) fwd_gather_rows<1>(fg, second, Xs, row0, rows_here);
+  else fwd_gather_rows<FWD_GATHER_NQ>(fg, second, Xs, row0, rows_here);
+  return n;
+}
+
+__device__ __forceinline__ void fwd_gather_save(const FwdGather& fg, bool second, int m, const float* Xs, long long row0, int rows_here) {
+  const GatherArgs& g = fg.g;
+  auto put = [&](float* out, int col0, int n) {
+    const uint32_t magic = div_magic(n);
+    for (int e = threadIdx.x; e < rows_here * n; e += NTHREADS) {
+      const int r = fast_div(e, magic, n);
+      out[row0 * n + e] = Xs[r * LDX + col0 + (e - r * n)];
+    }
+  };
+  if (second) {
+    put(g.next_state, 0, g.S);
+  } else if (m == 0) {
+    put(g.state, 0, g.S);
+    put(g.action, g.S, g.A);
+  }
 }
 
 __device__ __forceinline__ void fwd_save_x(const Mlp3FwdArgs& a, int m, const float* Xs, long long row0, int rows_here) {
diff --git a/mobody-model-based-off-dynamics-offline-reinforcement-learning_amd/csrc/mlp_fwd.hip b/mobody-model-based-off-dynamics-offline-reinforcement-learning_amd/csrc/mlp_fwd.hip
--- a/mobody-model-based-off-dynamics-offline-reinforcement-learning_amd/csrc/mlp_fwd.hip
+++ b/mobody-model-based-off-dynamics-offline-reinforcement-learning_amd/csrc/mlp_fwd.hip
@@ -34,8 +34,8 @@
   }
 }
 
-template <int ACT, int NT>
-__device__ __forceinline__ void mlp3_fwd_tile(const Mlp3FwdArgs& a, int m, float* Xs) {
+template <int ACT, int NT, bool GATHER = false>
+__device__ __forceinline__ void mlp3_fwd_tile(const Mlp3FwdArgs& a, int m, float* Xs, const FwdGather* fg = nullptr, bool second = false) {
   const long long row0 = (long long)blockIdx.x * TB;
   const int rows_here = (int)min((long long)TB, a.rows - row0);
   const float* w1 = a.w1 + m * a.sw1;
@@ -43,10 +43,12 @@
   TR(0);
   WideRing ring;
   wide_prefetch(w1, a.Kp1, ring);
-  tile_zero_cols(Xs, fwd_load_sources(a, m, Xs, row0, rows_here), a.Kp1, TB);
+  if constexpr (GATHER) tile_zero_cols(Xs, fwd_gather_tile(*fg, second, Xs, row0, rows_here), a.Kp1, TB);
+  else tile_zero_cols(Xs, fwd_load_sources(a, m, Xs, row0, rows_here), a.Kp1, TB);
   lds_barrier();
   TR(1);
   fwd_save_x(a, m, Xs, row0, rows_here);
+  if constexpr (GATHER) fwd_gather_save(*fg, second, m, Xs, row0, rows_here);
   const FwdTileOut t = fwd_tile_out(a, m, row0);
   float* h1 = t.h1;
   wide_layer<ACT, MLP_MT>(Xs, w1, a.b1 + m * a.sb1, a.Kp1, ring,
@@ -74,6 +76,15 @@
   mlp3_fwd_tile<ACT, NT>(s, second ? (int)blockIdx.y - members_a : (int)blockIdx.y, Xs);
 }
 
+template <int NT>
+__global__ __launch_bounds__(NTHREADS, 2) void k_mlp3_fwd2_gather(Mlp3FwdArgs a, Mlp3FwdArgs b, int members_a, FwdGather fg) {
+  extern __shared__ __attribute__((aligned(16))) float Xs[];
+  const bool second = (int)blockIdx.y >= members_a;
+  const Mlp3FwdArgs s = second ? b : a;
+  if ((long long)blockIdx.x * TB >= s.rows) return;
+  mlp3_fwd_tile<ACT_RELU, NT, true>(s, second ? (int)blockIdx.y - members_a : (int)blockIdx.y, Xs, &fg, second);
+}
+
 template <int ACT, int NT>
 static int launch_fwd_t(const Mlp3FwdArgs& a, int members, hipStream_t stream) {
   size_t lds = (size_t)TB * LDX * sizeof(float);
@@ -104,6 +115,21 @@
   ProfScope prof(PROF_MLP_FWD, stream);
   hipLaunchKernelGGL((k_mlp3_fwd2<ACT_RELU, NT>), grid, dim3(NTHREADS), lds, stream, a, b, members_a);
   MB_LAUNCH_OK("k_mlp3_fwd2");
+  return 0;
+}
+
+static int launch_fwd2_gather(const Mlp3FwdArgs& a, int members_a, const Mlp3FwdArgs& b, int members_b, const FwdGather& fg, hipStream_t stream) {
+  size_t lds = (size_t)TB * LDX * sizeof(float);
+  static bool once = false;
+  if (!once) {
+    int rc = allow_big_lds(k_mlp3_fwd2_gather<1>, 160 * 1024);
+    if (rc) return rc;
+    once = true;
+  }
+  dim3 grid((unsigned)cdiv(a.rows, TB), (unsigned)(members_a + members_b));
+  ProfScope prof(PROF_MLP_FWD, stream);
+  hipLaunchKernelGGL(k_mlp3_fwd2_gather<1>, grid, dim3(NTHREADS), lds, stream, a, b, members_a, fg);
+  MB_LAUNCH_OK("k_mlp3_fwd2_gather");
   return 0;
 }
 
@@ -140,6 +166,26 @@
     return rc ? rc : one(b, members_b);
   }
   return prec == PREC_F32 ? launch_fwd_pair(a, members_a, b, members_b, st) : launch_mlp3_fwd_bf(a, members_a, b, members_b, act, prec, st);
+}
+
+int launch_mlp3_forward_gather(const Mlp3FwdArgs& a, int members_a, const Mlp3FwdArgs& b, int members_b, const FwdGather& fg,
+                               int prec, hipStream_t st) {
+  const GatherArgs& g = fg.g;
+  const long long N = g.start[g.nbuf];
+  if (N <= 0 || members_a <= 0 || members_b <= 0) return fail(MOBODY_E_ARG, "launch_mlp3_forward_gather: needs both nets and a non-empty minibatch");
+  if (a.rows != N || b.rows != N) return fail(MOBODY_E_ARG, "launch_mlp3_forward_gather: the nets run on %lld / %lld rows, the minibatch has %lld", a.rows, b.rows, N);
+  for (int k = 0; k < g.nbuf; ++k)
+    if (!g.packed[k] && g.start[k + 1] > g.start[k]) return fail(MOBODY_E_ARG, "launch_mlp3_forward_gather: source %d is not a packed ring", k);
+  if (fg.off[0] != 0 || fg.n[0] != g.S + g.A || fg.off[1] != g.S + g.A || fg.n[1] != g.S)
+    return fail(MOBODY_E_ARG, "launch_mlp3_forward_gather: net a reads state | action, net b next_state");
+  auto chunks = [](int off, int n) { return ((off + n + 3) >> 2) - (off >> 2); };
+  const bool built = a.Np3 == 16 && (b.Np3 == 16 || (prec == PREC_F16X2 && b.Np3 == 32)) && nets_share_launch(a, b, ACT_RELU, prec) &&
+                     chunks(fg.off[0], fg.n[0]) <= 16 * FWD_GATHER_NQ && chunks(fg.off[1], fg.n[1] + 2) <= 16 * FWD_GATHER_NQ;
+  if (!built) {
+    int rc = launch_gather(g, N, st);
+    return rc ? rc : launch_mlp3_forward(a, members_a, b, members_b, ACT_RELU, prec, st);
+  }
+  return prec == PREC_F32 ? launch_fwd2_gather(a, members_a, b, members_b, fg, st) : launch_mlp3_fwd_bf_gather(a, members_a, b, members_b, fg, prec, st);
 }
 
 }
diff --git a/mobody-model-based-off-dynamics-offline-reinforcement-learning_amd/csrc/mlp_fwd_bf.hip b/mobody-model-based-off-dynamics-offline-reinforcement-learning_amd/csrc/mlp_fwd_bf.hip
--- a/mobody-model-based-off-dynamics-offline-reinforcement-learning_amd/csrc/mlp_fwd_bf.hip
+++ b/mobody-model-based-off-dynamics-offline-reinforcement-learning_amd/csrc/mlp_fwd_bf.hip
@@ -9,8 +9,8 @@
 constexpr int FWD_L1_RING = 3;
 constexpr int FWD_F16_WAVES = 4;
 
-template <int ACT, int PM, int NT, bool DS = false>
-__device__ __forceinline__ void mlp3_fwd_bf_tile(const Mlp3FwdArgs& a, int m, float* Xs) {
+template <int ACT, int PM, int NT, bool DS = false, bool GATHER = false>
+__device__ __forceinline__ void mlp3_fwd_bf_tile(const Mlp3FwdArgs& a, int m, float* Xs, const FwdGather* fg = nullptr, bool second = false) {
   char* Ps = reinterpret_cast<char*>(Xs);
   float* scr = reinterpret_cast<float*>(Ps + split_scr_offset<PM, TB>());
   const long long row0 = (long long)blockIdx.x * TB;
@@ -24,7 +24,9 @@
   WideRingT<FWD_L1_RING> ring;
   wide_prefetch(w1, a.Kp1, ring);
   int c0;
-  if (a.n[0] <= 32 && a.n[1] <= 32 && a.n[2] == 0) {
+  if constexpr (GATHER) {
+    c0 = fwd_gather_tile(*fg, second, Xs, row0, rows_here);
+  } else if (a.n[0] <= 32 && a.n[1] <= 32 && a.n[2] == 0) {
     tile_load2<TB>(Xs, a.src[0] + m * a.src_ms[0] + row0 * a.ld[0], a.ld[0], a.n[0],
                    a.n[1] > 0 ? a.src[1] + m * a.src_ms[1] + row0 * a.ld[1] : nullptr, a.ld[1], a.n[1], rows_here);
     c0 = a.n[0] + a.n[1];
@@ -35,6 +37,7 @@
   lds_barrier();
   TR(1);
   fwd_save_x(a, m, Xs, row0, rows_here);
+  if constexpr (GATHER) fwd_gather_save(*fg, second, m, Xs, row0, rows_here);
   const FwdTileOut t = fwd_tile_out(a, m, row0);
   float* d1 = DS ? a.save_d1 + ((long long)m * a.rows + row0) * HID : nullptr;
   float* d2 = DS ? a.save_d2 + ((long long)m * a.rows + row0) * HID : nullptr;
@@ -81,6 +84,47 @@
   }
 }
 
+template <int PM, int NT, int NT2 = NT>
+__global__ __launch_bounds__(NTHREADS, PM == 4 ? FWD_F16_WAVES : 2) void k_mlp3_fwd_bf_gather(Mlp3FwdArgs a, Mlp3FwdArgs b, int members_a, FwdGather fg) {
+  extern __shared__ __attribute__((aligned(16))) float Xs[];
+  const bool second = (int)blockIdx.y >= members_a;
+  const Mlp3FwdArgs s = second ? b : a;
+  if ((long long)blockIdx.x * TB >= s.rows) return;
+  if constexpr (NT2 == NT) {
+    mlp3_fwd_bf_tile<ACT_RELU, PM, NT, false, true>(s, second ? (int)blockIdx.y - members_a : (int)blockIdx.y, Xs, &fg, second);
+  } else {
+    if (second) mlp3_fwd_bf_tile<ACT_RELU, PM, NT2, false, true>(s, (int)blockIdx.y - members_a, Xs, &fg, true);
+    else mlp3_fwd_bf_tile<ACT_RELU, PM, NT, false, true>(s, (int)blockIdx.y, Xs, &fg, false);
+  }
+}
+
+template <int PM, int NT, int NT2 = NT>
+static int launch_bf_gather_t(const Mlp3FwdArgs& a, int members_a, const Mlp3FwdArgs& b, int members_b, const FwdGather& fg, hipStream_t st) {
+  constexpr size_t lds = split_lds_bytes<PM, TB>();
+  static bool once = false;
+  if (!once) {
+    int rc = allow_big_lds(k_mlp3_fwd_bf_gather<PM, NT, NT2>, 160 * 1024);
+    if (rc) return rc;
+    once = true;
+  }
+  ProfScope prof(PROF_MLP_FWD, st);
+  hipLaunchKernelGGL((k_mlp3_fwd_bf_gather<PM, NT, NT2>), dim3((unsigned)cdiv(a.rows, TB), (unsigned)(members_a + members_b)),
+                     dim3(NTHREADS), lds, st, a, b, members_a, fg);
+  MB_LAUNCH_OK("k_mlp3_fwd_bf_gather");
+  return 0;
+}
+
+int launch_mlp3_fwd_bf_gather(const Mlp3FwdArgs& a, int members_a, const Mlp3FwdArgs& b, int members_b, const FwdGather& fg,
+                              int prec, hipStream_t st) {
+  if (prec == PREC_F16X2 && b.Np3 == 32) return launch_bf_gather_t<4, 1, 2>(a, members_a, b, members_b, fg, st);
+  switch (prec) {
+    case PREC_BF16: return launch_bf_gather_t<1, 1>(a, members_a, b, members_b, fg, st);
+    case PREC_BF16X2: return launch_bf_gather_t<2, 1>(a, members_a, b, members_b, fg, st);
+    case PREC_BF16X3: return launch_bf_gather_t<3, 1>(a, members_a, b, members_b, fg, st);
+    default: return launch_bf_gather_t<4, 1>(a, members_a, b, members_b, fg, st);
+  }
+}
+
 template <int ACT, int PM, int NT, bool DS = false, int NT2 = NT>
 static int launch_bf_t(const Mlp3FwdArgs& a, int members_a, const Mlp3FwdArgs& b, int members_b, hipStream_t st) {
   constexpr size_t lds = split_lds_bytes<PM, TB>();
diff --git a/mobody-model-based-off-dynamics-offline-reinforcement-learning_amd/csrc/replay.hip b/mobody-model-based-off-dynamics-offline-reinforcement-learning_amd/csrc/replay.hip
--- a/mobody-model-based-off-dynamics-offline-reinforcement-learning_amd/csrc/replay.hip
+++ b/mobody-model-based-off-dynamics-offline-reinforcement-learning_amd/csrc/replay.hip
@@ -1,34 +1,12 @@
 #include <stdlib.h>
 
 #include "common.h"
+#include "gather.h"
 #include "rng.h"
 
 namespace mobody {
 
 constexpr int ROWS_WG = 16;
-
-__host__ __device__ inline bool view_packed(const MobodyBufferView& b, int S, int A) {
-  return b.pitch > 0 && b.pitch % 16 == 0 && b.pitch >= 2LL * S + A + 2 && (reinterpret_cast<uintptr_t>(b.state) & 15) == 0 &&
-         b.action == b.state + S && b.next_state == b.action + A && b.reward == b.next_state + S && b.not_done == b.reward + 1;
-}
-
-struct GatherArgs {
-  MobodyBufferView bufs[3];
-  int packed[3];
-  const int32_t* idx[3];
-  long long start[4];
-  int nbuf, S, A, WS;
-  float *state, *action, *next_state, *reward, *not_done;
-  uint32_t seed[3];
-  long long call_offset[3];
-  const long long* counter;
-  const long long* size[3];
-  long long* bump[4];
-  int nbump;
-};
-
-__host__ __device__ inline uint32_t div_magic(int n) { return (uint32_t)((0x100000000ULL + (uint32_t)n - 1) / (uint32_t)n); }
-__device__ __forceinline__ int fast_div(int e, uint32_t magic, int n) { return n == 1 ? e : (int)__umulhi((uint32_t)e, magic); }
 
 __device__ __forceinline__ void stage_to_batch(const float* stage, int WS, int off, int n, int rows, float* out) {
   const uint32_t magic = div_magic(n);
@@ -36,16 +14,6 @@
     const int r = fast_div(e, magic, n), c = e - r * n;
     out[e] = stage[r * WS + off + c];
   }
-}
-
-__device__ __forceinline__ long long gather_src(const GatherArgs& a, long long r, int& k) {
-  k = 0;
-  if (a.nbuf > 1 && r >= a.start[1]) k = 1;
-  if (a.nbuf > 2 && r >= a.start[2]) k = 2;
-  if (a.idx[k] != nullptr) return a.idx[k][r - a.start[k]];
-  const uint32_t call = (uint32_t)((a.counter ? a.counter[0] : 0) + a.call_offset[k]);
-  const long long sz = a.size[k][0];
-  return rng_index_at(a.seed[k], STREAM_SAMPLE, call, (uint64_t)(r - a.start[k]), (uint32_t)(sz > 0 ? sz : 1));
 }
 
 template <int P, int NQ>
@@ -65,14 +33,10 @@
     const long long src = gather_src(a, r, k);
     mine = a.bufs[k].state + src * a.bufs[k].pitch;
   }
-  typedef float v4f __attribute__((ext_vector_type(4)));
-  typedef const __attribute__((address_space(1))) v4f* gptr_t;
   v4f v[P][NQ];
 #pragma unroll
   for (int p = 0; p < P; ++p) {
-    const unsigned long long up = (unsigned long long)mine;
-    const unsigned lo = (unsigned)__shfl((int)(unsigned)up, (threadIdx.x & 48) + p, 64), hi = (unsigned)__shfl((int)(unsigned)(up >> 32), (threadIdx.x & 48) + p, 64);
-    gptr_t rp = (gptr_t)(((unsigned long long)hi << 32) | lo);
+    const gather_ptr_t rp = gather_group_row(mine, p);
 #pragma unroll
     for (int j = 0; j < NQ; ++j) v[p][j] = rp[min(lane + 16 * j, nq - 1)];
   }
@@ -138,7 +102,7 @@
   hipLaunchKernelGGL((k_gather_rows<P, NQ>), dim3((unsigned)cdiv(N, ROWS_WG * P)), dim3(256), lds, st, a);
 }
 
-static int launch_gather(const GatherArgs& a, long long N, hipStream_t st) {
+int launch_gather(const GatherArgs& a, long long N, hipStream_t st) {
   const size_t lds = (size_t)ROWS_WG * a.WS * sizeof(float);
   if (lds > 64 * 1024) return fail(MOBODY_E_ARG, "gather: rows of %d floats do not fit the LDS stage", a.WS);
   bool all_packed = true;
@@ -397,6 +361,28 @@
   return 0;
 }
 
+int mobody::gather_args_rng(const char* who, GatherArgs& a, const MobodyBufferView* bufs, const int64_t* counts, int nbuf, int S, int A,
+                            const uint32_t* seeds, const int64_t* call_offsets, const int64_t* counter, const int64_t* const* sizes,
+                            float* state, float* action, float* next_state, float* reward, float* not_done, int64_t* const* bump,
+                            int nbump, long long& N) {
+  N = 0;
+  MB_REQUIRE(bufs && counts && seeds && call_offsets && sizes && nbuf >= 1 && nbuf <= 3, "%s: need 1..3 source buffers", who);
+  MB_REQUIRE(nbump >= 0 && nbump <= 4 && (nbump == 0 || bump), "%s: at most 4 words to advance", who);
+  int rc = gather_common(who, a, bufs, counts, nbuf, S, A, state, action, next_state, reward, not_done, N);
+  if (rc || N == 0) return rc;
+  for (int k = 0; k < nbuf; ++k) {
+    MB_REQUIRE(counts[k] == 0 || sizes[k], "%s: null size word of source %d", who, k);
+    a.idx[k] = nullptr; a.seed[k] = seeds[k]; a.call_offset[k] = call_offsets[k]; a.size[k] = (const long long*)sizes[k];
+  }
+  a.counter = (const long long*)counter;
+  for (int k = 0; k < nbump; ++k) {
+    MB_REQUIRE(bump[k] && bump[k] != counter, "%s: bump word %d is null or the call counter itself", who, k);
+    a.bump[k] = (long long*)bump[k];
+  }
+  a.nbump = nbump;
+  return 0;
+}
+
 extern "C" int mobody_gather_batch(const MobodyBufferView* bufs, const int32_t* const* idx, const int64_t* counts,
                                    int nbuf, int S, int A, float* state, float* action, float* next_state,
                                    float* reward, float* not_done, void* stream) {
@@ -432,21 +418,10 @@
                                        const uint32_t* seeds, const int64_t* call_offsets, const int64_t* counter,
                                        const int64_t* const* sizes, float* state, float* action, float* next_state,
                                        float* reward, float* not_done, int64_t* const* bump, int nbump, void* stream) {
-  MB_REQUIRE(bufs && counts && seeds && call_offsets && sizes && nbuf >= 1 && nbuf <= 3, "mobody_gather_batch_rng: need 1..3 source buffers");
-  MB_REQUIRE(nbump >= 0 && nbump <= 4 && (nbump == 0 || bump), "mobody_gather_batch_rng: at most 4 words to advance");
   GatherArgs a{};
   long long N;
-  int rc = gather_common("mobody_gather_batch_rng", a, bufs, counts, nbuf, S, A, state, action, next_state, reward, not_done, N);
+  int rc = gather_args_rng("mobody_gather_batch_rng", a, bufs, counts, nbuf, S, A, seeds, call_offsets, counter, sizes, state, action,
+                           next_state, reward, not_done, bump, nbump, N);
   if (rc || N == 0) return rc;
-  for (int k = 0; k < nbuf; ++k) {
-    MB_REQUIRE(counts[k] == 0 || sizes[k], "mobody_gather_batch_rng: null size word of source %d", k);
-    a.idx[k] = nullptr; a.seed[k] = seeds[k]; a.call_offset[k] = call_offsets[k]; a.size[k] = (const long long*)sizes[k];
-  }
-  a.counter = (const long long*)counter;
-  for (int k = 0; k < nbump; ++k) {
-    MB_REQUIRE(bump[k] && bump[k] != counter, "mobody_gather_batch_rng: bump word %d is null or the call counter itself", k);
-    a.bump[k] = (long long*)bump[k];
-  }
-  a.nbump = nbump;
   return launch_gather(a, N, as_stream(stream));
 }
diff --git a/mobody-model-based-off-dynamics-offline-reinforcement-learning_amd/csrc/train.hip b/mobody-model-based-off-dynamics-offline-reinforcement-learning_amd/csrc/train.hip
--- a/mobody-model-based-off-dynamics-offline-reinforcement-learning_amd/csrc/train.hip
+++ b/mobody-model-based-off-dynamics-offline-reinforcement-learning_amd/csrc/train.hip
@@ -224,7 +224,7 @@
                        const float* state, const float* action,
                        const float* next_state, const float* reward, const float* not_done, const float* q_next,
                        float* grad_q, const AdamTarget& adam, float* loss_out, float* workspace, int policy_forward,
-                       void* stream, int phase = 0) {
+                       void* stream, int phase = 0, const FwdGather* gather = nullptr) {
   int rc = check_dims(d, "mobody_critic_step");
   if (rc) return rc;
   MB_REQUIRE(h && q_blob && q_blob_T && state && action && reward && not_done && (grad_q || adam.on) && loss_out && workspace,
@@ -244,7 +244,15 @@
                                   prec == PREC_F16X2 ? w.eh1q : nullptr);
   if (phase == 2) {
   } else if (q_next == nullptr) {
-    rc = launch_mlp3_forward(fq, 2, fwd_args(actor_blob, w.La, next_state, S, nullptr, 0, N, w.pin, 1, h->max_action, nullptr, nullptr, nullptr, nullptr, nullptr, aT), 1, ACT_RELU, prec, st);
+    const Mlp3FwdArgs fpn = fwd_args(actor_blob, w.La, next_state, S, nullptr, 0, N, w.pin, 1, h->max_action, nullptr, nullptr, nullptr, nullptr, nullptr, aT);
+    if (gather != nullptr) {
+      FwdGather fg = *gather;
+      fwd_set_gather(fg, 0, fq, 0);
+      fwd_set_gather(fg, 1, fpn, S + A);
+      rc = launch_mlp3_forward_gather(fq, 2, fpn, 1, fg, prec, st);
+    } else {
+      rc = launch_mlp3_forward(fq, 2, fpn, 1, ACT_RELU, prec, st);
+    }
     const Mlp3FwdArgs ft = fwd_args(qtarg_blob, w.Lq, next_state, S, w.pin, A, N, w.qt, 0, 1.f, nullptr, nullptr, nullptr, nullptr, nullptr, tT);
     if (!rc && policy_forward)
       rc = launch_mlp3_forward(ft, 2, fwd_args(actor_blob, w.La, state, S, nullptr, 0, N, w.pi, 1, h->max_action, w.xa, w.h1a, w.h2a, w.ma1, w.ma2, aT,
@@ -291,6 +299,33 @@
   at.bump = (long long*)bump;
   return critic_impl(d, h, actor_blob, actor_blob_T, q_blob, q_blob_T, qtarg_blob, qtarg_blob_T, state, action, next_state, reward,
                      not_done, q_next, nullptr, at, loss_out, workspace, policy_forward, stream);
+}
+
+extern "C" int mobody_critic_update_gather(const MobodyTrainDims* d, const MobodyHyper* h, const float* actor_blob,
+                                           const float* actor_blob_T, float* q_blob, float* q_blob_T, float* qtarg_blob,
+                                           float* qtarg_blob_T, float* state, float* action, float* next_state, float* reward,
+                                           float* not_done, const float* q_next, float* m, float* v, int64_t t,
+                                           const int64_t* t_dev, float lr, float* loss_out, float* workspace, int policy_forward,
+                                           int64_t* bump, int phase, const MobodyGatherRng* gr, void* stream) {
+  const char* who = "mobody_critic_update_gather";
+  MB_REQUIRE(h && q_blob && q_blob_T && qtarg_blob && m && v && d && gr, "%s: null pointer", who);
+  MB_REQUIRE(phase == 0, "%s: the step cannot be split (phase %d): the first forward launch writes the minibatch the backward reads", who, phase);
+  MB_REQUIRE(q_next == nullptr, "%s: q_next given: the launch that gathers is the one that evaluates pi(s')", who);
+  MB_REQUIRE(t_dev != nullptr || t >= 1, "%s: step t must be >= 1", who);
+  MB_REQUIRE(bump == nullptr || bump != t_dev, "%s: bump must not be the step word the launch reads", who);
+  FwdGather fg{};
+  long long N;
+  int rc = gather_args_rng(who, fg.g, gr->bufs, gr->counts, gr->nbuf, d->S, d->A, gr->seeds, gr->call_offsets, gr->counter, gr->sizes,
+                           state, action, next_state, reward, not_done, gr->bump, gr->nbump, N);
+  if (rc) return rc;
+  MB_REQUIRE(N == d->N, "%s: the counts add up to %lld rows, the step runs on %lld", who, N, (long long)d->N);
+  for (int k = 0; k < gr->nbuf; ++k)
+    MB_REQUIRE(gr->counts[k] == 0 || fg.g.packed[k], "%s: source %d is not a row-interleaved ring (mobody_ring_pitch)", who, k);
+  AdamTarget at = adam_target(q_blob, q_blob_T, m, v, qtarg_blob, t, t_dev, lr, h->tau, 1.f, h->precision);
+  at.target_T = qtarg_blob_T;
+  at.bump = (long long*)bump;
+  return critic_impl(d, h, actor_blob, actor_blob_T, q_blob, q_blob_T, qtarg_blob, qtarg_blob_T, state, action, next_state, reward,
+                     not_done, nullptr, nullptr, at, loss_out, workspace, policy_forward, stream, 0, &fg);
 }
 
 extern "C" int mobody_critic_update_phase(const MobodyTrainDims* d, const MobodyHyper* h, const float* actor_blob,
diff --git a/mobody-model-based-off-dynamics-offline-reinforcement-learning_amd/engine.py b/mobody-model-based-off-dynamics-offline-reinforcement-learning_amd/engine.py
--- a/mobody-model-based-off-dynamics-offline-reinforcement-learning_amd/engine.py
+++ b/mobody-model-based-off-dynamics-offline-reinforcement-learning_amd/engine.py
@@ -10,7 +10,7 @@
                use_src_sa_to_get_target_next_state=1, env_filter=10.0, rollout_from_src=0, fake_batch_scale=0.5,
                advantage=0, scale_Q=1, weight=2.5, bc_coef=1.0, q_weighted=1, filter_bad_rollout=1,
                penalty_coef=0.1, mopo=0, latent_reward=0, encoder_loss_coef=1, domain_loss_coef=0.0,
-               cycle_loss_coef=0.3)
+               cycle_loss_coef=0.3, fused_gather=1)
     cfg.update(over)
     return cfg
 
diff --git a/mobody-model-based-off-dynamics-offline-reinforcement-learning_amd/ops.py b/mobody-model-based-off-dynamics-offline-reinforcement-learning_amd/ops.py
--- a/mobody-model-based-off-dynamics-offline-reinforcement-learning_amd/ops.py
+++ b/mobody-model-based-off-dynamics-offline-reinforcement-learning_amd/ops.py
@@ -236,12 +236,15 @@
 
 
 def critic_update(dims, hyp, actor_blob, q_blob, q_blob_T, qtarg_blob, batch, m, v, t, lr, loss_out, ws, q_next=None,
-                  t_dev=None, policy_forward=False, actor_blob_T=None, qtarg_blob_T=None, bump=None, phase=0):
+                  t_dev=None, policy_forward=False, actor_blob_T=None, qtarg_blob_T=None, bump=None, phase=0, gather=None):
     s, a, s2, r, nd = batch
     args = (C.byref(dims), C.byref(hyp), ptr(actor_blob), ptr(actor_blob_T), ptr(q_blob), ptr(q_blob_T),
             ptr(qtarg_blob), ptr(qtarg_blob_T), ptr(s), ptr(a), ptr(s2), ptr(r), ptr(nd), ptr(q_next), ptr(m),
             ptr(v), int(t), ptr(t_dev), float(lr), ptr(loss_out), ptr(ws), int(bool(policy_forward)), ptr(bump))
-    if phase:
+    if gather is not None:
+        gr, keep = _gather_rng_args(**gather)
+        check(load().mobody_critic_update_gather(*args, int(phase), C.byref(gr), cur_stream()), "mobody_critic_update_gather")
+    elif phase:
         check(load().mobody_critic_update_phase(*args, int(phase), cur_stream()), "mobody_critic_update_phase")
     else:
         check(load().mobody_critic_update(*args, cur_stream()), "mobody_critic_update")
@@ -374,6 +377,17 @@
     check(load().mobody_adam_polyak_dev(in_dim, out_dim, members, ptr(blob), ptr(blob_T), ptr(grad), ptr(m), ptr(v),
                                         ptr(target), ptr(target_T), ptr(t_dev), float(lr), float(tau), float(grad_scale),
                                         prec_id(precision), cur_stream()), "mobody_adam_polyak_dev")
+
+
+def _gather_rng_args(buffers, counts, seeds, call_offsets, counter, sizes, bump=()):
+    n = len(buffers)
+    views = (_lib.MobodyBufferView * n)(*[buffer_view(b) for b in buffers])
+    cnt = (C.c_int64 * n)(*[int(c) for c in counts])
+    sd = (C.c_uint32 * n)(*[int(s) & 0xFFFFFFFF for s in seeds])
+    off = (C.c_int64 * n)(*[int(o) for o in call_offsets])
+    sz = (C.c_void_p * n)(*[ptr(s) for s in sizes])
+    bp = (C.c_void_p * max(1, len(bump)))(*[ptr(t) for t in bump])
+    return _lib.MobodyGatherRng(views, cnt, n, sd, off, ptr(counter), sz, bp, len(bump)), (views, cnt, sd, off, sz, bp)
 
 
 def gather_batch_rng(buffers, counts, seeds, call_offsets, counter, sizes, S, A, out, bump=()):
```

Result: faster. 47.81 million (median of 6 runs) (+1.1%).
